# StarsX/FluidX12

Measured on AMD Instinct MI355X. Metric: voxel-updates/sec (advect+40 Jacobi) at 256^3; achieved HBM GB/s vs peak, higher is better.
Workload: dtype f32

## Files before the change

fluidx12_amd/build.py:

```python
import os
import shutil
import subprocess
import sys

HERE = os.path.dirname(os.path.abspath(__file__))
CSRC = os.path.join(HERE, "csrc")
ROOT = os.path.dirname(HERE)
LIB = os.path.join(HERE, "libfluidx_hip.so")
OBJDIR = os.path.join(HERE, "build")

SOURCES = ["fx_api.cpp", "fx_knobs.cpp", "fx_context.cpp", "fx_schedule.cpp", "fx_jacobi_plan.cpp", "fx_emit_plan.cpp", "fx_heat_plan.cpp", "fx_comm.cpp", "fx_checkpoint.cpp", "fx_sim.hip", "fx_vorticity.hip", "fx_emit.hip", "fx_obstacle.hip", "fx_heat.hip", "fx_open.hip", "fx_advect_lds.hip", "fx_jacobi_strip.hip", "fx_jacobi_strip3.hip", "fx_jacobi_strip4.hip", "fx_jacobi_block.hip", "fx_jacobi_freeze.hip", "fx_jacobi_stripm.hip", "fx_jacobi2d.hip", "fx_render.hip", "fx_render_accel.hip", "fx_resolve.hip", "fx_bc6h.hip", "fx_sh.hip"]
HEADERS = ["fx_internal.h", "fx_context.h", "fx_host.h", "fx_hostmath.h", "fx_pk.h", "fx_march.h", "fx_store.h", "fx_knobs.h", os.path.join(ROOT, "include", "fluidx_hip.h")]

FLAGS = ["--offload-arch=gfx950", "-O3", "-std=c++17", "-fPIC", "-ffp-contract=off", "-fno-fast-math",
         "-Wall", "-Wno-unused-function", "-D__HIP_PLATFORM_AMD__"]
LAB = os.environ.get("FLUIDX_BUILD_LAB", "0") == "1"
if LAB:
    FLAGS = FLAGS + ["-DFX_LAB"]


EXTRA_FLAGS = {"fx_jacobi_strip3.hip": ["-mllvm", "-amdgpu-sched-strategy=max-ilp"] + (["-DFX_STRIP3C_ROWS=" + os.environ["FLUIDX_BUILD_STRIP3C_ROWS"]] if os.environ.get("FLUIDX_BUILD_STRIP3C_ROWS") else []),
               "fx_jacobi_strip.hip": ["-mllvm", "-amdgpu-sched-strategy=max-ilp"],
               "fx_jacobi_strip4.hip": (os.environ["FLUIDX_BUILD_STRIP4_SCHED"].split() if os.environ.get("FLUIDX_BUILD_STRIP4_SCHED") is not None else ["-mllvm", "-amdgpu-sched-strategy=max-ilp"]) + (["-DFX_STRIP4_OUTER_ROWS=" + os.environ["FLUIDX_BUILD_STRIP4_OUTER_ROWS"]] if os.environ.get("FLUIDX_BUILD_STRIP4_OUTER_ROWS") else []) + os.environ.get("FLUIDX_BUILD_STRIP4_DEFS", "").split(),
               "fx_render_accel.hip": [("-D%s=%s" % (d, os.environ[e])) for e, d in (("FLUIDX_BUILD_MASK_BITS", "FX_MASK_BUDGET_BITS"), ("FLUIDX_BUILD_VIEW_AHEAD", "FX_VIEW_AHEAD"), ("FLUIDX_BUILD_LIGHT_AHEAD", "FX_LIGHT_AHEAD"), ("FLUIDX_BUILD_LIGHT_RAY_WGS", "FX_LIGHT_RAY_WGS"), ("FLUIDX_BUILD_LIGHT_RAY_UNROLL", "FX_LIGHT_RAY_UNROLL"), ("FLUIDX_BUILD_VIEW_NT", "FX_VIEW_NT"), ("FLUIDX_BUILD_VIEW_WPE", "FX_VIEW_WPE")) if os.environ.get(e)],
               "fx_jacobi_freeze.hip": ["-mllvm", "-amdgpu-atomic-optimizer-strategy=None"] + (["-DFX_FREEZE_PROF"] if os.environ.get("FLUIDX_BUILD_FREEZE_PROF") else [])}


def kernel_source_hash(kernel):
    import hashlib
    import re
    pat = re.compile(r"\bvoid\s+" + re.escape(kernel) + r"\s*\(")
    for s in SOURCES:
        if not s.endswith(".hip"):
            continue
        text = open(os.path.join(CSRC, s), "rb").read()
        if pat.search(text.decode("utf-8", "replace")):
            h = hashlib.sha256()
            h.update(text)
            h.update(open(os.path.join(CSRC, "fx_pk.h"), "rb").read())
            if b'#include "fx_march.h"' in text:
                h.update(open(os.path.join(CSRC, "fx_march.h"), "rb").read())
            h.update(" ".join(FLAGS + EXTRA_FLAGS.get(s, [])).encode())
            return h.hexdigest()[:16]
    return None


def hipcc():
    exe = shutil.which("hipcc") or "/opt/rocm/bin/hipcc"
    if not os.path.exists(exe):
        raise RuntimeError("hipcc not found: the HIP library cannot be built")
    return exe


def _newer(path, deps):
    if not os.path.exists(path):
        return True
    t = os.path.getmtime(path)
    return any(os.path.getmtime(d) > t for d in deps)


def build_lib(force=False, verbose=False):
    os.makedirs(OBJDIR, exist_ok=True)
    hdrs = [h if os.path.isabs(h) else os.path.join(CSRC, h) for h in HEADERS]
    objs = []
    cc = hipcc()
# ... 63 lines not shown
```

fluidx12_amd/capi.py:

```python
import ctypes as C
import os

from . import build as _build

FX_OK = 0
FX_E_INVALID, FX_E_DEVICE, FX_E_NOMEM, FX_E_STATE, FX_E_COMM, FX_E_HALO = -1, -2, -3, -4, -5, -6

RAY_MARCH_DIRECT, RAY_MARCH_CUBEMAP, SEPARATE_LIGHT_PASS, OPTIMIZED = 0, 1, 2, 3
FRAME_COUNT = 3
STORAGE_FP32, STORAGE_FP16 = 0, 1
JACOBI_FIXED, JACOBI_FAITHFUL = 0, 1
ADDRESS_CLAMP, ADDRESS_MIRROR = 0, 1
FLAG_JACOBI_FUSE_MASK, FLAG_NO_OVERLAP, FLAG_RENDER_ONLY = 0xF, 0x10, 0x20
OPT_OVERLAP, OPT_JACOBI_ROUND, OPT_ADAPTIVE_HALO, OPT_COUNT_SAMPLES, OPT_RENDER_ACCEL = 1, 2, 3, 4, 5
ABI_VERSION = 7
(FIELD_VELOCITY, FIELD_VELOCITY1, FIELD_COLOR, FIELD_COLOR_PREV, FIELD_PRESSURE, FIELD_DIVERGENCE,
 FIELD_LIGHTMAP, FIELD_CUBEMAP, FIELD_TARGET, FIELD_TARGET_FLOAT, FIELD_CUBE_DEPTH) = range(11)
FIELD_TEMPERATURE = 11
DEPTH_DEVICE = 0x1
LIGHT_DIRECTIONAL, LIGHT_POINT = 0, 1
MAX_EMITTERS = 16
OBSTACLES_DEVICE = 0x1
MAX_HEAT_SOURCES = 16
WALL_X_LO, WALL_X_HI, WALL_Y_LO, WALL_Y_HI, WALL_Z_LO, WALL_Z_HI = 0x01, 0x02, 0x04, 0x08, 0x10, 0x20
# ... 16 lines not shown

class Light(C.Structure):
    _fields_ = [("struct_size", C.c_uint32), ("kind", C.c_uint32), ("position", C.c_float * 3), ("color", C.c_float * 4),
                ("ambient", C.c_float * 4)]


class Emitter(C.Structure):
    _fields_ = [("struct_size", C.c_uint32), ("flags", C.c_uint32), ("center", C.c_float * 3), ("radius", C.c_float),
                ("color_rate", C.c_float * 4), ("force", C.c_float * 3), ("swirl", C.c_float)]


class Buoyancy(C.Structure):
    _fields_ = [("struct_size", C.c_uint32), ("flags", C.c_uint32), ("ambient", C.c_float), ("density_weight", C.c_float),
                ("lift", C.c_float), ("cooling", C.c_float), ("up", C.c_float * 3)]


class HeatSource(C.Structure):
    _fields_ = [("struct_size", C.c_uint32), ("flags", C.c_uint32), ("center", C.c_float * 3), ("radius", C.c_float), ("rate", C.c_float)]


class Timing(C.Structure):
    _fields_ = [("advect_ms", C.c_double), ("divergence_ms", C.c_double), ("jacobi_ms", C.c_double),
                ("project_ms", C.c_double), ("light_ms", C.c_double), ("view_ms", C.c_double),
                ("exchange_ms", C.c_double), ("steps", C.c_uint64), ("jacobi_launches", C.c_uint64),
                ("jacobi_sweeps", C.c_uint64), ("renders", C.c_uint64), ("resolve_ms", C.c_double),
                ("jacobi_main_ms", C.c_double), ("jacobi_main_launches", C.c_uint64), ("jacobi_main_sweeps", C.c_uint64),
                ("exchange_bytes", C.c_uint64), ("advect_halo_planes", C.c_uint64), ("chain_ms", C.c_double),
                ("freeze_solves", C.c_uint64), ("freeze_sweeps", C.c_uint64), ("exchange_calls", C.c_uint64),
                ("view_samples", C.c_uint64), ("light_samples", C.c_uint64), ("lightmap_fetches", C.c_uint64),
                ("freeze_strip_launches", C.c_uint64)]


_vp, _fp = C.c_void_p, C.POINTER(C.c_float)
SYMBOLS = {
    "fx_abi_version": (C.c_int, []),
    "fx_error_string": (C.c_char_p, [C.c_int]),
    "fx_create": (C.c_int, [C.POINTER(_vp), C.POINTER(Desc)]),
    "fx_destroy": (C.c_int, [_vp]),
    "fx_set_max_samples": (C.c_int, [_vp, C.c_uint32, C.c_uint32]),
    "fx_set_sh": (C.c_int, [_vp, _fp]),
    "fx_update_frame": (C.c_int, [_vp, C.c_float, C.c_uint8, _fp, _fp, _fp]),
    "fx_simulate": (C.c_int, [_vp, _vp, C.c_uint8]),
    "fx_render": (C.c_int, [_vp, _vp, C.c_uint8, C.c_uint8]),
    "fx_get_frame_info": (C.c_int, [_vp, C.POINTER(FrameInfo)]),
    "fx_synchronize": (C.c_int, [_vp]),
    "fx_last_error": (C.c_char_p, [_vp]),
    "fx_upload": (C.c_int, [_vp, C.c_int, _vp, C.c_size_t]),
    "fx_download": (C.c_int, [_vp, C.c_int, _vp, C.c_size_t]),
    "fx_field_bytes": (C.c_size_t, [_vp, C.c_int]),
    "fx_field_digest": (C.c_int, [_vp, C.c_int, C.c_uint32, C.c_uint32, C.POINTER(C.c_uint64)]),
    "fx_checkpoint_save": (C.c_int, [_vp, C.c_char_p]),
    "fx_checkpoint_load": (C.c_int, [_vp, C.c_char_p]),
    "fx_advect": (C.c_int, [_vp, _vp]),
    "fx_divergence": (C.c_int, [_vp, _vp]),
    "fx_jacobi": (C.c_int, [_vp, _vp, C.c_uint32]),
    "fx_project": (C.c_int, [_vp, _vp]),
    "fx_set_vorticity_confinement": (C.c_int, [_vp, C.c_float]),
    "fx_confine_vorticity": (C.c_int, [_vp, _vp]),
    "fx_set_emitters": (C.c_int, [_vp, C.POINTER(Emitter), C.c_uint32]),
    "fx_get_emitters": (C.c_int, [_vp, C.POINTER(Emitter), C.c_uint32, C.POINTER(C.c_uint32)]),
    "fx_set_impulse": (C.c_int, [_vp, C.c_int]),
    "fx_emit": (C.c_int, [_vp, _vp]),
    "fx_set_obstacles": (C.c_int, [_vp, _vp, _vp, C.c_size_t, C.c_uint32]),
    "fx_get_obstacles": (C.c_int, [_vp, _vp, C.c_size_t, C.POINTER(C.c_uint64)]),
    "fx_enforce_obstacles": (C.c_int, [_vp, _vp]),
    "fx_set_buoyancy": (C.c_int, [_vp, C.POINTER(Buoyancy)]),
    "fx_get_buoyancy": (C.c_int, [_vp, C.POINTER(Buoyancy), C.POINTER(C.c_int)]),
    "fx_set_heat_sources": (C.c_int, [_vp, C.POINTER(HeatSource), C.c_uint32]),
    "fx_get_heat_sources": (C.c_int, [_vp, C.POINTER(HeatSource), C.c_uint32, C.POINTER(C.c_uint32)]),
    "fx_heat": (C.c_int, [_vp, _vp]),
    "fx_set_open_walls": (C.c_int, [_vp, C.c_uint32]),
    "fx_get_open_walls": (C.c_int, [_vp, C.POINTER(C.c_uint32)]),
    "fx_open_inflow": (C.c_int, [_vp, _vp]),
    "fx_sh_transform": (C.c_int, [_vp, _fp, C.c_uint32, _fp]),
    "fx_set_environment": (C.c_int, [_vp, _fp, C.c_uint32]),
    "fx_render_environment": (C.c_int, [_vp, _vp, C.c_uint8]),
    "fx_clear_render_target": (C.c_int, [_vp, _vp, _fp]),
    "fx_render_cube": (C.c_int, [_vp, _vp, C.c_uint8]),
    "fx_set_scene_depth": (C.c_int, [_vp, _vp, _vp, C.c_uint32, C.c_uint32, C.c_float, C.c_float, C.c_uint32]),
    "fx_set_light": (C.c_int, [_vp, C.POINTER(Light)]),
    "fx_get_light": (C.c_int, [_vp, C.POINTER(Light)]),
    "fx_dds_cube_info": (C.c_int, [_vp, C.c_size_t, C.POINTER(C.c_uint32), C.POINTER(C.c_uint32)]),
    "fx_dds_decode_cube": (C.c_int, [_vp, _vp, C.c_size_t, C.c_uint32, _fp, C.c_size_t]),
    "fx_timing_enable": (C.c_int, [_vp, C.c_int]),
    "fx_set_option": (C.c_int, [_vp, C.c_uint32, C.c_uint32]),
    "fx_set_knob": (C.c_int, [C.c_char_p, C.c_char_p]),
    "fx_knob_name": (C.c_char_p, [C.c_uint32]),
    "fx_comm_gather_color": (C.c_int, [_vp, _vp, _vp, C.c_int, C.POINTER(C.c_uint32), C.POINTER(C.c_uint32)]),
    "fx_timing_read": (C.c_int, [_vp, C.POINTER(Timing), C.c_int]),
    "fx_comm_id_bytes": (C.c_size_t, []),
    "fx_comm_get_unique_id": (C.c_int, [_vp, C.c_size_t]),
    "fx_comm_init_rank": (C.c_int, [_vp, _vp, C.c_size_t, C.c_int, C.c_int]),
    "fx_comm_init_local": (C.c_int, [C.POINTER(_vp), C.c_int]),
    "fx_comm_init_peer": (C.c_int, [C.POINTER(_vp), C.c_int]),
}

_lib = None
LAB_KNOBS = {"ADVECT_BLOCK", "ADVECT_FAST", "ADVECT_LDS_HALF", "ADVECT_TILE_ROWS", "ADVECT_ZCHUNK", "BLOCK_REMAP", "BLOCK_SHAPE", "DEBUG_NO_COPY",
             "FREEZE_DENSE_LEVELS", "FREEZE_DENSE_ONE", "FREEZE_FAST", "FREEZE_FUSE_DIV", "FREEZE_NT", "FREEZE_SHRINK", "FREEZE_T", "FREEZE_WGS",
             "JACOBI2D_TILE", "JACOBI_BLOCK", "JACOBI_BLOCKG", "LIGHT_FILL_DIRTY", "LIGHT_RAY_NT", "LIGHT_RAY_WGS", "OBSTACLE_V4", "PROJECT_V4", "ROW_VW",
             "STRIP3H_PAIRS", "STRIP3_COOP", "STRIP3_NO512", "STRIP3_OFF", "STRIP3_ZCHUNK", "STRIP4T", "STRIP4T_256", "STRIP4T_512", "STRIP4T_FROM", "STRIP4T_GRID", "STRIP4T_NARROW", "STRIP4T_NARROW_FROM", "STRIP4T_PIECES", "STRIP4X", "STRIP4X_MINP", "STRIP4X_NT", "STRIP4X_ORDER", "STRIP4X_WGS",
             "STRIP4_OCTET", "STRIP4_ZCHUNK", "STRIP4_ZFLOOR", "STRIP_GENERIC", "STRIP_R", "STRIP_REMAP", "STRIP_WGS", "STRIP_WIDE", "STRIP_ZCHUNK", "VIEW_ORDER", "VIEW_WGS", "VORT_ZCHUNK", "XCD_REMAP"}


def lib_path():
    return _build.LIB
# ... 62 lines not shown
```

fluidx12_amd/csrc/fx_advect_lds.hip:

```cpp
#include "fx_internal.h"
#include <algorithm>
#include <cstdlib>
#include <cstdio>

namespace fx {

namespace {

constexpr int TX = 64;
constexpr int HX = TX + 2;
constexpr int NSLOT = 4;
template <bool HALF, int TY> struct Lay {
	static constexpr int NCELL = HX * (TY + 2);
	static constexpr int VEL_BYTES = NCELL * 4;
	static constexpr int COL_BYTES = HALF ? 2 * NCELL * 4 : NCELL * 16;
	static constexpr int SLOT_BYTES = COL_BYTES + 3 * VEL_BYTES;
};
typedef _Float16 h16;
typedef _Float16 h16x4 __attribute__((ext_vector_type(4)));
__device__ __forceinline__ h16 to_h16(float v) { asm("" : "+v"(v)); return (h16)v; }
__device__ __forceinline__ float lo_half(uint32_t d) { return (float)__builtin_bit_cast(h16, (uint16_t)(d & 0xffffu)); }
__device__ __forceinline__ float hi_half(uint32_t d) { return (float)__builtin_bit_cast(h16, (uint16_t)(d >> 16)); }

__device__ __forceinline__ float lerpf(float a, float b, float f) { return fmaf(f, b - a, a); }
__device__ __forceinline__ float saturatef(float x) { return fminf(fmaxf(x, 0.0f), 1.0f); }

__device__ __forceinline__ int addr_tap(int i, int n, int mode)
{
	if (mode == FX_ADDRESS_MIRROR) {
		const int period = 2 * n;
		int m = i % period;
		if (m < 0) m += period;
		return m < n ? m : period - 1 - m;
	}
	return min(max(i, 0), n - 1);
}

typedef __attribute__((address_space(3))) void lds_void;
typedef const __attribute__((address_space(1))) void glb_void;

template <int VEL_BYTES>
__device__ __forceinline__ void stage64(const void* col, const void* v0, const void* v1, const void* v2, uint32_t off_col, uint32_t off_vel, uint32_t lds_col, uint32_t lds_vel)
{
	uint32_t keep;
	lds_col = __builtin_amdgcn_readfirstlane(lds_col);
	lds_vel = __builtin_amdgcn_readfirstlane(lds_vel);
	asm volatile(
		"s_mov_b32 %0, m0\n\t"
		"s_mov_b32 m0, %7\n\t"
		"s_nop 0\n\t"
		"global_load_lds_dwordx4 %5, %1\n\t"
		"s_mov_b32 m0, %8\n\t"
		"s_nop 0\n\t"
		"global_load_lds_dword %6, %2\n\t"
		"s_add_u32 m0, m0, %9\n\t"
		"s_nop 0\n\t"
		"global_load_lds_dword %6, %3\n\t"
		"s_add_u32 m0, m0, %9\n\t"
		"s_nop 0\n\t"
		"global_load_lds_dword %6, %4\n\t"
		"s_mov_b32 m0, %0"
		: "=&s"(keep)
		: "s"(col), "s"(v0), "s"(v1), "s"(v2), "v"(off_col), "v"(off_vel), "s"(lds_col), "s"(lds_vel), "n"(VEL_BYTES)
		: "scc");
}

template <int VEL_BYTES>
__device__ __forceinline__ void stage64h(const void* col, const void* v0, const void* v1, const void* v2, uint32_t off_col, uint32_t off_vel, uint32_t lds_col, uint32_t lds_vel)
{
	uint32_t keep;
	lds_col = __builtin_amdgcn_readfirstlane(lds_col);
	lds_vel = __builtin_amdgcn_readfirstlane(lds_vel);
	const uint32_t off_col_hi = off_col + 4u;
	asm volatile(
		"s_mov_b32 %0, m0\n\t"
		"s_mov_b32 m0, %8\n\t"
		"s_nop 0\n\t"
		"global_load_lds_dword %5, %1\n\t"
		"s_add_u32 m0, m0, %10\n\t"
		"s_nop 0\n\t"
		"global_load_lds_dword %6, %1\n\t"
		"s_mov_b32 m0, %9\n\t"
		"s_nop 0\n\t"
		"global_load_lds_ushort %7, %2\n\t"
		"s_add_u32 m0, m0, %10\n\t"
		"s_nop 0\n\t"
		"global_load_lds_ushort %7, %3\n\t"
		"s_add_u32 m0, m0, %10\n\t"
		"s_nop 0\n\t"
		"global_load_lds_ushort %7, %4\n\t"
		"s_mov_b32 m0, %0"
		: "=&s"(keep)
		: "s"(col), "s"(v0), "s"(v1), "s"(v2), "v"(off_col), "v"(off_col_hi), "v"(off_vel), "s"(lds_col), "s"(lds_vel), "n"(VEL_BYTES)
		: "scc");
}

template <typename T>
__device__ __forceinline__ T ldg32(const void* base, uint32_t byte_off)
{
	return *reinterpret_cast<const T*>(static_cast<const char*>(base) + byte_off);
}


template <bool P2> __device__ __forceinline__ uint32_t rows(uint32_t y, int lgX, const Geom& g) { return P2 ? y << lgX : y * (uint32_t)g.X; }
template <bool P2> __device__ __forceinline__ uint32_t planes(uint32_t z, int lgP, const Geom& g) { return P2 ? z << lgP : z * ((uint32_t)g.X * (uint32_t)g.Y); }

template <bool HALF, bool P2>
__device__ __forceinline__ void advect_gather(const Geom& g, const SimParams& sp, int ix, int iy, int z0, int z1, bool z_present, float fx, float fy, float fz,
	const char* v0, const char* v1, const char* v2, const void* __restrict__ col_in, int lgX, int lgP, unsigned* halo_overflow, float (&u)[3], float (&c)[4])
{
	const int xa0 = addr_tap(ix, g.X, sp.address), xa1 = addr_tap(ix + 1, g.X, sp.address);
	const int ya0 = addr_tap(iy, g.Y, sp.address), ya1 = addr_tap(iy + 1, g.Y, sp.address);
	if (!z_present) {
		atomicOr(halo_overflow, 1u);
		z0 = min(max(z0, g.zlo), g.zhi);
		z1 = min(max(z1, g.zlo), g.zhi);
	}
	const uint32_t p0 = planes<P2>((uint32_t)g.lz(z0), lgP, g), p1 = planes<P2>((uint32_t)g.lz(z1), lgP, g);
	const uint32_t ry0 = rows<P2>((uint32_t)ya0, lgX, g), ry1 = rows<P2>((uint32_t)ya1, lgX, g);
	const uint32_t c000 = p0 + ry0 + (uint32_t)xa0, c100 = p0 + ry0 + (uint32_t)xa1;
	const uint32_t c010 = p0 + ry1 + (uint32_t)xa0, c110 = p0 + ry1 + (uint32_t)xa1;
	const uint32_t c001 = p1 + ry0 + (uint32_t)xa0, c101 = p1 + ry0 + (uint32_t)xa1;
	const uint32_t c011 = p1 + ry1 + (uint32_t)xa0, c111 = p1 + ry1 + (uint32_t)xa1;
	const char* vb[3] = { v0, v1, v2 };
	auto gv = [](const char* b, uint32_t cell) -> float { return HALF ? (float)ldg32<h16>(b, cell * 2u) : ldg32<float>(b, cell * 4u); };
	auto gc = [&](uint32_t cell) -> float4 {
		if (HALF) { const h16x4 h = ldg32<h16x4>(col_in, cell * 8u); return make_float4((float)h.x, (float)h.y, (float)h.z, (float)h.w); }
		return ldg32<float4>(col_in, cell * 16u);
	};
#pragma unroll
	for (int a = 0; a < 3; ++a) {
		const float c00 = lerpf(gv(vb[a], c000), gv(vb[a], c100), fx);
		const float c10 = lerpf(gv(vb[a], c010), gv(vb[a], c110), fx);
		const float c01 = lerpf(gv(vb[a], c001), gv(vb[a], c101), fx);
		const float c11 = lerpf(gv(vb[a], c011), gv(vb[a], c111), fx);
		u[a] = lerpf(lerpf(c00, c10, fy), lerpf(c01, c11, fy), fz);
	}
	const float4 t000 = gc(c000), t100 = gc(c100), t010 = gc(c010), t110 = gc(c110);
	const float4 t001 = gc(c001), t101 = gc(c101), t011 = gc(c011), t111 = gc(c111);
#define FX_TRI(m) lerpf(lerpf(lerpf(t000.m, t100.m, fx), lerpf(t010.m, t110.m, fx), fy), \
	lerpf(lerpf(t001.m, t101.m, fx), lerpf(t011.m, t111.m, fx), fy), fz)
	c[0] = FX_TRI(x); c[1] = FX_TRI(y); c[2] = FX_TRI(z); c[3] = FX_TRI(w);
#undef FX_TRI
}

template <bool HALF, bool ALPHA>
__device__ __forceinline__ void advect_finish(const SimParams& sp, float (&u)[3], float (&c)[4], float ex, float dx, float dz, float dt, float atten,
	uint32_t id, uint32_t stride, void* __restrict__ vel_out, void* __restrict__ col_out, float* __restrict__ alpha_out)
{
	if (__builtin_amdgcn_ballot_w64(sp.impulse && ex > -6.5f) != 0) {
		const float basis = exp2f(ex);
		if (basis >= 0.0183156393f) {
			float Fx, Fy, Fz;
			if (sp.is3d) {
				Fx = fmaf(basis, 0.0f, dz * -200.0f);
				Fy = fmaf(basis, 192.0f, 0.0f);
				Fz = fmaf(basis, 0.0f, dx * 200.0f);
			} else {
				Fx = 0.0f; Fy = basis * 48.0f; Fz = 0.0f;
			}
			u[0] = fmaf(Fx, dt, u[0]); u[1] = fmaf(Fy, dt, u[1]); u[2] = fmaf(Fz, dt, u[2]);
			const float bdt = basis * dt;
			c[0] = saturatef(fmaf(bdt, 8.0f, c[0]));
			c[1] = saturatef(fmaf(bdt, 16.0f, c[1]));
			c[2] = saturatef(fmaf(bdt, 40.0f, c[2]));
			c[3] = saturatef(fmaf(bdt, 40.0f, c[3]));
		}
	}
	char* vo = static_cast<char*>(vel_out);
	char* co = static_cast<char*>(col_out);
	if (HALF) {
		*reinterpret_cast<h16*>(vo + id * 2u) = to_h16(u[0] * atten);
		*reinterpret_cast<h16*>(vo + (stride + id) * 2u) = to_h16(u[1] * atten);
		*reinterpret_cast<h16*>(vo + (2u * stride + id) * 2u) = to_h16(u[2] * atten);
		h16x4 hc;
		hc.x = to_h16(c[0] * atten); hc.y = to_h16(c[1] * atten); hc.z = to_h16(c[2] * atten); hc.w = to_h16(c[3] * atten);
		*reinterpret_cast<h16x4*>(co + id * 8u) = hc;
		if (ALPHA) *reinterpret_cast<float*>(reinterpret_cast<char*>(alpha_out) + id * 4u) = (float)hc.w;
	} else {
		*reinterpret_cast<float*>(vo + id * 4u) = u[0] * atten;
		*reinterpret_cast<float*>(vo + (stride + id) * 4u) = u[1] * atten;
		*reinterpret_cast<float*>(vo + (2u * stride + id) * 4u) = u[2] * atten;
		*reinterpret_cast<float4*>(co + id * 16u) = make_float4(c[0] * atten, c[1] * atten, c[2] * atten, c[3] * atten);
		if (ALPHA) *reinterpret_cast<float*>(reinterpret_cast<char*>(alpha_out) + id * 4u) = c[3] * atten;
	}
}

}

template <bool HALF, int TY, bool DEFER, bool P2, bool ALPHA>
__global__ __launch_bounds__(64 * TY) __attribute__((amdgpu_waves_per_eu(4, 4))) void k_advect_lds(const Geom g, const SimParams sp,
	const void* __restrict__ vel_in, const void* __restrict__ col_in, void* __restrict__ vel_out, void* __restrict__ col_out, float* __restrict__ alpha_out,
	int z_begin, int nzp, int zchunk, int nchunks, unsigned* halo_overflow, float rX, float rY, float rZ, float inv_rr,
	int lgX, int lgY, int lg_gx, int lg_gy, uint32_t* __restrict__ far_list, uint32_t* __restrict__ far_flat, uint32_t* __restrict__ far_total, uint32_t far_cap)
{
	__shared__ uint32_t far_n, far_base;
	extern __shared__ __attribute__((aligned(16))) char lds[];

	const int tid = (int)threadIdx.x, lane = tid & 63, wave = __builtin_amdgcn_readfirstlane(tid >> 6);
	const int ntx = P2 ? 1 << lg_gx : lg_gx, nty = P2 ? 1 << lg_gy : lg_gy;
	const int ntiles = ntx * nty * nchunks;
	int tl = (int)blockIdx.x;
	{
		const int q = ntiles >> 3, r = ntiles & 7, xcd = tl & 7, j = tl >> 3;
		tl = xcd * q + min(xcd, r) + j;
	}
	const int tx = P2 ? tl & (ntx - 1) : tl % ntx, ty = P2 ? (tl >> lg_gx) & (nty - 1) : (tl / ntx) % nty, chunk = P2 ? tl >> (lg_gx + lg_gy) : tl / (ntx * nty);
	const int x0t = tx << 6, y0t = ty * TY;
	const int zb = z_begin + chunk * zchunk, ze = min(zb + zchunk, z_begin + nzp);
	if (zb >= ze) return;

	const int lgP = lgX + lgY;
	constexpr int COL_BYTES = Lay<HALF, TY>::COL_BYTES, SLOT_BYTES = Lay<HALF, TY>::SLOT_BYTES;
	constexpr int NCELL = Lay<HALF, TY>::NCELL, VEL_BYTES = Lay<HALF, TY>::VEL_BYTES, NT = 64 * TY;
	constexpr uint32_t ES = HALF ? 2 : 4, CS = HALF ? 8 : 16;
	const uint32_t stride = planes<P2>((uint32_t)g.nzl(), lgP, g);
	const char* v0 = reinterpret_cast<const char*>(vel_in);
	const char* v1 = v0 + (size_t)stride * ES;
	const char* v2 = v1 + (size_t)stride * ES;

	uint32_t src_a, src_b = 0;
	{
		const int c = tid, r = c / HX, cc = c - r * HX;
		src_a = rows<P2>((uint32_t)addr_tap(y0t - 1 + r, g.Y, sp.address), lgX, g) + (uint32_t)addr_tap(x0t - 1 + cc, g.X, sp.address);
	}
	const bool has_b = NT + tid < NCELL;
	if (has_b) {
		const int c = NT + tid, r = c / HX, cc = c - r * HX;
		src_b = rows<P2>((uint32_t)addr_tap(y0t - 1 + r, g.Y, sp.address), lgX, g) + (uint32_t)addr_tap(x0t - 1 + cc, g.X, sp.address);
	}
	const bool wave_has_b = NT + wave * 64 < NCELL;

	const uint32_t lds0 = (uint32_t)(size_t)(__attribute__((address_space(3))) char*)lds;
	auto fill = [&](int zq) {
		const int za = min(max(addr_tap(zq, g.Zg, sp.address), g.zlo), g.zhi);
		const size_t pz = planes<P2>((uint32_t)g.lz(za), lgP, g);
		const uint32_t slot = __builtin_amdgcn_readfirstlane(lds0 + (uint32_t)(((zq + 4) & 3) * SLOT_BYTES));
		const char* bc = reinterpret_cast<const char*>(col_in) + pz * CS;
		const char *b0 = v0 + pz * ES, *b1 = v1 + pz * ES, *b2 = v2 + pz * ES;
		if (HALF) stage64h<VEL_BYTES>(bc, b0, b1, b2, src_a * CS, src_a * ES, slot + (uint32_t)wave * (64 * 4), slot + COL_BYTES + (uint32_t)wave * (64 * 4));
		else stage64<VEL_BYTES>(bc, b0, b1, b2, src_a * CS, src_a * ES, slot + (uint32_t)wave * (64 * 16), slot + COL_BYTES + (uint32_t)wave * (64 * 4));
		if (wave_has_b) {
			if (has_b) {
				if (HALF) stage64h<VEL_BYTES>(bc, b0, b1, b2, src_b * CS, src_b * ES, slot + (NT + (uint32_t)wave * 64) * 4, slot + COL_BYTES + (NT + (uint32_t)wave * 64) * 4);
				else stage64<VEL_BYTES>(bc, b0, b1, b2, src_b * CS, src_b * ES, slot + (NT + (uint32_t)wave * 64) * 16, slot + COL_BYTES + (NT + (uint32_t)wave * 64) * 4);
			}
		}
	};

	if (DEFER && tid == 0) far_n = 0u;
	fill(zb - 1);
	fill(zb);
	fill(zb + 1);
	asm volatile("s_waitcnt vmcnt(0)" ::: "memory");
	__syncthreads();

	const int x = x0t + lane, y = y0t + wave;
	const bool has_voxel = P2 || (x < g.X && y < g.Y);
	const float dt = sp.dt;
	const float px = P2 ? ((float)x + 0.5f) * rX : ((float)x + 0.5f) / (float)g.X;
	const float py = P2 ? ((float)y + 0.5f) * rY : ((float)y + 0.5f) / (float)g.Y;
	const float dx = px + -0.5f, dy = py + -0.100000001f;
	const float dxy2 = fmaf(dy, dy, dx * dx);
	const uint32_t own = (uint32_t)((wave + 1) * HX + lane + 1);
	const float atten = fmaxf(fmaf(-dt, 0.200000003f, 1.0f), 0.0f);

	auto compute = [&](int z) {
		if (!has_voxel) return;
		const float pz = P2 ? ((float)z + 0.5f) * rZ : ((float)z + 0.5f) / (float)g.Zg;
		const float dz = pz + -0.5f;
		const float d2 = fmaf(dz, dz, dxy2);
		const float ex = ((d2 * -4.0f) * inv_rr) * 1.44269502f;

		const char* sc = lds + ((z + 4) & 3) * SLOT_BYTES;
		const uint32_t* vs = reinterpret_cast<const uint32_t*>(sc + COL_BYTES);
		auto vval = [](uint32_t d) -> float { return HALF ? lo_half(d) : __uint_as_float(d); };
		const float u0x = vval(vs[own]), u0y = vval(vs[NCELL + own]), u0z = vval(vs[2 * NCELL + own]);
		const float ax = fmaf(-u0x, dt, px), ay = fmaf(-u0y, dt, py), az = fmaf(-u0z, dt, pz);
		const float tx_ = ax * (float)g.X - 0.5f, ty_ = ay * (float)g.Y - 0.5f, tz_ = az * (float)g.Zg - 0.5f;
		const float flx = floorf(tx_), fly = floorf(ty_), flz = floorf(tz_);
		const float fx = tx_ - flx, fy = ty_ - fly, fz = tz_ - flz;
		const int ix = (int)flx, iy = (int)fly, iz = (int)flz;
		const int jx = ix - x, jy = iy - y, jz = iz - z;
		int z0 = addr_tap(iz, g.Zg, sp.address), z1 = addr_tap(iz + 1, g.Zg, sp.address);
		const bool z_present = z0 >= g.zlo && z0 <= g.zhi && z1 >= g.zlo && z1 <= g.zhi;
		const bool inwin = (unsigned)(jx + 1) <= 1u && (unsigned)(jy + 1) <= 1u && (unsigned)(jz + 1) <= 1u && z_present;

		float u[3], c[4];
		if (DEFER && !inwin) {
			const uint32_t slot = atomicAdd(&far_n, 1u);
			far_list[(size_t)blockIdx.x * far_cap + slot] = P2 ? (uint32_t)x | (uint32_t)y << lgX | (uint32_t)z << lgP
				: ((uint32_t)z * (uint32_t)g.Y + (uint32_t)y) * (uint32_t)g.X + (uint32_t)x;
		}
		if (DEFER || inwin) {
			const int kx = DEFER && !inwin ? 0 : jx, ky = DEFER && !inwin ? 0 : jy, kz = DEFER && !inwin ? z : iz;
			const uint32_t c0 = (uint32_t)((int)own + ky * HX + kx);
			const char* s0 = lds + ((kz + 4) & 3) * SLOT_BYTES;
			const char* s1 = lds + ((kz + 5) & 3) * SLOT_BYTES;
#pragma unroll
			for (int a = 0; a < 3; ++a) {
				const uint32_t* p0 = reinterpret_cast<const uint32_t*>(s0 + COL_BYTES + a * VEL_BYTES) + c0;
				const uint32_t* p1 = reinterpret_cast<const uint32_t*>(s1 + COL_BYTES + a * VEL_BYTES) + c0;
				const float c00 = lerpf(vval(p0[0]), vval(p0[1]), fx);
				const float c10 = lerpf(vval(p0[HX]), vval(p0[HX + 1]), fx);
				const float c01 = lerpf(vval(p1[0]), vval(p1[1]), fx);
				const float c11 = lerpf(vval(p1[HX]), vval(p1[HX + 1]), fx);
				u[a] = lerpf(lerpf(c00, c10, fy), lerpf(c01, c11, fy), fz);
			}
			float4 t000, t100, t010, t110, t001, t101, t011, t111;
			if (HALF) {
				auto tex = [](const char* slot, uint32_t c) -> float4 {
					const uint32_t rg = reinterpret_cast<const uint32_t*>(slot)[c], ba = reinterpret_cast<const uint32_t*>(slot)[NCELL + c];
					return make_float4(lo_half(rg), hi_half(rg), lo_half(ba), hi_half(ba));
				};
				t000 = tex(s0, c0); t100 = tex(s0, c0 + 1); t010 = tex(s0, c0 + HX); t110 = tex(s0, c0 + HX + 1);
				t001 = tex(s1, c0); t101 = tex(s1, c0 + 1); t011 = tex(s1, c0 + HX); t111 = tex(s1, c0 + HX + 1);
			} else {
				const float4* q0 = reinterpret_cast<const float4*>(s0) + c0;
				const float4* q1 = reinterpret_cast<const float4*>(s1) + c0;
				t000 = q0[0]; t100 = q0[1]; t010 = q0[HX]; t110 = q0[HX + 1];
				t001 = q1[0]; t101 = q1[1]; t011 = q1[HX]; t111 = q1[HX + 1];
			}
#define FX_TRI(m) lerpf(lerpf(lerpf(t000.m, t100.m, fx), lerpf(t010.m, t110.m, fx), fy), \
	lerpf(lerpf(t001.m, t101.m, fx), lerpf(t011.m, t111.m, fx), fy), fz)
			c[0] = FX_TRI(x); c[1] = FX_TRI(y); c[2] = FX_TRI(z); c[3] = FX_TRI(w);
#undef FX_TRI
		} else {
			advect_gather<HALF, P2>(g, sp, ix, iy, z0, z1, z_present, fx, fy, fz, v0, v1, v2, col_in, lgX, lgP, halo_overflow, u, c);
		}

		const uint32_t id = planes<P2>((uint32_t)g.lz(z), lgP, g) + rows<P2>((uint32_t)y, lgX, g) + (uint32_t)x;
		advect_finish<HALF, ALPHA>(sp, u, c, ex, dx, dz, dt, atten, id, stride, vel_out, col_out, alpha_out);
	};

	for (int z = zb; z < ze; ++z) {
		if (z + 2 <= ze) fill(z + 2);
		compute(z);
		if (!(P2 || y < g.Y)) asm volatile("s_waitcnt vmcnt(0)" ::: "memory");
		else if (ALPHA) asm volatile("s_waitcnt vmcnt(5)" ::: "memory");
		else asm volatile("s_waitcnt vmcnt(4)" ::: "memory");
		__syncthreads();
	}
	if (DEFER) {
		const uint32_t n = far_n;
		if (n != 0u) {
			if (tid == 0) far_base = atomicAdd(far_total, n);
			__syncthreads();
			const uint32_t base = far_base;
			const uint32_t* seg = far_list + (size_t)blockIdx.x * far_cap;
			for (uint32_t i = (uint32_t)tid; i < n; i += (uint32_t)NT) far_flat[base + i] = seg[i];
		}
	}
}

template <bool HALF, bool P2, bool ALPHA>
__global__ __launch_bounds__(256) void k_advect_far(const Geom g, const SimParams sp,
	const void* __restrict__ vel_in, const void* __restrict__ col_in, void* __restrict__ vel_out, void* __restrict__ col_out, float* __restrict__ alpha_out,
	const uint32_t* __restrict__ far_flat, const uint32_t* __restrict__ far_total, uint32_t* __restrict__ far_total_next, unsigned* halo_overflow,
	float rX, float rY, float rZ, float inv_rr, int lgX, int lgY)
{
	const uint32_t n = *far_total;
	if (blockIdx.x == 0 && threadIdx.x == 0) *far_total_next = 0u;
	const int lgP = lgX + lgY;
	constexpr uint32_t ES = HALF ? 2 : 4;
	const uint32_t stride = planes<P2>((uint32_t)g.nzl(), lgP, g);
	const char* v0 = reinterpret_cast<const char*>(vel_in);
	const char* v1 = v0 + (size_t)stride * ES;
	const char* v2 = v1 + (size_t)stride * ES;
	const float dt = sp.dt;
	const float atten = fmaxf(fmaf(-dt, 0.200000003f, 1.0f), 0.0f);
	for (uint32_t i = blockIdx.x * 256u + threadIdx.x; i < n; i += gridDim.x * 256u) {
		const uint32_t code = far_flat[i];
		int x, y, z;
		if (P2) { x = (int)(code & (uint32_t)(g.X - 1)); y = (int)((code >> lgX) & (uint32_t)(g.Y - 1)); z = (int)(code >> lgP); }
		else { const uint32_t XY = (uint32_t)g.X * (uint32_t)g.Y, rem = code % XY; z = (int)(code / XY); y = (int)(rem / (uint32_t)g.X); x = (int)(rem % (uint32_t)g.X); }
		const float px = P2 ? ((float)x + 0.5f) * rX : ((float)x + 0.5f) / (float)g.X;
		const float py = P2 ? ((float)y + 0.5f) * rY : ((float)y + 0.5f) / (float)g.Y;
		const float pz = P2 ? ((float)z + 0.5f) * rZ : ((float)z + 0.5f) / (float)g.Zg;
		const float dx = px + -0.5f, dy = py + -0.100000001f, dz = pz + -0.5f;
		const float dxy2 = fmaf(dy, dy, dx * dx);
		const float d2 = fmaf(dz, dz, dxy2);
		const float ex = ((d2 * -4.0f) * inv_rr) * 1.44269502f;
		const uint32_t id = planes<P2>((uint32_t)g.lz(z), lgP, g) + rows<P2>((uint32_t)y, lgX, g) + (uint32_t)x;
		auto gv = [](const char* b, uint32_t cell) -> float { return HALF ? (float)ldg32<h16>(b, cell * 2u) : ldg32<float>(b, cell * 4u); };
		const float u0x = gv(v0, id), u0y = gv(v1, id), u0z = gv(v2, id);
		const float ax = fmaf(-u0x, dt, px), ay = fmaf(-u0y, dt, py), az = fmaf(-u0z, dt, pz);
		const float tx_ = ax * (float)g.X - 0.5f, ty_ = ay * (float)g.Y - 0.5f, tz_ = az * (float)g.Zg - 0.5f;
		const float flx = floorf(tx_), fly = floorf(ty_), flz = floorf(tz_);
		const float fx = tx_ - flx, fy = ty_ - fly, fz = tz_ - flz;
		const int ix = (int)flx, iy = (int)fly, iz = (int)flz;
		const int z0 = addr_tap(iz, g.Zg, sp.address), z1 = addr_tap(iz + 1, g.Zg, sp.address);
		const bool z_present = z0 >= g.zlo && z0 <= g.zhi && z1 >= g.zlo && z1 <= g.zhi;
		float u[3], c[4];
		advect_gather<HALF, P2>(g, sp, ix, iy, z0, z1, z_present, fx, fy, fz, v0, v1, v2, col_in, lgX, lgP, halo_overflow, u, c);
		advect_finish<HALF, ALPHA>(sp, u, c, ex, dx, dz, dt, atten, id, stride, vel_out, col_out, alpha_out);
	}
}


hipError_t launch_advect_lds(const Geom& g, const SimParams& sp, int half_store, const void* vel_in, const void* col_in,
	void* vel_out, void* col_out, int z_begin, int z_end, unsigned* halo_overflow, uint32_t* far_scratch, size_t far_words, int far_parity, bool* far_used, hipStream_t s, bool force,
	AdvectAlpha* alpha)
{
	if (far_used) *far_used = false;
	if (alpha) alpha->written = false;
	auto pow2 = [](int v) { return v > 0 && (v & (v - 1)) == 0; };
	const int nzp = z_end - z_begin;
	const bool p2 = pow2(g.X) && pow2(g.Y) && pow2(g.Zg);
	const int TY = p2 && FX_KNOB_INT("ADVECT_TILE_ROWS", 8) == 16 ? 16 : 8;
	const size_t min_voxels = (size_t)1 << 22;
	if (g.Zg <= 1 || g.X < TX || g.Y < TY || nzp < 12 || (!force && (size_t)g.X * g.Y * (size_t)nzp < min_voxels) ||
		g.cells_local() * 16 >= ((size_t)1 << 32))
		return hipErrorNotSupported;
	const int half_on = FX_KNOB_INT("ADVECT_LDS_HALF", 1);
	if (half_store && !half_on) return hipErrorNotSupported;
	auto lg = [](int v) { int k = 0; while ((1 << k) < v) ++k; return k; };
	const int ntx = (g.X + TX - 1) / TX, nty = (g.Y + TY - 1) / TY;
	const int lgX = lg(g.X), lgY = lg(g.Y), lg_gx = p2 ? lg(ntx) : ntx, lg_gy = p2 ? lg(nty) : nty;
	const int tiles_xy = ntx * nty;
	const bool want_defer = far_scratch && FX_KNOB_INT("ADVECT_DEFER", 1) != 0;
	int zchunk = FX_KNOB_INT("ADVECT_ZCHUNK", want_defer ? 32 : 16);
	if (!p2 && !FX_KNOB("ADVECT_ZCHUNK")) {
		const int chunks = std::max(1, 512 / tiles_xy);
		zchunk = std::max(8, (nzp + chunks - 1) / chunks);
	}
	if (zchunk < 4) zchunk = 4;
	if (zchunk > nzp) zchunk = nzp;
	const int nchunks = (nzp + zchunk - 1) / zchunk;
	const float rX = 1.0f / (float)g.X, rY = 1.0f / (float)g.Y, rZ = 1.0f / (float)g.Zg, inv_rr = sp.is3d ? 256.0f : 1024.0f;
	const uint32_t nwg = (uint32_t)(tiles_xy * nchunks), far_cap = (uint32_t)(TX * TY * zchunk);
	const size_t flat_words = (size_t)g.X * g.Y * (size_t)nzp;
	const bool defer = want_defer && far_words >= 2 + flat_words + (size_t)nwg * far_cap && ((uint64_t)g.Zg << (lgX + lgY)) <= ((uint64_t)1 << 32);
	if (far_used) *far_used = defer;
	uint32_t* far_total = far_scratch ? far_scratch + (far_parity & 1) : nullptr;
	uint32_t* far_total_next = far_scratch ? far_scratch + ((far_parity & 1) ^ 1) : nullptr;
	uint32_t* far_flat = far_scratch ? far_scratch + 2 : nullptr;
	uint32_t* far_list = far_scratch ? far_scratch + 2 + flat_words : nullptr;
#define FX_ADV(H_, TY_, D_, P_, A_) do { \
		static bool attr_set = false; \
		if (!attr_set) { (void)hipFuncSetAttribute(reinterpret_cast<const void*>(k_advect_lds<H_, TY_, D_, P_, A_>), hipFuncAttributeMaxDynamicSharedMemorySize, NSLOT * Lay<H_, TY_>::SLOT_BYTES); attr_set = true; } \
		hipLaunchKernelGGL((k_advect_lds<H_, TY_, D_, P_, A_>), dim3(tiles_xy * nchunks), dim3(64 * TY_), (NSLOT * Lay<H_, TY_>::SLOT_BYTES), s, g, sp, vel_in, col_in, vel_out, col_out, alpha_out, \
			z_begin, nzp, zchunk, nchunks, halo_overflow, rX, rY, rZ, inv_rr, lgX, lgY, lg_gx, lg_gy, far_list, far_flat, far_total, far_cap); } while (0)
#define FX_FAR(H_, P_, A_) hipLaunchKernelGGL((k_advect_far<H_, P_, A_>), dim3(far_wgs), dim3(256), 0, s, g, sp, vel_in, col_in, vel_out, col_out, alpha_out, far_flat, far_total, far_total_next, halo_overflow, rX, rY, rZ, inv_rr, lgX, lgY)
	const int far_wgs = 1024;
	float* alpha_out = alpha && alpha->out && defer && TY == 8 && g.nzl() == g.Zg && z_begin == 0 && z_end == g.Zg ? alpha->out : nullptr;
	if (alpha_out) {
		if (half_store) { if (p2) { FX_ADV(true, 8, true, true, true); FX_FAR(true, true, true); } else { FX_ADV(true, 8, true, false, true); FX_FAR(true, false, true); } }
		else { if (p2) { FX_ADV(false, 8, true, true, true); FX_FAR(false, true, true); } else { FX_ADV(false, 8, true, false, true); FX_FAR(false, false, true); } }
		alpha->written = true;
	} else if (!p2) {
		if (defer) {
			if (half_store) { FX_ADV(true, 8, true, false, false); FX_FAR(true, false, false); } else { FX_ADV(false, 8, true, false, false); FX_FAR(false, false, false); }
		} else { if (half_store) FX_ADV(true, 8, false, false, false); else FX_ADV(false, 8, false, false, false); }
	} else if (defer) {
		if (TY == 16) { if (half_store) FX_ADV(true, 16, true, true, false); else FX_ADV(false, 16, true, true, false); }
		else { if (half_store) FX_ADV(true, 8, true, true, false); else FX_ADV(false, 8, true, true, false); }
		if (half_store) FX_FAR(true, true, false); else FX_FAR(false, true, false);
	} else {
		if (TY == 16) { if (half_store) FX_ADV(true, 16, false, true, false); else FX_ADV(false, 16, false, true, false); }
		else { if (half_store) FX_ADV(true, 8, false, true, false); else FX_ADV(false, 8, false, true, false); }
	}
#undef FX_FAR
#undef FX_ADV
	return hipGetLastError();
}

size_t advect_far_words(const Geom& g, int nzp)
{
	if (g.Zg <= 1 || g.X < TX || g.Y < 16 || nzp < 12) return 0;
	const size_t tiled = (size_t)((g.X + TX - 1) / TX * TX) * (size_t)((g.Y + 7) / 8 * 8);
	return 2 + (size_t)g.X * g.Y * (size_t)nzp + tiled * (size_t)(nzp + 32);
}

}
```

fluidx12_amd/csrc/fx_api.cpp:

```cpp
#include "fx_host.h"
#include <cstring>
#include "fx_hostmath.h"

using namespace fx;
using namespace fxh;

extern "C" {

int fx_abi_version(void) { return FX_ABI_VERSION; }

int fx_set_max_samples(fx_ctx* ctx, uint32_t max_ray, uint32_t max_light)
{
	if (!ctx || !max_ray || !max_light) return FX_E_INVALID;
	ctx->max_ray_samples = max_ray;
	ctx->max_light_samples = max_light;
	return FX_OK;
}

int fx_set_sh(fx_ctx* ctx, const float* coeffs27)
{
	if (!ctx) return FX_E_INVALID;
	if (!ctx->sh_dev) return FX_E_STATE;
	if (!coeffs27) { ctx->has_sh = false; return FX_OK; }
	DeviceGuard dg(ctx->device);
// ... 295 lines not shown

int fx_set_environment(fx_ctx* ctx, const float* cube, uint32_t n)
{
	if (!ctx || (cube && (!n || n > 8192))) return FX_E_INVALID;
	DeviceGuard dg(ctx->device);
	FX_HIP(hipDeviceSynchronize());
	if (ctx->env) { FX_HIP(hipFree(ctx->env)); ctx->env = nullptr; ctx->env_n = 0; }
	if (!cube) return FX_OK;
	const size_t bytes = (size_t)6 * n * n * 3 * sizeof(float);
	FX_HIP(hipMalloc((void**)&ctx->env, bytes));
	FX_HIP(hipMemcpy(ctx->env, cube, bytes, hipMemcpyHostToDevice));
	ctx->env_n = n;
	return FX_OK;
}

int fx_render_environment(fx_ctx* ctx, void* stream, uint8_t frame_index)
{
	if (!ctx || frame_index >= FX_FRAME_COUNT) return FX_E_INVALID;
	if (!ctx->env || !ctx->view_valid) return FX_E_STATE;
	DeviceGuard dg(ctx->device);
	hipStream_t s = pick_stream(ctx, stream);
	int rc = ensure_target(ctx, s);
	if (rc) return rc;
	ScopedMark mk(ctx, s, MK_RESOLVE);
	FX_HIP(launch_environment(ctx->env, (int)ctx->env_n, ctx->fc, (int)ctx->desc.viewport_w, (int)ctx->desc.viewport_h,
		ctx->target, ctx->target_float, s));
	return FX_OK;
}

int fx_get_frame_info(fx_ctx* ctx, fx_frame_info* out)
{
	if (!ctx || !out) return FX_E_INVALID;
	out->cube_lod = ctx->cube_lod;
	out->cube_size = (uint32_t)ctx->g.X >> ctx->cube_lod;
	out->ray_samples = ctx->ray_samples;
	out->visibility_mask = ctx->visibility_mask;
	out->frame_parity = ctx->frame_parity;
	out->edge_pixels = ctx->edge_pixels;
	out->time_step = ctx->time_step;
	std::memcpy(out->world_view_proj_i, ctx->fc.wvp_i, sizeof out->world_view_proj_i);
	std::memcpy(out->screen_to_world, ctx->fc.s2w, sizeof out->screen_to_world);
	return FX_OK;
}

int fx_advect(fx_ctx* ctx, void* stream)
{
	if (!ctx) return FX_E_INVALID;
	if (ctx->desc.flags & FX_FLAG_RENDER_ONLY) return FX_E_STATE;
	if (!ctx->frame_valid) return FX_E_STATE;
	if (ctx->nranks > 1) return FX_E_INVALID;
	hipStream_t s = pick_stream(ctx, stream);
	ScopedMark mk(ctx, s, MK_ADVECT);
	return advect_range(ctx, s, owned(ctx), false);
}

static int sim_guard(const fx_ctx* ctx, bool whole = true)
{
	if (!ctx) return FX_E_INVALID;
	if (ctx->desc.flags & FX_FLAG_RENDER_ONLY) return FX_E_STATE;
	if (whole && (ctx->g.nz != ctx->g.Zg || ctx->nranks > 1)) return FX_E_INVALID;
	return FX_OK;
}

static int run_stage(fx_ctx* ctx, void* stream, int (*phase)(fx_ctx*, hipStream_t))
{
	const int rc = sim_guard(ctx);
	return rc ? rc : phase(ctx, pick_stream(ctx, stream));
}

int fx_set_vorticity_confinement(fx_ctx* ctx, float epsilon)
{
	if (!std::isfinite(epsilon) || epsilon < 0.0f) return FX_E_INVALID;
	if (const int rc = sim_guard(ctx)) return rc;
	ctx->vort_eps = epsilon;
	return FX_OK;
}

int fx_confine_vorticity(fx_ctx* ctx, void* stream) { return run_stage(ctx, stream, confine_phase); }

int fx_set_emitters(fx_ctx* ctx, const fx_emitter* list, uint32_t count)
{
	if (const int rc = sim_guard(ctx)) return rc;
	if (count > FX_MAX_EMITTERS || (count && !list)) return FX_E_INVALID;
	for (uint32_t k = 0; k < count; ++k) {
		const fx_emitter& e = list[k];
		if (e.struct_size != sizeof(fx_emitter) || e.flags != 0) return FX_E_INVALID;
		if (!std::isfinite(e.radius) || !(e.radius > 0.0f) || !std::isfinite(e.swirl)) return FX_E_INVALID;
		for (int a = 0; a < 3; ++a) if (!std::isfinite(e.center[a]) || !std::isfinite(e.force[a])) return FX_E_INVALID;
		for (int a = 0; a < 4; ++a) if (!std::isfinite(e.color_rate[a]) || e.color_rate[a] < 0.0f) return FX_E_INVALID;
	}
	ctx->emitters.assign(list, list + count);
	return FX_OK;
}

int fx_get_emitters(fx_ctx* ctx, fx_emitter* out, uint32_t capacity, uint32_t* count)
{
	if (const int rc = sim_guard(ctx, false)) return rc;
	if (!count || (capacity && !out)) return FX_E_INVALID;
	*count = (uint32_t)ctx->emitters.size();
	for (uint32_t k = 0; k < capacity && k < *count; ++k) out[k] = ctx->emitters[k];
	return FX_OK;
}

int fx_set_impulse(fx_ctx* ctx, int enabled)
{
	if (const int rc = sim_guard(ctx, !enabled)) return rc;
// ... 333 lines not shown
			hipMemcpyAsync(ctx->rec_host, ctx->gath_dev, 4 * sizeof(int) * (size_t)nranks, hipMemcpyDeviceToHost, ctx->stream) == hipSuccess &&
			hipStreamSynchronize(ctx->stream) == hipSuccess;
		bool tiles = ok;
		for (int r = 0; ok && r + 1 < nranks; ++r) tiles = tiles && ctx->rec_host[4 * r] + ctx->rec_host[4 * r + 1] == ctx->rec_host[4 * (r + 1)];
		if (ok) ok = hipMemset(ctx->step_rec, 0, 4 * sizeof(int)) == hipSuccess;
		if (!ok || !tiles) {
			ctx->last_error = ok ? "fx_comm_init_rank: the slabs of the ranks do not tile the grid in rank order" : "fx_comm_init_rank: exchanging the slab ranges failed";
			std::fprintf(stderr, "fluidx: %s\n", ctx->last_error.c_str());
			destroy_lanes(g); delete t; delete g;
			return ok ? FX_E_INVALID : FX_E_COMM;
		}
	}
	ctx->group = g; ctx->rank = rank; ctx->nranks = nranks;
	return FX_OK;
}

int fx_comm_gather_color(fx_ctx* ctx, void* stream, fx_ctx* full, int root, const uint32_t* slab_z0, const uint32_t* slab_nz)
{
	if (!ctx || !ctx->group || root < 0 || root >= ctx->nranks) return FX_E_INVALID;
	if (group_broken(ctx)) return FX_E_STATE;
	if (!is_driver(ctx)) return FX_OK;
	const bool local = ctx->group->transport->is_local();
	const bool am_root = local || ctx->rank == root;
	if (am_root) {
		if (!full || full->g.X != ctx->g.X || full->g.Y != ctx->g.Y || full->g.Zg != ctx->g.Zg || full->g.nz != full->g.Zg ||
			full->half != ctx->half) return FX_E_INVALID;
		if (!local && full->device != ctx->device) return FX_E_INVALID;
		if (local && full->device != ctx->group->members[(size_t)root]->device) return FX_E_INVALID;
	}
	if (!local && (!slab_z0 || !slab_nz)) return FX_E_INVALID;
	const size_t plane_bytes = ctx->g.plane() * 4 * elem_size(ctx);
	std::vector<GatherPart> parts((size_t)ctx->nranks);
	for (int r = 0; r < ctx->nranks; ++r) {
		const fx_ctx* m = local ? ctx->group->members[r] : (r == ctx->rank ? ctx : nullptr);
		const uint32_t z0 = local ? (uint32_t)m->g.z0 : slab_z0[r], nz = local ? (uint32_t)m->g.nz : slab_nz[r];
		if (z0 > (uint32_t)ctx->g.Zg || nz > (uint32_t)ctx->g.Zg - z0) return FX_E_INVALID;
		if (!local && r == ctx->rank && (z0 != (uint32_t)ctx->g.z0 || nz != (uint32_t)ctx->g.nz)) return FX_E_INVALID;
		parts[r].rank = r;
		parts[r].bytes = (size_t)nz * plane_bytes;
		parts[r].src = m ? (const char*)m->col[m->frame_parity] + (size_t)m->g.H * plane_bytes : nullptr;
		parts[r].dst = am_root ? (char*)full->col[full->frame_parity] + (size_t)z0 * plane_bytes : nullptr;
		if (am_root) full->accel_alpha_of = nullptr;
	}
	DeviceGuard dg(ctx->device);
	hipStream_t s = pick_stream(ctx, stream);
	if (ctx->halo_fault) return FX_E_HALO;
	std::vector<hipStream_t> streams;
	if (ctx->group->per_member) for (fx_ctx* m : ctx->group->members) streams.push_back(m->stream);
	else streams.push_back(s);
	hipStream_t done_on = ctx->group->per_member ? streams[(size_t)root] : s;
	ScopedMark mk(ctx, s, MK_EXCH);
	int rc = ctx->group->transport->gather(ctx->group, parts, root, streams);
	if (rc) return rc;
	if (am_root && full->stream != done_on) {
		fx_lane& L = ctx->group->per_member ? ctx->group->lanes[(size_t)root] : ctx->group->lanes[0];
		DeviceGuard dgr(L.device);
		FX_HIP(hipEventRecord(L.ev_done, done_on));
		DeviceGuard dgf(full->device);
		FX_HIP(hipStreamWaitEvent(full->stream, L.ev_done, 0));
	}
	return FX_OK;
}

static int check_local_members(fx_ctx** ctxs, int nranks, bool one_device)
{
	if (!ctxs || nranks < 1) return FX_E_INVALID;
	int zexp = 0;
	for (int r = 0; r < nranks; ++r) {
		if (!ctxs[r]) return FX_E_INVALID;
		int rc = check_slab_chain(ctxs[r], r, nranks);
		if (rc) return rc;
		if (ctxs[r]->g.z0 != zexp || (one_device && ctxs[r]->device != ctxs[0]->device)) return FX_E_INVALID;
		const fx_desc &a = ctxs[r]->desc, &b = ctxs[0]->desc;
		if (a.grid_x != b.grid_x || a.grid_y != b.grid_y || a.grid_z != b.grid_z || a.halo_advect != b.halo_advect ||
			a.halo_jacobi != b.halo_jacobi || a.jacobi_iters != b.jacobi_iters || a.jacobi_mode != b.jacobi_mode ||
			a.storage != b.storage || a.advect_address != b.advect_address)
			return FX_E_INVALID;
		for (int q = 0; q < r; ++q) if (ctxs[q] == ctxs[r]) return FX_E_INVALID;
		zexp += ctxs[r]->g.nz;
	}
	return FX_OK;
}

static int init_in_process_group(fx_ctx** ctxs, int nranks, bool peer)
{
	int rc = check_local_members(ctxs, nranks, !peer);
	if (rc) return rc;
	if (peer) {
		for (int r = 0; r + 1 < nranks; ++r) {
			const int a = ctxs[r]->device, b = ctxs[r + 1]->device;
			if (a == b) continue;
			int ab = 0, ba = 0;
			if (hipDeviceCanAccessPeer(&ab, a, b) != hipSuccess || hipDeviceCanAccessPeer(&ba, b, a) != hipSuccess || !ab || !ba) {
				ctxs[0]->last_error = "fx_comm_init_peer: two neighbouring slabs live on devices without peer access";
				return FX_E_DEVICE;
			}
			for (int k = 0; k < 2; ++k) {
				DeviceGuard dg(k ? b : a);
				const hipError_t e = hipDeviceEnablePeerAccess(k ? a : b, 0);
				if (e != hipSuccess && e != hipErrorPeerAccessAlreadyEnabled) { (void)hipGetLastError(); return FX_E_DEVICE; }
				(void)hipGetLastError();
			}
		}
	}
	for (int r = 0; r < nranks; ++r)
		if (!ctxs[r]->step_rec) { if ((rc = make_step_record(ctxs[r], 1, false))) return rc; }
// ... 28 lines not shown
```

fluidx12_amd/csrc/fx_context.cpp:

```cpp
#include "fx_host.h"
#include <time.h>

using namespace fx;
using namespace fxh;

namespace fx {
bool digest_range_ok(const Geom& g, uint32_t z_begin, uint32_t z_count)
{
	if (!z_count) return true;
	if (g.nz < 0 || z_count > (uint32_t)g.nz) return false;
	const int64_t first = (int64_t)z_begin, end = first + (int64_t)z_count;
	return first >= (int64_t)g.z0 && end <= (int64_t)g.z0 + (int64_t)g.nz;
}
}

namespace fxh {

size_t ev_record(fx_ctx* c, hipStream_t s)
{
	if (c->ev_used == c->ev.size()) {
		hipEvent_t e;
		if (hipEventCreate(&e) != hipSuccess) return (size_t)-1;
		c->ev.push_back(e);
	}
// ... 12 lines not shown
		case MK_DIV: c->acc.divergence_ms += ms; break;
		case MK_JACOBI: c->acc.jacobi_ms += ms; c->acc.jacobi_launches += m.launches; c->acc.jacobi_sweeps += m.sweeps;
			c->acc.jacobi_main_ms += ms; c->acc.jacobi_main_launches += m.launches; c->acc.jacobi_main_sweeps += m.sweeps; break;
		case MK_JACOBI_TAIL: c->acc.jacobi_ms += ms; c->acc.jacobi_launches += m.launches; c->acc.jacobi_sweeps += m.sweeps; break;
		case MK_PROJECT: c->acc.project_ms += ms; break;
		case MK_LIGHT: c->acc.light_ms += ms; break;
		case MK_VIEW: c->acc.view_ms += ms; break;
		case MK_EXCH: c->acc.exchange_ms += ms; break;
		case MK_RESOLVE: c->acc.resolve_ms += ms; break;
		case MK_CHAIN: c->acc.chain_ms += ms; break;
		}
	}
	c->marks.clear();
	c->ev_used = 0;
	return FX_OK;
}

int ensure_stage(fx_ctx* ctx, size_t bytes)
{
	if (ctx->stage_bytes >= bytes) return FX_OK;
	if (ctx->stage) { FX_HIP(hipFree(ctx->stage)); ctx->stage = nullptr; ctx->stage_bytes = 0; }
	FX_HIP(hipMalloc((void**)&ctx->stage, bytes));
	ctx->stage_bytes = bytes;
	return FX_OK;
}

void destroy_lanes(fx_comm_group* g)
{
	for (fx_lane& l : g->lanes) {
		DeviceGuard dg(l.device);
		if (l.comm) (void)hipStreamDestroy(l.comm);
		if (l.face) (void)hipStreamDestroy(l.face);
		for (hipEvent_t e : { l.ev_ready, l.ev_done, l.ev_col_ready, l.ev_col_done, l.ev_int, l.ev_face1, l.x_ready, l.x_done }) if (e) (void)hipEventDestroy(e);
	}
	g->lanes.clear();
}

void group_release(fx_comm_group* g)
{
	{
		DeviceGuard dg(g->lanes.empty() ? 0 : g->lanes[0].device);
		if (g->shared_stream) (void)hipStreamDestroy(g->shared_stream);
	}
	destroy_lanes(g);
	delete g->transport;
	delete g;
}

void free_all(fx_ctx* c)
{
	for (int i = 0; i < 2; ++i) {
		if (c->vel[i]) (void)hipFree(c->vel[i]);
		if (c->col[i]) (void)hipFree(c->col[i]);
		if (c->p[i]) (void)hipFree(c->p[i]);
	}
	void* others[] = { c->env, c->cube_depth, c->depth_own, c->accel.occ, c->accel.alpha, c->accel.bits, c->accel.list, c->accel.cells, c->accel.gi, c->accel.ctr, c->target, c->target_float, c->p_face[0], c->p_face[1], c->b, c->frozen, c->frozen_alt, c->lightmap, c->cube, c->sh_dev, c->halo_overflow, c->stage,
		c->sh_scratch[0], c->sh_scratch[1], c->sh_scratch[2], c->sh_scratch[3], c->p_aux, c->fz_mask[0], c->fz_mask[1], c->fz_mask[2], c->fz_tile_next, c->fz_stat, c->fz_list[0], c->fz_list[1], c->fz_counts, c->sample_counters, c->adv_far, c->obst_code, c->obst_spare, c->obst_stats, c->temp[0], c->temp[1] };
	for (void* q : others) if (q) (void)hipFree(q);
	for (hipEvent_t e : c->ev) (void)hipEventDestroy(e);
	if (c->step_rec) (void)hipFree(c->step_rec);
	if (c->gath_dev) (void)hipFree(c->gath_dev);
	if (c->rec_host) (void)hipHostFree(c->rec_host);
	if (c->fz_active_host) (void)hipHostFree(c->fz_active_host);
	if (c->fz_active_ev) (void)hipEventDestroy(c->fz_active_ev);
	if (c->rec_ev) (void)hipEventDestroy(c->rec_ev);
	if (c->owns_stream && c->stream) (void)hipStreamDestroy(c->stream);
}

}

extern "C" {

const char* fx_error_string(int status)
{
	switch (status) {
	case FX_OK: return "ok";
	case FX_E_INVALID: return "invalid argument";
	case FX_E_DEVICE: return "HIP device/runtime error";
	case FX_E_NOMEM: return "out of memory";
	case FX_E_STATE: return "invalid call order";
	case FX_E_COMM: return "RCCL communication error";
	case FX_E_HALO: return "advection back-trace left the exchanged halo";
	default: return "unknown status";
	}
}

int fx_create(fx_ctx** out, const fx_desc* d)
{
	if (!out || !d || d->struct_size != sizeof(fx_desc)) return FX_E_INVALID;
	*out = nullptr;
	if (!d->grid_x || !d->grid_y || !d->grid_z) return FX_E_INVALID;
	if (d->grid_x != d->grid_y) return FX_E_INVALID;
	if (d->grid_x > 65535 || d->grid_z > 65535) return FX_E_INVALID;
	if (d->storage > FX_STORAGE_FP16 || d->jacobi_mode > FX_JACOBI_FAITHFUL || d->advect_address > FX_ADDRESS_MIRROR) return FX_E_INVALID;
	if (!d->jacobi_iters) return FX_E_INVALID;
	uint32_t z0 = d->slab_z0, nz = d->slab_nz ? d->slab_nz : d->grid_z;
	if (z0 + nz > d->grid_z) return FX_E_INVALID;
	const bool slab = nz != d->grid_z;

	int ndev = 0;
	if (hipGetDeviceCount(&ndev) != hipSuccess || ndev <= 0) return FX_E_DEVICE;
	int dev = d->device;
	if (dev < 0 && hipGetDevice(&dev) != hipSuccess) return FX_E_DEVICE;
	if (dev >= ndev) return FX_E_INVALID;

	fx_ctx* ctx = new (std::nothrow) fx_ctx();
	if (!ctx) return FX_E_NOMEM;
	ctx->desc = *d;
	ctx->desc.slab_z0 = z0; ctx->desc.slab_nz = nz;
	default_light(ctx);
// ... 29 lines not shown
			FX_HIP(hipMalloc((void**)&ctx->p[i], cells * 4));
			FX_HIP(hipMemsetAsync(ctx->vel[i], 0, 3 * cells * es, ctx->stream));
			FX_HIP(hipMemsetAsync(ctx->col[i], 0, 4 * cells * es, ctx->stream));
			FX_HIP(hipMemsetAsync(ctx->p[i], 0, cells * 4, ctx->stream));
		}
		if (slab && !(d->flags & FX_FLAG_RENDER_ONLY))
			for (int i = 0; i < 2; ++i) {
				FX_HIP(hipMalloc((void**)&ctx->p_face[i], cells * 4));
				FX_HIP(hipMemsetAsync(ctx->p_face[i], 0, cells * 4, ctx->stream));
			}
		if (!(d->flags & FX_FLAG_RENDER_ONLY)) {
			FX_HIP(hipMalloc((void**)&ctx->b, cells * 4));
			FX_HIP(hipMemsetAsync(ctx->b, 0, cells * 4, ctx->stream));
		}
		if (d->jacobi_mode == FX_JACOBI_FAITHFUL && !(d->flags & FX_FLAG_RENDER_ONLY)) {
			FX_HIP(hipMalloc((void**)&ctx->frozen, cells));
			FX_HIP(hipMemsetAsync(ctx->frozen, 0, cells, ctx->stream));
			if (ctx->g.Zg == 1) {
				FX_HIP(hipMalloc((void**)&ctx->frozen_alt, cells));
				FX_HIP(hipMemsetAsync(ctx->frozen_alt, 0, cells, ctx->stream));
			}
			if (jacobi_freeze_supported(ctx->g)) {
				const size_t mb = jacobi_freeze_mask_bytes(ctx->g), nt = (size_t)jacobi_freeze_tiles(ctx->g);
				FX_HIP(hipMalloc((void**)&ctx->p_aux, cells * 4));
				FX_HIP(hipMemsetAsync(ctx->p_aux, 0, cells * 4, ctx->stream));
				for (int i = 0; i < 3; ++i) {
					FX_HIP(hipMalloc((void**)&ctx->fz_mask[i], mb));
					FX_HIP(hipMemsetAsync(ctx->fz_mask[i], 0, mb, ctx->stream));
				}
				FX_HIP(hipMalloc((void**)&ctx->fz_tile_next, nt * sizeof(uint32_t)));
				FX_HIP(hipMemsetAsync(ctx->fz_tile_next, 0, nt * sizeof(uint32_t), ctx->stream));
				for (int i = 0; i < 2; ++i) FX_HIP(hipMalloc(&ctx->fz_list[i], jacobi_freeze_list_bytes(ctx->g)));
				FX_HIP(hipMalloc((void**)&ctx->fz_counts, 2 * jacobi_freeze_count_words() * sizeof(uint32_t)));
				FX_HIP(hipMemsetAsync(ctx->fz_counts, 0, 2 * jacobi_freeze_count_words() * sizeof(uint32_t), ctx->stream));
				FX_HIP(hipMalloc((void**)&ctx->fz_stat, kFreezeStatRing * sizeof(uint32_t)));
				FX_HIP(hipMemsetAsync(ctx->fz_stat, 0, kFreezeStatRing * sizeof(uint32_t), ctx->stream));
				ctx->fz_iters.assign(kFreezeStatRing, 0);
				if (jacobi_freeze_strip_supported(ctx->g) && hipHostMalloc((void**)&ctx->fz_active_host, 64, hipHostMallocMapped) == hipSuccess) {
					ctx->fz_active_host[0] = 0u;
					if (hipHostGetDevicePointer((void**)&ctx->fz_active_dev, ctx->fz_active_host, 0) != hipSuccess) ctx->fz_active_dev = nullptr;
				} else (void)hipGetLastError();
			}
		}
		FX_HIP(hipMalloc((void**)&ctx->halo_overflow, sizeof(unsigned)));
		FX_HIP(hipMemsetAsync(ctx->halo_overflow, 0, sizeof(unsigned), ctx->stream));
		if (!(d->flags & FX_FLAG_RENDER_ONLY)) {
			ctx->adv_far_tried = true;
			const size_t words = advect_far_words(ctx->g, ctx->g.nz);
			if (words) {
				if (hipMalloc((void**)&ctx->adv_far, words * sizeof(uint32_t)) == hipSuccess) {
					FX_HIP(hipMemsetAsync(ctx->adv_far, 0, 2 * sizeof(uint32_t), ctx->stream));
					ctx->adv_far_words = words;
				} else { (void)hipGetLastError(); ctx->adv_far = nullptr; }
			}
		}
		if (d->grid_z > 1) {
			FX_HIP(hipMalloc((void**)&ctx->lightmap, ctx->g.cells_owned() * 4));
			FX_HIP(hipMemsetAsync(ctx->lightmap, 0, ctx->g.cells_owned() * 4, ctx->stream));
			size_t off = 0;
			for (uint32_t m = 0; m < kNumMips; ++m) {
				ctx->cube_mip_offset[m] = off;
				const size_t sz = std::max<uint32_t>(d->grid_x >> m, 1);
				off += 6 * sz * sz * 4;
			}
			FX_HIP(hipMalloc((void**)&ctx->cube, off));
			FX_HIP(hipMemsetAsync(ctx->cube, 0, off, ctx->stream));
			if (d->viewport_w && d->viewport_h) {
				FX_HIP(hipMalloc((void**)&ctx->cube_depth, off));
				FX_HIP(hipMemsetD32Async((hipDeviceptr_t)ctx->cube_depth, 0x3f800000, off / 4, ctx->stream));
			}
			if (!slab && ctx->g.cells_owned() <= ((size_t)1 << 28) && ctx->g.X >= 4) {
				RenderAccel& A = ctx->accel;
				render_accel_layout(ctx->g, &A);
				const size_t ncell = (size_t)A.CX * A.CY * A.CZ, vox = ctx->g.cells_owned(), bw = render_accel_bits_words(A);
				FX_HIP(hipMalloc((void**)&A.occ, 2 * ncell * sizeof(float)));
				FX_HIP(hipMalloc((void**)&A.alpha, vox * sizeof(float)));
				FX_HIP(hipMalloc((void**)&A.bits, bw * sizeof(uint32_t)));
				FX_HIP(hipMemsetAsync(A.bits, 0, bw * sizeof(uint32_t), ctx->stream));
				FX_HIP(hipMalloc((void**)&A.list, vox * sizeof(uint32_t)));
				FX_HIP(hipMalloc((void**)&A.cells, ncell * sizeof(uint32_t)));
				FX_HIP(hipMalloc((void**)&A.ctr, render_accel_ctr_words(ctx->g) * sizeof(uint32_t)));
				FX_HIP(hipMemsetAsync(A.ctr, 0, render_accel_ctr_words(ctx->g) * sizeof(uint32_t), ctx->stream));
				ctx->accel_ok = true;
			}
			FX_HIP(hipMalloc((void**)&ctx->sh_dev, 27 * sizeof(float)));
			FX_HIP(hipMemsetAsync(ctx->sh_dev, 0, 27 * sizeof(float), ctx->stream));
		}
		FX_HIP(hipStreamSynchronize(ctx->stream));
		return FX_OK;
	}();
	if (rc != FX_OK) { free_all(ctx); delete ctx; return rc; }
	*out = ctx;
	return FX_OK;
}

int fx_destroy(fx_ctx* ctx)
{
	if (!ctx) return FX_E_INVALID;
	DeviceGuard dg(ctx->device);
	(void)hipDeviceSynchronize();
	if (ctx->group) {
		fx_comm_group* g = ctx->group;
		for (auto& m : g->members) if (m == ctx) m = nullptr;
		g->broken = true;
		if (--g->refs == 0) group_release(g);
	}
// ... 127 lines not shown
	const unsigned long long gfirst = (unsigned long long)z_begin * plane, gcells = (unsigned long long)g.Zg * plane;
	switch (field) {
	case FX_FIELD_VELOCITY: case FX_FIELD_VELOCITY1: {
		const char* src = (const char*)ctx->vel[field == FX_FIELD_VELOCITY1];
		for (int a = 0; a < 3; ++a) FX_HIP(launch_digest(src + (a * cl + first) * es, n, (int)es, a * gcells + gfirst, acc, ctx->stream));
		break;
	}
	case FX_FIELD_COLOR: case FX_FIELD_COLOR_PREV: {
		const char* src = (const char*)ctx->col[field == FX_FIELD_COLOR ? ctx->frame_parity : 1 - ctx->frame_parity];
		FX_HIP(launch_digest(src + first * 4 * es, 4 * n, (int)es, 4 * gfirst, acc, ctx->stream));
		break;
	}
	case FX_FIELD_PRESSURE: FX_HIP(launch_digest(ctx->p[ctx->p_cur] + first, n, 4, gfirst, acc, ctx->stream)); break;
	default: FX_HIP(launch_digest(ctx->b + first, n, 4, gfirst, acc, ctx->stream)); break;
	}
	FX_HIP(hipStreamSynchronize(ctx->stream));
	FX_HIP(hipMemcpy(out, acc, 16, hipMemcpyDeviceToHost));
	return FX_OK;
}

int fx_upload(fx_ctx* ctx, int field, const void* host, size_t bytes)
{
	if (!ctx || !host) return FX_E_INVALID;
	size_t need = 0;
	int rc = field_info(ctx, field, &need);
	if (rc) return rc;
	if (bytes != need) return FX_E_INVALID;
	DeviceGuard dg(ctx->device);
	FX_HIP(hipDeviceSynchronize());
	if (field <= FX_FIELD_DIVERGENCE || field == FX_FIELD_TEMPERATURE) { ctx->fz_dense_n = 0; ctx->fz_active_pending = false; }
	const size_t n = ctx->g.cells_owned(), off = (size_t)ctx->g.H * ctx->g.plane(), cl = ctx->g.cells_local();
	const size_t es = elem_size(ctx);
	switch (field) {
	case FX_FIELD_VELOCITY: case FX_FIELD_VELOCITY1: {
		if (field == FX_FIELD_VELOCITY && ctx->group) {
			if (!ctx->group->transport->is_local() && ctx->opt_adaptive && ctx->rec_pending && !ctx->collective_upload) return FX_E_STATE;
			ctx->need_valid = false;
		}
		char* dst = (char*)ctx->vel[field == FX_FIELD_VELOCITY1];
		if ((rc = ensure_stage(ctx, need))) return rc;
		FX_HIP(hipMemcpy(ctx->stage, host, need, hipMemcpyHostToDevice));
		for (int a = 0; a < 3; ++a)
			FX_HIP(launch_to_storage(ctx->stage + a * n, dst + (a * cl + off) * es, n, ctx->half, ctx->stream));
		break;
	}
	case FX_FIELD_COLOR: case FX_FIELD_COLOR_PREV: {
		if (ctx->col_halo_buf >= 0 && ctx->group) {
			if (!ctx->group->transport->is_local() && !ctx->collective_upload) return FX_E_STATE;
			if (ctx->group->transport->is_local()) { for (fx_ctx* m : ctx->group->members) if (m) m->col_halo_buf = -1; }
			else ctx->col_halo_buf = -1;
		}
		char* dst = (char*)ctx->col[field == FX_FIELD_COLOR ? ctx->frame_parity : 1 - ctx->frame_parity];
		if (ctx->accel_alpha_of == dst) ctx->accel_alpha_of = nullptr;
		if ((rc = ensure_stage(ctx, need))) return rc;
		FX_HIP(hipMemcpy(ctx->stage, host, need, hipMemcpyHostToDevice));
		FX_HIP(launch_to_storage(ctx->stage, dst + off * 4 * es, 4 * n, ctx->half, ctx->stream));
		break;
	}
	case FX_FIELD_PRESSURE:
		FX_HIP(hipMemcpy(ctx->p[ctx->p_cur] + off, host, need, hipMemcpyHostToDevice));
		break;
	case FX_FIELD_DIVERGENCE:
		FX_HIP(hipMemcpy(ctx->b + off, host, need, hipMemcpyHostToDevice));
		break;
	case FX_FIELD_TEMPERATURE:
		FX_HIP(hipMemcpy(ctx->temp[ctx->temp_cur], host, need, hipMemcpyHostToDevice));
		break;
	case FX_FIELD_CUBEMAP:
		FX_HIP(hipMemcpy(ctx->cube + ctx->cube_mip_offset[ctx->cube_lod], host, need, hipMemcpyHostToDevice));
		ctx->cube_depth_on[ctx->cube_lod] = false;
		break;
	default:
		return FX_E_INVALID;
	}
	FX_HIP(hipStreamSynchronize(ctx->stream));
	return FX_OK;
}

int fx_download(fx_ctx* ctx, int field, void* host, size_t bytes)
{
	if (!ctx || !host) return FX_E_INVALID;
	size_t need = 0;
	int rc = field_info(ctx, field, &need);
	if (rc) return rc;
	if (bytes != need) return FX_E_INVALID;
	DeviceGuard dg(ctx->device);
	FX_HIP(hipDeviceSynchronize());
	if (field <= FX_FIELD_DIVERGENCE && (rc = halo_fault_status(ctx))) return rc;
	const size_t n = ctx->g.cells_owned(), off = (size_t)ctx->g.H * ctx->g.plane(), cl = ctx->g.cells_local();
	const size_t es = elem_size(ctx);
	switch (field) {
	case FX_FIELD_VELOCITY: case FX_FIELD_VELOCITY1: {
		const char* src = (const char*)ctx->vel[field == FX_FIELD_VELOCITY1];
		if ((rc = ensure_stage(ctx, need))) return rc;
		for (int a = 0; a < 3; ++a)
			FX_HIP(launch_from_storage(src + (a * cl + off) * es, ctx->stage + a * n, n, ctx->half, ctx->stream));
		FX_HIP(hipStreamSynchronize(ctx->stream));
		FX_HIP(hipMemcpy(host, ctx->stage, need, hipMemcpyDeviceToHost));
		break;
	}
	case FX_FIELD_COLOR: case FX_FIELD_COLOR_PREV: {
		const char* src = (const char*)ctx->col[field == FX_FIELD_COLOR ? ctx->frame_parity : 1 - ctx->frame_parity];
		if ((rc = ensure_stage(ctx, need))) return rc;
		FX_HIP(launch_from_storage(src + off * 4 * es, ctx->stage, 4 * n, ctx->half, ctx->stream));
		FX_HIP(hipStreamSynchronize(ctx->stream));
		FX_HIP(hipMemcpy(host, ctx->stage, need, hipMemcpyDeviceToHost));
// ... 128 lines not shown
```

fluidx12_amd/csrc/fx_context.h:

```cpp
#pragma once
#include "fx_internal.h"
#include <vector>
#include <string>

struct fx_comm_group;
struct fx_lane;

struct fx_ctx {
	fx_desc desc;
	fx::Geom g;
	int half;
	int device;
	hipStream_t stream;
	bool owns_stream;

	void* vel[2];
	void* col[2];
	float* p[2];
	int p_cur;
	float* p_face[2];
	float* b;
	uint8_t* frozen;
	uint8_t* frozen_alt = nullptr;
	float* p_aux = nullptr;
	uint32_t* fz_active_host = nullptr;
	uint32_t* fz_active_dev = nullptr;
	hipEvent_t fz_active_ev = nullptr;
	bool fz_active_pending = false;
	int fz_dense_n = 0;
	uint8_t* fz_mask[3] = { nullptr, nullptr, nullptr };
	uint32_t* fz_tile_next = nullptr;
	void* fz_list[2] = { nullptr, nullptr };
	uint32_t* fz_counts = nullptr;
	uint32_t* fz_stat = nullptr;
	float* fz_x_p = nullptr;
	uint8_t* fz_x_m = nullptr;
	bool fz_fuse_div = false;
	uint32_t* adv_far = nullptr;
	bool adv_far_tried = false;
	size_t adv_far_words = 0;
	uint32_t adv_far_turn = 0;
	uint32_t fz_gen = 0;
	uint32_t fz_gen_mark = 0;
	std::vector<uint32_t> fz_iters;
	uint32_t* lightmap;
	uint8_t* cube;
	size_t cube_mip_offset[5];
	float* cube_depth;
	bool cube_depth_on[5];
	const float* depth;
	float* depth_own;
	float depth_zn, depth_zf;
	float vort_eps = 0.0f;
	std::vector<fx_emitter> emitters;
	bool impulse_on = true;
	uint8_t* obst_code = nullptr;
	uint8_t* obst_spare = nullptr;
	unsigned* obst_stats = nullptr;
	uint64_t obst_cells = 0;
	int obst_lo[3] = { 0, 0, 0 }, obst_hi[3] = { 0, 0, 0 };
	uint32_t open_faces = 0;
	bool buoy_on = false;
	fx_buoyancy buoy = { (uint32_t)sizeof(fx_buoyancy), 0u, 0.0f, 0.0f, 0.0f, 0.0f, { 0.0f, 1.0f, 0.0f } };
	float* temp[2] = { nullptr, nullptr };
	int temp_cur = 0;
	std::vector<fx_heat_source> heat_sources;
	uint32_t light_kind = 0;
	float wvp[16];
	float* env;
	uint32_t env_n;
	fx::RenderAccel accel = {};
	bool accel_ok = false;
	const void* accel_alpha_of = nullptr;
	bool rendered_since_step = false;
	bool lightmap_filled = false;
	float lightmap_key[9] = {};
	hipStream_t last_step_stream = nullptr;
	hipStream_t rendered_on = nullptr;
	int opt_render_accel = 1;
	uint8_t* target;
	float* target_float;
	float* sh_dev;
	bool has_sh;
	unsigned* halo_overflow;
	float* stage;
	size_t stage_bytes;
	float* sh_scratch[4];
	size_t sh_scratch_n;

	uint32_t max_ray_samples, max_light_samples;
	uint32_t ray_samples, cube_lod, visibility_mask;
	uint8_t frame_parity;
	float time_step;
	float edge_pixels;
// ... 98 lines not shown
```

fluidx12_amd/csrc/fx_internal.h:

```cpp
#pragma once
#include <hip/hip_runtime.h>
#include <stdint.h>
#include <stddef.h>
#include "../../include/fluidx_hip.h"
#include "fx_knobs.h"

namespace fx {

struct Geom {
	int X, Y;
	int Zg;
	int z0;
	int nz;
	int H;
	int zlo, zhi;
	__host__ __device__ size_t plane() const { return (size_t)X * Y; }
	__host__ __device__ int nzl() const { return nz + 2 * H; }
	__host__ __device__ size_t cells_local() const { return plane() * (size_t)nzl(); }
	__host__ __device__ size_t cells_owned() const { return plane() * (size_t)nz; }
	__host__ __device__ int lz(int z) const { return z - z0 + H; }
};
inline bool whole_grid(const Geom& g) { return g.nz == g.Zg && g.H == 0; }
inline bool open_faces_ok(const Geom& g, unsigned faces) { return !(faces & ~0x3Fu) && !(g.Zg <= 1 && (faces & (FX_WALL_Z_LO | FX_WALL_Z_HI))); }
inline bool colour_wants_wide_offsets(const Geom& g) { return g.cells_local() * 16 >= ((size_t)1 << 32); }

struct FrameConsts {
	float world_i[12];
	float world[12];
	float eye_pt[3];
	float light_pt[3];
	float light_color[4];
	float ambient[4];
	float wvp_i[16];
	float s2w[16];
};

struct DepthArgs {
	const float* depth;
	int W, H;
	float wvp[16];
	float z_near, z_far;
	float* cube_depth;
};

struct SimParams {
	float dt;
	int address;
	int is3d;
	int impulse = 1;
};

struct AdvectAlpha { float* out; bool written; };
hipError_t launch_advect(const Geom& g, const SimParams& sp, int half_store, const void* vel_in, const void* col_in,
	void* vel_out, void* col_out, int z_begin, int z_end, unsigned* halo_overflow, hipStream_t s, uint32_t* far_scratch = nullptr, size_t far_words = 0, int far_parity = 0, bool* far_used = nullptr,
	AdvectAlpha* alpha = nullptr);
hipError_t launch_advect_lds(const Geom& g, const SimParams& sp, int half_store, const void* vel_in, const void* col_in,
	void* vel_out, void* col_out, int z_begin, int z_end, unsigned* halo_overflow, uint32_t* far_scratch, size_t far_words, int far_parity, bool* far_used, hipStream_t s, bool force,
	AdvectAlpha* alpha = nullptr);
size_t advect_far_words(const Geom& g, int nzp);
hipError_t launch_confine_vorticity(const Geom& g, int half_store, const void* vel_in, void* vel_out, float eps, float dt, hipStream_t s);
const int kEmitTileX = 64, kEmitTileY = 4;
struct EmitBall { float c[3], rr, rate[4], force[3], swirl; int lo[3], hi[3]; };
struct EmitArgs { int n, x0, y0, z0, tiles_x, tiles_y, tiles_z; EmitBall e[FX_MAX_EMITTERS]; };
int emit_plan(const Geom& g, const fx_emitter* list, int count, EmitArgs* out);
hipError_t launch_emit(const Geom& g, int half_store, void* vel, void* col, float* alpha, const fx_emitter* list, int count, float dt, hipStream_t s);
const int kHeatTileX = 64, kHeatTileY = 4;
struct HeatBall { float c[3], rr, rate; int lo[3], hi[3]; };
struct HeatArgs { float ambient, weight, lift, cooling, up[3]; int axes, n, tiles_x, tiles_y; HeatBall s[FX_MAX_HEAT_SOURCES]; };
int heat_plan(const Geom& g, const fx_buoyancy& b, const fx_heat_source* list, int count, HeatArgs* out);
hipError_t launch_heat(const Geom& g, int half_store, const fx_buoyancy& b, const fx_heat_source* list, int count, const void* vel0, void* vel1,
	const void* col, const float* t_in, float* t_out, const uint8_t* code, float dt, int address, hipStream_t s, unsigned faces = 0);
__host__ __device__ inline float open_wall_weight(float fl, float f, int n, unsigned lo_open, unsigned hi_open)
{
	float w = 1.0f;
	if (lo_open && fl < 0.0f) w = fl == -1.0f ? f : 0.0f;
	if (hi_open && fl >= (float)(n - 1)) w = fl == (float)(n - 1) ? 1.0f - f : 0.0f;
	return w;
}
__host__ __device__ inline float open_wall_trace(float u0, float dt, int i, int n, unsigned lo_open, unsigned hi_open)
{
	const float p = ((float)i + 0.5f) / (float)n;
	const float a = fmaf(-u0, dt, p);
	const float t = a * (float)n - 0.5f;
	const float fl = floorf(t);
	return open_wall_weight(fl, t - fl, n, lo_open, hi_open);
}
const int kOpenTileX = 64, kOpenTileY = 4;
hipError_t launch_open_inflow(const Geom& g, int half_store, const void* vel0, void* col, float* alpha, unsigned faces, float dt, hipStream_t s);
hipError_t launch_divergence(const Geom& g, int half_store, const void* vel, float* b, int z_begin, int z_end, hipStream_t s);
hipError_t launch_obstacle_codes(const Geom& g, const uint8_t* solid_dev, uint8_t* code, unsigned* stats_dev, hipStream_t s);
hipError_t launch_obstacle_mask(const uint8_t* code, uint8_t* solid_dev, size_t n, hipStream_t s);
long long obstacle_enforce_tiles(const int lo[3], const int hi[3], int* x0, int* y0, int* tiles_x, int* tiles_y);
hipError_t launch_obstacle_enforce(const Geom& g, int half_store, const uint8_t* code, const int lo[3], const int hi[3], void* vel, void* col,
	float* alpha, hipStream_t s);
hipError_t launch_divergence_obs(const Geom& g, int half_store, const void* vel, const uint8_t* code, float* b, int z_begin, int z_end, hipStream_t s);
hipError_t launch_jacobi_bnd(const Geom& g, const float* p_in, const float* b, const uint8_t* code, float* p_out, unsigned faces,
	int z_begin, int z_end, hipStream_t s);
hipError_t launch_project_bnd(const Geom& g, const SimParams& sp, int half_store, const void* vel_in, const float* p, const uint8_t* code,
	void* vel_out, unsigned faces, int z_begin, int z_end, hipStream_t s);
enum SimStage { SIM_DIVERGENCE = 0, SIM_PROJECT = 1 };
enum SimRowKernel { ROW_SCALAR = 0, ROW_V4 = 4, ROW_VW2 = 2, ROW_VW3 = 3 };
int sim_row_kernel(const Geom& g, int half_store, int stage, int is3d);
bool digest_range_ok(const Geom& g, uint32_t z_begin, uint32_t z_count);
hipError_t launch_jacobi_sweep(const Geom& g, const float* p_in, const float* b, float* p_out, uint8_t* frozen,
	int z_begin, int z_end, hipStream_t s);
hipError_t launch_jacobi_sweep2(const Geom& g, const float* p_in, const float* b, float* p_out, uint8_t* frozen,
	int z_begin, int z_end, int z_begin2, int z_end2, hipStream_t s);
bool jacobi_strip_supported(const Geom& g);
bool jacobi_strip_wide(const Geom& g);
hipError_t launch_jacobi_strip(const Geom& g, const float* p_in, const float* b, float* p_out, int sweeps, int z_begin, int z_end, hipStream_t s);
bool jacobi_strip3_supported(const Geom& g);
// ... 118 lines not shown
```

fluidx12_amd/csrc/fx_schedule.cpp:

```cpp
#include "fx_host.h"
#include <memory>

using namespace fx;

namespace fxh {

int for_members(fx_ctx* ctx, std::vector<fx_ctx*>& out)
{
	out.clear();
	if (ctx->group && ctx->group->transport->is_local() && !ctx->group->broken) out = ctx->group->members;
	else out.push_back(ctx);
	return FX_OK;
}


static inline bool peer_group(const fx_ctx* c) { return c->group && c->group->per_member; }
static inline hipStream_t CS(const fx_ctx* m, hipStream_t s) { return peer_group(m) ? m->group->lane_of(m).compute : s; }
struct LaneRef { fx_lane* lane; hipStream_t compute; };
static std::vector<LaneRef> lanes_of(fx_ctx* lead, const std::vector<fx_ctx*>& M, hipStream_t s)
{
	std::vector<LaneRef> out;
	if (!lead->group) return out;
	if (lead->group->per_member) for (fx_ctx* m : M) out.push_back(LaneRef{ &lead->group->lane_of(m), lead->group->lane_of(m).compute });
	else out.push_back(LaneRef{ &lead->group->lanes[0], s });
// ... 21 lines not shown
	for (size_t i = 0; i < M.size(); ++i) {
		for (int j = 0; j < nspec; ++j) {
			if (specs[j].k <= 0) continue;
			ExchItem it[4];
			const int n = exchange_items(M[i], specs[j].set, specs[j].k, specs[j].pidx, it);
			halo_segments(M[i], it, n, segs[i]);
		}
		total += segs[i].size();
		if (M[i]->timing_on) for (const Seg& sg : segs[i]) M[i]->acc.exchange_bytes += sg.bytes;
	}
	if (!total) return FX_OK;
	for (fx_ctx* m : M) if (m->timing_on) m->acc.exchange_calls += 1;
	return ctx->group->transport->exchange(ctx->group, segs, streams, channel);
}

#define FX_LANES(body) do { for (const LaneRef& L : lanes_of(ctx, M, s)) { DeviceGuard dgl_(L.lane->device); body } } while (0)
static int comm_fork(fx_ctx* ctx, const std::vector<fx_ctx*>& M, hipStream_t s)
{
	FX_LANES(FX_HIP(hipEventRecord(L.lane->ev_ready, L.compute)); FX_HIP(hipStreamWaitEvent(L.lane->comm, L.lane->ev_ready, 0)););
	return FX_OK;
}
static int comm_mark_done(fx_ctx* ctx, const std::vector<fx_ctx*>& M, hipStream_t s) { FX_LANES(FX_HIP(hipEventRecord(L.lane->ev_done, L.lane->comm));); return FX_OK; }
static int comm_join(fx_ctx* ctx, const std::vector<fx_ctx*>& M, hipStream_t s) { FX_LANES(FX_HIP(hipStreamWaitEvent(L.compute, L.lane->ev_done, 0));); return FX_OK; }


int advect_range(fx_ctx* ctx, hipStream_t s, Range r, bool own_only)
{
	if (r.hi <= r.lo) return FX_OK;
	DeviceGuard dg(ctx->device);
	const SimParams sp{ ctx->time_step, (int)ctx->desc.advect_address, ctx->g.Zg > 1 ? 1 : 0, ctx->impulse_on ? 1 : 0 };
	const int par = ctx->frame_parity;
	Geom g = ctx->g;
	g.zlo = std::max(g.zlo, g.z0 - ctx->adv_w_lo); g.zhi = std::min(g.zhi, g.z0 + g.nz - 1 + ctx->adv_w_hi);
	if (own_only) { g.zlo = std::max(g.zlo, g.z0); g.zhi = std::min(g.zhi, g.z0 + g.nz - 1); }
	if (!ctx->adv_far && !ctx->adv_far_tried) {
		ctx->adv_far_tried = true;
		const size_t words = advect_far_words(g, g.nz);
		if (words) {
			if (hipMalloc((void**)&ctx->adv_far, words * sizeof(uint32_t)) == hipSuccess) {
				FX_HIP(hipMemsetAsync(ctx->adv_far, 0, 2 * sizeof(uint32_t), s));
				ctx->adv_far_words = words;
			} else {
				(void)hipGetLastError();
				ctx->adv_far = nullptr;
			}
		}
	}
	const bool lend = ctx->adv_far != nullptr;
	bool far_used = false;
	const bool frame_was_rendered = ctx->rendered_since_step && ctx->rendered_on == s;
	ctx->rendered_since_step = false;
	AdvectAlpha aa{ frame_was_rendered && ctx->accel_ok && ctx->opt_render_accel && FX_KNOB_INT("ADVECT_ALPHA", 1) ? ctx->accel.alpha : nullptr, false };
	if (ctx->accel_alpha_of == ctx->col[par]) ctx->accel_alpha_of = nullptr;
	FX_HIP(launch_advect(g, sp, ctx->half, ctx->vel[0], ctx->col[1 - par], ctx->vel[1], ctx->col[par],
		r.lo, r.hi, ctx->halo_overflow, s, lend ? ctx->adv_far : nullptr, lend ? ctx->adv_far_words : 0, (int)(ctx->adv_far_turn & 1u), &far_used, &aa));
	if (aa.written) ctx->accel_alpha_of = ctx->col[par];
	if (far_used) ++ctx->adv_far_turn;
	return FX_OK;
}

int options_digest(const fx_ctx* c)
{
	uint32_t h = 2166136261u;
	uint32_t dt_bits;
	std::memcpy(&dt_bits, &c->time_step, 4);
	for (uint32_t v : { (uint32_t)c->opt_overlap, (uint32_t)c->opt_round, (uint32_t)c->opt_adaptive, dt_bits }) h = (h ^ v) * 16777619u;
	return (int)(h & 0x3FFFFFFFu);
}

static int record_step(fx_ctx* ctx, std::vector<fx_ctx*>& M, hipStream_t s)
{
	if (!multi_rank(ctx) || !ctx->step_rec) return FX_OK;
	for (fx_ctx* m : M) {
		if (m->rec_in_project) { m->rec_in_project = false; continue; }
		DeviceGuard dg(m->device);
		FX_HIP(launch_face_need(m->g, m->half, m->vel[0], m->time_step, (int)m->desc.advect_address, options_digest(m), m->halo_overflow, m->step_rec, CS(m, s)));
	}
	DeviceGuard dg(ctx->device);
	if (ctx->group->transport->is_local()) {
		for (fx_ctx* m : M) {
			DeviceGuard dgm(m->device);
			FX_HIP(hipMemcpyAsync(m->rec_host, m->step_rec, 4 * sizeof(int), hipMemcpyDeviceToHost, CS(m, s)));
			FX_HIP(hipEventRecord(m->rec_ev, CS(m, s)));
		}
	} else {
		hipStream_t cs = s;
		if (overlap_level(ctx) >= 1) { int rc = comm_fork(ctx, M, s); if (rc) return rc; cs = ctx->group->lanes[0].comm; }
		if (ctx->group->transport->allgather(ctx->step_rec, 4, ctx->gath_dev, cs) != FX_OK) { ctx->last_error = "rccl: all-gather of the step record failed"; return FX_E_COMM; }
		FX_HIP(hipMemcpyAsync(ctx->rec_host, ctx->gath_dev, 4 * sizeof(int) * (size_t)ctx->nranks, hipMemcpyDeviceToHost, cs));
		FX_HIP(hipEventRecord(ctx->rec_ev, cs));
	}
	for (fx_ctx* m : M) { m->rec_pending = true; m->need_valid = true; m->rec_dt = m->time_step; }
	return FX_OK;
}

static int consume_record(fx_ctx* ctx, std::vector<fx_ctx*>& M)
{
	const int Ha = (int)ctx->desc.halo_advect;
	for (fx_ctx* m : M) { m->adv_w_lo = has_lower(m) ? Ha : 0; m->adv_w_hi = has_upper(m) ? Ha : 0; }
	if (!multi_rank(ctx) || !ctx->rec_pending) return FX_OK;
	const bool local = ctx->group->transport->is_local();
	for (fx_ctx* m : M) {
		DeviceGuard dg(m->device);
		FX_HIP(hipEventSynchronize(m->rec_ev));
		if (!local) break;
	}
	const int n = ctx->nranks;
	auto rec = [&](int r) -> const int* { return local ? M[(size_t)r]->rec_host : ctx->rec_host + 4 * r; };
// ... 41 lines not shown
	if (ov && ctx->group->min_nz <= 2 * Ha) ov = false;
	if (!ov) {
		if ((rc = consume_record(ctx, M))) return rc;
		if (col_ready) FX_LANES(FX_HIP(hipStreamWaitEvent(L.compute, L.lane->ev_col_done, 0)););
		const ExchSpec spec{ col_ready ? EX_ADVECT_VEL : EX_ADVECT_IN, Ha, 0 };
		if ((rc = do_exchange(ctx, M, &spec, 1, ON_COMPUTE, s))) return rc;
		for (fx_ctx* m : M) {
			ScopedMark mk(m, CS(m, s), MK_ADVECT);
			if (m->timing_on) m->acc.advect_halo_planes += (uint64_t)(m->adv_w_lo + m->adv_w_hi);
			if ((rc = advect_range(m, CS(m, s), owned(m), false))) return rc;
		}
		return FX_OK;
	}
	if ((rc = comm_fork(ctx, M, s))) return rc;
	for (fx_ctx* m : M) {
		ScopedMark mk(m, CS(m, s), MK_ADVECT);
		const Range o = owned(m);
		if ((rc = advect_range(m, CS(m, s), Range{ o.lo + (has_lower(m) ? Ha : 0), o.hi - (has_upper(m) ? Ha : 0) }, true))) return rc;
	}
	if ((rc = consume_record(ctx, M))) return rc;
	if (col_ready) FX_LANES(FX_HIP(hipStreamWaitEvent(L.lane->comm, L.lane->ev_col_done, 0)););
	const ExchSpec spec{ col_ready ? EX_ADVECT_VEL : EX_ADVECT_IN, Ha, 0 };
	if ((rc = do_exchange(ctx, M, &spec, 1, ON_COMM, s))) return rc;
	if ((rc = comm_mark_done(ctx, M, s))) return rc;
	if ((rc = comm_join(ctx, M, s))) return rc;
	for (fx_ctx* m : M) {
		ScopedMark mk(m, CS(m, s), MK_ADVECT);
		if (m->timing_on) m->acc.advect_halo_planes += (uint64_t)(m->adv_w_lo + m->adv_w_hi);
		const Range o = owned(m);
		if (has_lower(m) && (rc = advect_range(m, CS(m, s), Range{ o.lo, o.lo + Ha }, false))) return rc;
		if (has_upper(m) && (rc = advect_range(m, CS(m, s), Range{ o.hi - Ha, o.hi }, false))) return rc;
	}
	return FX_OK;
}

static float* alpha_mirror(const fx_ctx* ctx) { return ctx->accel_alpha_of == ctx->col[ctx->frame_parity] ? ctx->accel.alpha : nullptr; }

int confine_phase(fx_ctx* ctx, hipStream_t s)
{
	if (!(ctx->vort_eps > 0.0f) || !(ctx->time_step > 0.0f)) return FX_OK;
	DeviceGuard dg(ctx->device);
	ScopedMark mk(ctx, s, MK_ADVECT);
	FX_HIP(launch_confine_vorticity(ctx->g, ctx->half, ctx->vel[1], ctx->vel[0], ctx->vort_eps, ctx->time_step, s));
	std::swap(ctx->vel[0], ctx->vel[1]);
	return FX_OK;
}

int open_inflow_phase(fx_ctx* ctx, hipStream_t s)
{
	if (!ctx->open_faces || !(ctx->time_step > 0.0f)) return FX_OK;
	DeviceGuard dg(ctx->device);
	ScopedMark mk(ctx, s, MK_ADVECT);
	FX_HIP(launch_open_inflow(ctx->g, ctx->half, ctx->vel[0], ctx->col[ctx->frame_parity], alpha_mirror(ctx), ctx->open_faces, ctx->time_step, s));
	return FX_OK;
}

int emit_phase(fx_ctx* ctx, hipStream_t s)
{
	if (ctx->emitters.empty() || !(ctx->time_step > 0.0f)) return FX_OK;
	DeviceGuard dg(ctx->device);
	ScopedMark mk(ctx, s, MK_ADVECT);
	FX_HIP(launch_emit(ctx->g, ctx->half, ctx->vel[1], ctx->col[ctx->frame_parity], alpha_mirror(ctx), ctx->emitters.data(), (int)ctx->emitters.size(), ctx->time_step, s));
	return FX_OK;
}

int heat_phase(fx_ctx* ctx, hipStream_t s)
{
	if (!ctx->buoy_on || !ctx->temp[0] || !(ctx->time_step > 0.0f)) return FX_OK;
	DeviceGuard dg(ctx->device);
	ScopedMark mk(ctx, s, MK_ADVECT);
	const int cur = ctx->temp_cur;
	FX_HIP(launch_heat(ctx->g, ctx->half, ctx->buoy, ctx->heat_sources.data(), (int)ctx->heat_sources.size(), ctx->vel[0], ctx->vel[1],
		ctx->col[ctx->frame_parity], ctx->temp[cur], ctx->temp[1 - cur], ctx->obst_code, ctx->time_step, (int)ctx->desc.advect_address, s, ctx->open_faces));
	ctx->temp_cur = 1 - cur;
	return FX_OK;
}

int enforce_phase(fx_ctx* ctx, hipStream_t s)
{
	if (!ctx->obst_code || !ctx->obst_cells || !(ctx->time_step > 0.0f)) return FX_OK;
	DeviceGuard dg(ctx->device);
	ScopedMark mk(ctx, s, MK_ADVECT);
	FX_HIP(launch_obstacle_enforce(ctx->g, ctx->half, ctx->obst_code, ctx->obst_lo, ctx->obst_hi, ctx->vel[1], ctx->col[ctx->frame_parity], alpha_mirror(ctx), s));
	return FX_OK;
}

int divergence_phase(fx_ctx* ctx, hipStream_t s)
{
	DeviceGuard dg(ctx->device);
	ScopedMark mk(ctx, s, MK_DIV);
	const Range r = owned(ctx);
	if (ctx->obst_code) {
		FX_HIP(launch_divergence_obs(ctx->g, ctx->half, ctx->vel[1], ctx->obst_code, ctx->b, r.lo, r.hi, s));
		return FX_OK;
	}
	FX_HIP(launch_divergence(ctx->g, ctx->half, ctx->vel[1], ctx->b, r.lo, r.hi, s));
	return FX_OK;
}

static JacobiPolicy policy_of(const fx_ctx* c)
{
	return jacobi_policy(c->g, (int)(c->desc.flags & FX_FLAG_JACOBI_FUSE_MASK), c->frozen != nullptr, c->frozen_alt != nullptr);
}

static int jacobi_launch(fx_ctx* ctx, hipStream_t s, int src, JacobiLaunch l, Range r, ScopedMark* mk)
{
	r.lo = std::max(r.lo, 0); r.hi = std::min(r.hi, ctx->g.Zg);
	if (r.hi <= r.lo) return FX_OK;
	DeviceGuard dg(ctx->device);
	FX_HIP(launch_jacobi(ctx->g, l, ctx->p[src], ctx->b, ctx->p[src ^ 1], ctx->frozen, ctx->frozen ? ctx->frozen_alt : nullptr, r.lo, r.hi, s));
	if (l.family == JF_TILE2D && ctx->frozen) std::swap(ctx->frozen, ctx->frozen_alt);
	if (mk) { mk->launches += 1; mk->sweeps += l.sweeps; }
	return FX_OK;
}

static int jacobi_round(fx_ctx* ctx, hipStream_t s, int count, ScopedMark* mk)
{
	std::vector<JacobiLaunch> plan(count);
	plan.resize(jacobi_plan(policy_of(ctx), count, plan.data()));
	int left = count;
	for (const JacobiLaunch& l : plan) {
		const int t = l.sweeps;
		if (mk && mk->kind == MK_JACOBI && mk->launches && t * mk->launches < mk->sweeps) mk->split(MK_JACOBI_TAIL);
		left -= t;
		const int rc = jacobi_launch(ctx, s, ctx->p_cur, l, grown(ctx, multi_rank(ctx) ? left : 0), mk);
		if (rc) return rc;
		ctx->p_cur ^= 1;
	}
	return FX_OK;
}

static int clear_freeze_masks(std::vector<fx_ctx*>& M, hipStream_t s)
{
	for (fx_ctx* m : M)
		if (m->frozen) { DeviceGuard dg(m->device); if (hipMemsetAsync(m->frozen, 0, m->g.cells_local(), s) != hipSuccess) return FX_E_DEVICE; }
	return FX_OK;
// ... 290 lines not shown
```

fluidx12_amd/csrc/fx_sim.hip:

```cpp
#include "fx_internal.h"
#include <algorithm>
#include <cstdlib>
#include <cstdio>

namespace fx {

typedef _Float16 h16;
typedef _Float16 h16x4 __attribute__((ext_vector_type(4)));

struct __attribute__((packed, aligned(4))) F32Pair { float a, b; };
struct __attribute__((packed, aligned(2))) F16Pair { _Float16 a, b; };

template <bool HALF> struct Store;
template <> struct Store<false> {
	typedef float S;
	typedef float4 S4;
	static __device__ __forceinline__ void ld2(const S* p, size_t i, float& a, float& b)
	{
		const F32Pair v = *reinterpret_cast<const F32Pair*>(p + i);
		a = v.a; b = v.b;
	}
	static __device__ __forceinline__ float ld(const S* p, size_t i) { return p[i]; }
	static __device__ __forceinline__ float stored(float v) { return v; }
	static __device__ __forceinline__ void st(S* p, size_t i, float v) { p[i] = v; }
// ... 704 lines not shown
	if (__builtin_amdgcn_ballot_w64(lo > 0 || hi > 0) == 0) return;
#pragma unroll
	for (int o = 32; o > 0; o >>= 1) { lo = max(lo, __shfl_xor(lo, o)); hi = max(hi, __shfl_xor(hi, o)); }
	if ((threadIdx.x & 63) == 0) { if (lo > 0) atomicMax(rec, lo); if (hi > 0) atomicMax(rec + 1, hi); }
}

template <bool HALF>
__global__ __launch_bounds__(256) void k_copy_owned(const Geom g, const typename Store<HALF>::S* __restrict__ src,
	typename Store<HALF>::S* __restrict__ dst)
{
	const size_t n = g.cells_owned();
	const size_t off = (size_t)g.H * g.plane();
	for (size_t i = (size_t)blockIdx.x * blockDim.x + threadIdx.x; i < 3 * n; i += (size_t)gridDim.x * blockDim.x) {
		const size_t a = i / n, r = i - a * n;
		dst[a * g.cells_local() + off + r] = src[a * g.cells_local() + off + r];
	}
}

template <bool HALF>
__global__ __launch_bounds__(256) void k_to_storage(const float* __restrict__ src, typename Store<HALF>::S* __restrict__ dst, size_t n)
{
	for (size_t i = (size_t)blockIdx.x * blockDim.x + threadIdx.x; i < n; i += (size_t)gridDim.x * blockDim.x)
		Store<HALF>::st(dst, i, src[i]);
}
template <bool HALF>
__global__ __launch_bounds__(256) void k_from_storage(const typename Store<HALF>::S* __restrict__ src, float* __restrict__ dst, size_t n)
{
	for (size_t i = (size_t)blockIdx.x * blockDim.x + threadIdx.x; i < n; i += (size_t)gridDim.x * blockDim.x)
		dst[i] = Store<HALF>::ld(src, i);
}

static inline dim3 grid_xyz(const Geom& g, int nzp) { return dim3(((g.X + 63) / 64) * ((g.Y + 3) / 4) * nzp, 1, 1); }
static inline unsigned grid_1d(size_t n) { return (unsigned)((n + 255) / 256 < 4096 ? (n + 255) / 256 : 4096); }
enum { REMAP_JACOBI = 0, REMAP_ADVECT = 1, REMAP_DIV = 2, REMAP_PROJECT = 3 };
static int xcd_remap_on(int which)
{
	int mode[4] = { 1, 0, 0, 0 };
	const char* e = FX_KNOB("XCD_REMAP");
	int a, b_, c, d;
	if (e && sscanf(e, "%d,%d,%d,%d", &a, &b_, &c, &d) == 4) { mode[0] = a; mode[1] = b_; mode[2] = c; mode[3] = d; }
	return mode[which];
}

static int xcd_remap_for(int which, const Geom& g)
{
	const char* fe_ = FX_KNOB("XCD_REMAP");
	const bool forced = fe_ && *fe_;
	if (forced || which == REMAP_JACOBI) return xcd_remap_on(which);
	return g.Zg > 1 && g.plane() <= 32768 && g.cells_local() < (size_t)6 << 20 ? 1 : 0;
}

hipError_t launch_advect(const Geom& g, const SimParams& sp, int half_store, const void* vel_in, const void* col_in,
	void* vel_out, void* col_out, int z_begin, int z_end, unsigned* halo_overflow, hipStream_t s, uint32_t* far_scratch, size_t far_words, int far_parity, bool* far_used,
	AdvectAlpha* alpha)
{
	if (far_used) *far_used = false;
	if (alpha) alpha->written = false;
	if (z_end <= z_begin) return hipSuccess;
	int bx = 64, by = 4, bz = 1;
	if (const char* e = FX_KNOB("ADVECT_BLOCK")) {
		int a, b_, c;
		if (sscanf(e, "%d,%d,%d", &a, &b_, &c) == 3 && a > 0 && b_ > 0 && c > 0 && a * b_ * c <= 256) { bx = a; by = b_; bz = c; }
	}
	const int nzp = z_end - z_begin;
	{
		const char* le = FX_KNOB("ADVECT_LDS");
		if (!(le && le[0] == '0') && bx == 64 && by == 4 && bz == 1 && !xcd_remap_on(REMAP_ADVECT)) {
			const hipError_t e = launch_advect_lds(g, sp, half_store, vel_in, col_in, vel_out, col_out, z_begin, z_end, halo_overflow, far_scratch, far_words, far_parity, far_used, s, le && le[0] == '2', alpha);
			if (e != hipErrorNotSupported) return e;
		}
	}
	float* alpha_out = alpha && alpha->out && g.nzl() == g.Zg && z_begin == 0 && z_end == g.Zg ? alpha->out : nullptr;
	if (alpha_out) alpha->written = true;
	const char* fe = FX_KNOB("ADVECT_FAST");
	const bool fast_off = fe && fe[0] == '0';
	auto pow2 = [](int v) { return v > 0 && (v & (v - 1)) == 0; };
	if (!fast_off && pow2(g.X) && pow2(g.Y) && pow2(g.Zg) && g.X >= 2 && g.cells_local() * 16 < ((size_t)1 << 32) &&
		bx == 64 && by == 4 && bz == 1 && !xcd_remap_on(REMAP_ADVECT)) {
		const dim3 block(64, 4, 1), grid(((g.X + 63) / 64) * ((g.Y + 3) / 4) * nzp, 1, 1);
		const float rX = 1.0f / (float)g.X, rY = 1.0f / (float)g.Y, rZ = 1.0f / (float)g.Zg, inv_rr = sp.is3d ? 256.0f : 1024.0f;
		auto lg = [](int v) { int k = 0; while ((1 << k) < v) ++k; return k; };
		const int lgX = lg(g.X), lgY = lg(g.Y), lg_gx = lg((g.X + 63) / 64), lg_gy = lg((g.Y + 3) / 4);
		if (half_store)
			hipLaunchKernelGGL(k_advect_fast<true>, grid, block, 0, s, g, sp, (const h16*)vel_in, (const h16x4*)col_in,
				(h16*)vel_out, (h16x4*)col_out, z_begin, nzp, halo_overflow, rX, rY, rZ, inv_rr, lgX, lgY, lg_gx, lg_gy, alpha_out);
		else
			hipLaunchKernelGGL(k_advect_fast<false>, grid, block, 0, s, g, sp, (const float*)vel_in, (const float4*)col_in,
				(float*)vel_out, (float4*)col_out, z_begin, nzp, halo_overflow, rX, rY, rZ, inv_rr, lgX, lgY, lg_gx, lg_gy, alpha_out);
		return hipGetLastError();
	}
	const int cbz = g.Zg > 1 ? bz : 1;
	const dim3 block(bx, by, cbz), grid(((g.X + bx - 1) / bx) * ((g.Y + by - 1) / by) * ((nzp + cbz - 1) / cbz), 1, 1);
	if (half_store)
		hipLaunchKernelGGL(k_advect<true>, grid, block, 0, s, g, sp, (const h16*)vel_in, (const h16x4*)col_in,
			(h16*)vel_out, (h16x4*)col_out, z_begin, nzp, xcd_remap_for(REMAP_ADVECT, g), halo_overflow, alpha_out);
	else
		hipLaunchKernelGGL(k_advect<false>, grid, block, 0, s, g, sp, (const float*)vel_in, (const float4*)col_in,
			(float*)vel_out, (float4*)col_out, z_begin, nzp, xcd_remap_for(REMAP_ADVECT, g), halo_overflow, alpha_out);
	return hipGetLastError();
}

hipError_t launch_divergence(const Geom& g, int half_store, const void* vel, float* b, int z_begin, int z_end, hipStream_t s)
{
	if (z_end <= z_begin) return hipSuccess;
	const int w = sim_row_kernel(g, half_store, SIM_DIVERGENCE, g.Zg > 1);
	if (w == ROW_V4) {
		const int nzp = z_end - z_begin, X4 = g.X >> 2;
		const int bx = X4 < 64 ? X4 : 64;
		int by = 256 / bx; if (by > g.Y) by = g.Y;
		const dim3 block(bx, by, 1), grid(((X4 + bx - 1) / bx) * ((g.Y + by - 1) / by) * nzp, 1, 1);
		if (half_store) hipLaunchKernelGGL(k_divergence_v4<true>, grid, block, 0, s, g, (const h16*)vel, b, z_begin, nzp, xcd_remap_for(REMAP_DIV, g), by);
		else hipLaunchKernelGGL(k_divergence_v4<false>, grid, block, 0, s, g, (const float*)vel, b, z_begin, nzp, xcd_remap_for(REMAP_DIV, g), by);
		return hipGetLastError();
	}
	if (w != ROW_SCALAR) {
		const int nzp = z_end - z_begin, XW = g.X / w;
		const int bx = XW < 64 ? XW : 64;
		int by = 256 / bx; if (by > g.Y) by = g.Y;
		const dim3 block(bx, by, 1), grid(((XW + bx - 1) / bx) * ((g.Y + by - 1) / by) * nzp, 1, 1);
		if (half_store) hipLaunchKernelGGL((k_divergence_vw<2, true>), grid, block, 0, s, g, (const h16*)vel, b, z_begin, nzp, xcd_remap_for(REMAP_DIV, g), by);
		else if (w == 3) hipLaunchKernelGGL((k_divergence_vw<3, false>), grid, block, 0, s, g, (const float*)vel, b, z_begin, nzp, xcd_remap_for(REMAP_DIV, g), by);
// ... 165 lines not shown
```

fluidx12_amd/fluid.py:

```python
import ctypes as C
import os

import numpy as np

from . import capi


def look_at_lh(eye, focus, up):
    eye, focus, up = (np.asarray(v, np.float32) for v in (eye, focus, up))
    z = focus - eye
    z = z / np.float32(np.sqrt(np.dot(z, z)))
    x = np.cross(up, z).astype(np.float32)
    x = x / np.float32(np.sqrt(np.dot(x, x)))
    y = np.cross(z, x).astype(np.float32)
    m = np.zeros((4, 4), np.float32)
    m[:3, 0], m[:3, 1], m[:3, 2] = x, y, z
    m[3, :3] = [-np.dot(x, eye), -np.dot(y, eye), -np.dot(z, eye)]
    m[3, 3] = 1.0
    return m


def perspective_fov_lh(fovy, aspect, zn, zf):
    h = np.float32(np.cos(0.5 * fovy) / np.sin(0.5 * fovy))
    w = np.float32(h / np.float32(aspect))
# ... 144 lines not shown
                                                     capi.DEPTH_DEVICE), "SetSceneDepth")
            self._depth_ref = depth
            return
        a = np.ascontiguousarray(depth, np.float32)
        if a.shape != (h, w):
            raise ValueError("depth must be float32[%d][%d], got %s" % (h, w, a.shape))
        capi.check(self._lib.fx_set_scene_depth(self._ctx, stream, a.ctypes.data_as(C.c_void_p), w, h, float(z_near), float(z_far), 0),
                   "SetSceneDepth")
        self._depth_ref = None

    def SetLight(self, position, kind="directional", color=None, ambient=None):
        self._need()
        if position is None:
            capi.check(self._lib.fx_set_light(self._ctx, None), "SetLight")
            return
        l = capi.Light()
        capi.check(self._lib.fx_get_light(self._ctx, C.byref(l)), "SetLight")
        l.struct_size = C.sizeof(capi.Light)
        l.kind = {"directional": capi.LIGHT_DIRECTIONAL, "point": capi.LIGHT_POINT}[kind]
        l.position = (C.c_float * 3)(*[float(v) for v in position])
        if color is not None:
            l.color = (C.c_float * 4)(*[float(v) for v in color])
        if ambient is not None:
            l.ambient = (C.c_float * 4)(*[float(v) for v in ambient])
        capi.check(self._lib.fx_set_light(self._ctx, C.byref(l)), "SetLight")

    def GetLight(self):
        self._need()
        l = capi.Light()
        capi.check(self._lib.fx_get_light(self._ctx, C.byref(l)), "GetLight")
        return {"kind": "point" if l.kind == capi.LIGHT_POINT else "directional", "position": tuple(l.position), "color": tuple(l.color),
                "ambient": tuple(l.ambient)}

    def default_time_step(self):
        X, Y, Z = self.grid
        return (2.0 if Z > 1 else 1.0) / Y

    def Synchronize(self):
        self._need()
        rc = self._lib.fx_synchronize(self._ctx)
        if rc != capi.FX_OK:
            note = self.last_error
            capi.check(rc, "Synchronize" + (" [%s]" % note if note else ""))

    @property
    def last_error(self):
        self._need()
        e = self._lib.fx_last_error(self._ctx)
        return e.decode() if e else ""

    def Advect(self, stream=None):
        capi.check(self._lib.fx_advect(self._ctx, stream), "Advect")

    def SetVorticityConfinement(self, eps):
        self._need()
        capi.check(self._lib.fx_set_vorticity_confinement(self._ctx, float(eps)), "SetVorticityConfinement")

    def ConfineVorticity(self, stream=None):
        self._need()
        capi.check(self._lib.fx_confine_vorticity(self._ctx, stream), "ConfineVorticity")

    def SetEmitters(self, emitters):
        self._need()
        items = list(emitters or ())
        arr = (capi.Emitter * max(len(items), 1))()
        is3d = self.grid[2] > 1
        for k, e in enumerate(items):
            if isinstance(e, capi.Emitter):
                arr[k] = e
                continue
            arr[k].struct_size, arr[k].flags = C.sizeof(capi.Emitter), int(e.get("flags", 0))
            arr[k].center = (C.c_float * 3)(*[float(v) for v in e["center"]])
            arr[k].radius = float(e["radius"])
            arr[k].color_rate = (C.c_float * 4)(*[float(v) for v in e.get("color_rate", (8.0, 16.0, 40.0, 40.0))])
            arr[k].force = (C.c_float * 3)(*[float(v) for v in e.get("force", (0.0, 192.0 if is3d else 48.0, 0.0))])
            arr[k].swirl = float(e.get("swirl", 200.0))
        capi.check(self._lib.fx_set_emitters(self._ctx, arr if items else None, len(items)), "SetEmitters")

    def GetEmitters(self):
        self._need()
        n = C.c_uint32(0)
        arr = (capi.Emitter * capi.MAX_EMITTERS)()
        capi.check(self._lib.fx_get_emitters(self._ctx, arr, capi.MAX_EMITTERS, C.byref(n)), "GetEmitters")
        return [{"center": tuple(e.center), "radius": e.radius, "color_rate": tuple(e.color_rate), "force": tuple(e.force), "swirl": e.swirl,
                 "flags": e.flags} for e in arr[:n.value]]

    def SetImpulse(self, enabled):
        self._need()
        capi.check(self._lib.fx_set_impulse(self._ctx, 1 if enabled else 0), "SetImpulse")

    def Emit(self, stream=None):
        self._need()
        capi.check(self._lib.fx_emit(self._ctx, stream), "Emit")

    def SetObstacles(self, mask, stream=None):
        self._need()
        if mask is None:
            capi.check(self._lib.fx_set_obstacles(self._ctx, stream, None, 0, 0), "SetObstacles")
            return
        if hasattr(mask, "data_ptr") and getattr(mask, "is_cuda", False):
            import torch
            t = (mask != 0).to(dtype=torch.uint8).contiguous()
            torch.cuda.current_stream(t.device).synchronize()
            capi.check(self._lib.fx_set_obstacles(self._ctx, stream, t.data_ptr(), t.numel(), capi.OBSTACLES_DEVICE), "SetObstacles")
            return
        m = np.ascontiguousarray(np.asarray(mask) != 0, dtype=np.uint8)
# ... 232 lines not shown
```

include/fluidx_hip.h:

```cpp
#ifndef FLUIDX_HIP_H
#define FLUIDX_HIP_H

#include <stddef.h>
#include <stdint.h>

#ifdef __cplusplus
extern "C" {
#endif

#define FX_ABI_VERSION 7

enum fx_status {
	FX_OK = 0,
	FX_E_INVALID = -1,
	FX_E_DEVICE = -2,
	FX_E_NOMEM = -3,
	FX_E_STATE = -4,
	FX_E_COMM = -5,
	FX_E_HALO = -6
};

enum fx_render_flags {
	FX_RAY_MARCH_DIRECT = 0,
	FX_RAY_MARCH_CUBEMAP = 1,
// ... 60 lines not shown
	double   chain_ms;
	uint64_t freeze_solves, freeze_sweeps;
	uint64_t exchange_calls;
	uint64_t view_samples, light_samples, lightmap_fetches;
	uint64_t freeze_strip_launches;
} fx_timing;

int fx_abi_version(void);
const char* fx_error_string(int status);

int fx_create(fx_ctx** out, const fx_desc* desc);
int fx_destroy(fx_ctx* ctx);
int fx_set_max_samples(fx_ctx* ctx, uint32_t max_ray_samples, uint32_t max_light_samples);
int fx_set_sh(fx_ctx* ctx, const float* coeffs27);
int fx_update_frame(fx_ctx* ctx, float time_step, uint8_t frame_index,
	const float view[16], const float proj[16], const float eye[3]);
int fx_simulate(fx_ctx* ctx, void* stream, uint8_t frame_index);
int fx_render(fx_ctx* ctx, void* stream, uint8_t frame_index, uint8_t flags);
int fx_clear_render_target(fx_ctx* ctx, void* stream, const float rgba[4]);
int fx_render_cube(fx_ctx* ctx, void* stream, uint8_t frame_index);

#define FX_DEPTH_DEVICE 0x1u
int fx_set_scene_depth(fx_ctx* ctx, void* stream, const float* depth, uint32_t width, uint32_t height,
	float z_near, float z_far, uint32_t flags);

#define FX_LIGHT_DIRECTIONAL 0u
#define FX_LIGHT_POINT       1u
typedef struct fx_light {
	uint32_t struct_size, kind;
	float position[3];
	float color[4];
	float ambient[4];
} fx_light;
int fx_set_light(fx_ctx* ctx, const fx_light* light);
int fx_get_light(fx_ctx* ctx, fx_light* out);

int fx_set_environment(fx_ctx* ctx, const float* cube, uint32_t n);
int fx_render_environment(fx_ctx* ctx, void* stream, uint8_t frame_index);

int fx_get_frame_info(fx_ctx* ctx, fx_frame_info* out);

int fx_synchronize(fx_ctx* ctx);
const char* fx_last_error(fx_ctx* ctx);

int fx_upload(fx_ctx* ctx, int field, const void* host, size_t bytes);
int fx_download(fx_ctx* ctx, int field, void* host, size_t bytes);
size_t fx_field_bytes(fx_ctx* ctx, int field);
int fx_field_digest(fx_ctx* ctx, int field, uint32_t z_begin, uint32_t z_count, uint64_t out[2]);

int fx_checkpoint_save(fx_ctx* ctx, const char* path);
int fx_checkpoint_load(fx_ctx* ctx, const char* path);

int fx_advect(fx_ctx* ctx, void* stream);
int fx_divergence(fx_ctx* ctx, void* stream);
int fx_jacobi(fx_ctx* ctx, void* stream, uint32_t iters);
int fx_project(fx_ctx* ctx, void* stream);

int fx_set_vorticity_confinement(fx_ctx* ctx, float epsilon);
int fx_confine_vorticity(fx_ctx* ctx, void* stream);

#define FX_MAX_EMITTERS 16u
typedef struct fx_emitter {
	uint32_t struct_size, flags;
	float center[3];
	float radius;
	float color_rate[4];
	float force[3];
	float swirl;
} fx_emitter;
int fx_set_emitters(fx_ctx* ctx, const fx_emitter* list, uint32_t count);
int fx_get_emitters(fx_ctx* ctx, fx_emitter* out, uint32_t capacity, uint32_t* count);
int fx_set_impulse(fx_ctx* ctx, int enabled);
int fx_emit(fx_ctx* ctx, void* stream);

#define FX_OBSTACLES_DEVICE 0x1u
int fx_set_obstacles(fx_ctx* ctx, void* stream, const uint8_t* solid, size_t bytes, uint32_t flags);
int fx_get_obstacles(fx_ctx* ctx, uint8_t* solid_out, size_t bytes, uint64_t* solid_cells);
int fx_enforce_obstacles(fx_ctx* ctx, void* stream);

#define FX_WALL_X_LO 0x01u
#define FX_WALL_X_HI 0x02u
#define FX_WALL_Y_LO 0x04u
#define FX_WALL_Y_HI 0x08u
#define FX_WALL_Z_LO 0x10u
#define FX_WALL_Z_HI 0x20u
int fx_set_open_walls(fx_ctx* ctx, uint32_t faces);
int fx_get_open_walls(fx_ctx* ctx, uint32_t* faces);
int fx_open_inflow(fx_ctx* ctx, void* stream);

#define FX_MAX_HEAT_SOURCES 16u
typedef struct fx_buoyancy {
	uint32_t struct_size, flags;
	float ambient;
	float density_weight;
	float lift;
	float cooling;
	float up[3];
} fx_buoyancy;
typedef struct fx_heat_source {
	uint32_t struct_size, flags;
	float center[3];
	float radius;
	float rate;
} fx_heat_source;
int fx_set_buoyancy(fx_ctx* ctx, const fx_buoyancy* buoyancy);
int fx_get_buoyancy(fx_ctx* ctx, fx_buoyancy* out, int* enabled);
// ... 31 lines not shown
```

Before: 21.90 billion.

## Skip advection of provably empty colour boxes using per-box emptiness flags

Adds per-tile emptiness flags for the colour field, double-buffered across frames. The LDS advect kernel checks whether a tile's back-traced source region is entirely empty and, if so, takes a lean path (a new lean kernel) that skips staging and gathering colour. Flags are republished after each advect and cleared whenever emit, obstacle, inflow or upload modify colour. This aims to cut memory traffic for empty regions, at the cost of bookkeeping, extra atomics and the risk of stale flags producing wrong output.

```diff
diff --git a/fluidx12_amd/build.py b/fluidx12_amd/build.py
--- a/fluidx12_amd/build.py
+++ b/fluidx12_amd/build.py
@@ -9,8 +9,8 @@
 LIB = os.path.join(HERE, "libfluidx_hip.so")
 OBJDIR = os.path.join(HERE, "build")
 
-SOURCES = ["fx_api.cpp", "fx_knobs.cpp", "fx_context.cpp", "fx_schedule.cpp", "fx_jacobi_plan.cpp", "fx_emit_plan.cpp", "fx_heat_plan.cpp", "fx_comm.cpp", "fx_checkpoint.cpp", "fx_sim.hip", "fx_vorticity.hip", "fx_emit.hip", "fx_obstacle.hip", "fx_heat.hip", "fx_open.hip", "fx_advect_lds.hip", "fx_jacobi_strip.hip", "fx_jacobi_strip3.hip", "fx_jacobi_strip4.hip", "fx_jacobi_block.hip", "fx_jacobi_freeze.hip", "fx_jacobi_stripm.hip", "fx_jacobi2d.hip", "fx_render.hip", "fx_render_accel.hip", "fx_resolve.hip", "fx_bc6h.hip", "fx_sh.hip"]
-HEADERS = ["fx_internal.h", "fx_context.h", "fx_host.h", "fx_hostmath.h", "fx_pk.h", "fx_march.h", "fx_store.h", "fx_knobs.h", os.path.join(ROOT, "include", "fluidx_hip.h")]
+SOURCES = ["fx_api.cpp", "fx_knobs.cpp", "fx_context.cpp", "fx_schedule.cpp", "fx_jacobi_plan.cpp", "fx_emit_plan.cpp", "fx_heat_plan.cpp", "fx_comm.cpp", "fx_checkpoint.cpp", "fx_sim.hip", "fx_vorticity.hip", "fx_emit.hip", "fx_obstacle.hip", "fx_heat.hip", "fx_open.hip", "fx_advect_lds.hip", "fx_advect_lean.hip", "fx_jacobi_strip.hip", "fx_jacobi_strip3.hip", "fx_jacobi_strip4.hip", "fx_jacobi_block.hip", "fx_jacobi_freeze.hip", "fx_jacobi_stripm.hip", "fx_jacobi2d.hip", "fx_render.hip", "fx_render_accel.hip", "fx_resolve.hip", "fx_bc6h.hip", "fx_sh.hip"]
+HEADERS = ["fx_internal.h", "fx_advect_stage.h", "fx_context.h", "fx_host.h", "fx_hostmath.h", "fx_pk.h", "fx_march.h", "fx_store.h", "fx_knobs.h", os.path.join(ROOT, "include", "fluidx_hip.h")]
 
 FLAGS = ["--offload-arch=gfx950", "-O3", "-std=c++17", "-fPIC", "-ffp-contract=off", "-fno-fast-math",
          "-Wall", "-Wno-unused-function", "-D__HIP_PLATFORM_AMD__"]
diff --git a/fluidx12_amd/capi.py b/fluidx12_amd/capi.py
--- a/fluidx12_amd/capi.py
+++ b/fluidx12_amd/capi.py
@@ -92,6 +92,7 @@
     "fx_checkpoint_save": (C.c_int, [_vp, C.c_char_p]),
     "fx_checkpoint_load": (C.c_int, [_vp, C.c_char_p]),
     "fx_advect": (C.c_int, [_vp, _vp]),
+    "fx_get_lean_boxes": (C.c_int, [_vp, C.POINTER(C.c_uint32)]),
     "fx_divergence": (C.c_int, [_vp, _vp]),
     "fx_jacobi": (C.c_int, [_vp, _vp, C.c_uint32]),
     "fx_project": (C.c_int, [_vp, _vp]),
diff --git a/fluidx12_amd/csrc/fx_advect_lds.hip b/fluidx12_amd/csrc/fx_advect_lds.hip
--- a/fluidx12_amd/csrc/fx_advect_lds.hip
+++ b/fluidx12_amd/csrc/fx_advect_lds.hip
@@ -1,43 +1,13 @@
-#include "fx_internal.h"
+#include "fx_advect_stage.h"
 #include <algorithm>
 #include <cstdlib>
 #include <cstdio>
 
 namespace fx {
 
+using namespace advst;
+
 namespace {
-
-constexpr int TX = 64;
-constexpr int HX = TX + 2;
-constexpr int NSLOT = 4;
-template <bool HALF, int TY> struct Lay {
-	static constexpr int NCELL = HX * (TY + 2);
-	static constexpr int VEL_BYTES = NCELL * 4;
-	static constexpr int COL_BYTES = HALF ? 2 * NCELL * 4 : NCELL * 16;
-	static constexpr int SLOT_BYTES = COL_BYTES + 3 * VEL_BYTES;
-};
-typedef _Float16 h16;
-typedef _Float16 h16x4 __attribute__((ext_vector_type(4)));
-__device__ __forceinline__ h16 to_h16(float v) { asm("" : "+v"(v)); return (h16)v; }
-__device__ __forceinline__ float lo_half(uint32_t d) { return (float)__builtin_bit_cast(h16, (uint16_t)(d & 0xffffu)); }
-__device__ __forceinline__ float hi_half(uint32_t d) { return (float)__builtin_bit_cast(h16, (uint16_t)(d >> 16)); }
-
-__device__ __forceinline__ float lerpf(float a, float b, float f) { return fmaf(f, b - a, a); }
-__device__ __forceinline__ float saturatef(float x) { return fminf(fmaxf(x, 0.0f), 1.0f); }
-
-__device__ __forceinline__ int addr_tap(int i, int n, int mode)
-{
-	if (mode == FX_ADDRESS_MIRROR) {
-		const int period = 2 * n;
-		int m = i % period;
-		if (m < 0) m += period;
-		return m < n ? m : period - 1 - m;
-	}
-	return min(max(i, 0), n - 1);
-}
-
-typedef __attribute__((address_space(3))) void lds_void;
-typedef const __attribute__((address_space(1))) void glb_void;
 
 template <int VEL_BYTES>
 __device__ __forceinline__ void stage64(const void* col, const void* v0, const void* v1, const void* v2, uint32_t off_col, uint32_t off_vel, uint32_t lds_col, uint32_t lds_vel)
@@ -95,113 +65,25 @@
 		: "scc");
 }
 
-template <typename T>
-__device__ __forceinline__ T ldg32(const void* base, uint32_t byte_off)
-{
-	return *reinterpret_cast<const T*>(static_cast<const char*>(base) + byte_off);
-}
-
-
-template <bool P2> __device__ __forceinline__ uint32_t rows(uint32_t y, int lgX, const Geom& g) { return P2 ? y << lgX : y * (uint32_t)g.X; }
-template <bool P2> __device__ __forceinline__ uint32_t planes(uint32_t z, int lgP, const Geom& g) { return P2 ? z << lgP : z * ((uint32_t)g.X * (uint32_t)g.Y); }
-
-template <bool HALF, bool P2>
-__device__ __forceinline__ void advect_gather(const Geom& g, const SimParams& sp, int ix, int iy, int z0, int z1, bool z_present, float fx, float fy, float fz,
-	const char* v0, const char* v1, const char* v2, const void* __restrict__ col_in, int lgX, int lgP, unsigned* halo_overflow, float (&u)[3], float (&c)[4])
-{
-	const int xa0 = addr_tap(ix, g.X, sp.address), xa1 = addr_tap(ix + 1, g.X, sp.address);
-	const int ya0 = addr_tap(iy, g.Y, sp.address), ya1 = addr_tap(iy + 1, g.Y, sp.address);
-	if (!z_present) {
-		atomicOr(halo_overflow, 1u);
-		z0 = min(max(z0, g.zlo), g.zhi);
-		z1 = min(max(z1, g.zlo), g.zhi);
-	}
-	const uint32_t p0 = planes<P2>((uint32_t)g.lz(z0), lgP, g), p1 = planes<P2>((uint32_t)g.lz(z1), lgP, g);
-	const uint32_t ry0 = rows<P2>((uint32_t)ya0, lgX, g), ry1 = rows<P2>((uint32_t)ya1, lgX, g);
-	const uint32_t c000 = p0 + ry0 + (uint32_t)xa0, c100 = p0 + ry0 + (uint32_t)xa1;
-	const uint32_t c010 = p0 + ry1 + (uint32_t)xa0, c110 = p0 + ry1 + (uint32_t)xa1;
-	const uint32_t c001 = p1 + ry0 + (uint32_t)xa0, c101 = p1 + ry0 + (uint32_t)xa1;
-	const uint32_t c011 = p1 + ry1 + (uint32_t)xa0, c111 = p1 + ry1 + (uint32_t)xa1;
-	const char* vb[3] = { v0, v1, v2 };
-	auto gv = [](const char* b, uint32_t cell) -> float { return HALF ? (float)ldg32<h16>(b, cell * 2u) : ldg32<float>(b, cell * 4u); };
-	auto gc = [&](uint32_t cell) -> float4 {
-		if (HALF) { const h16x4 h = ldg32<h16x4>(col_in, cell * 8u); return make_float4((float)h.x, (float)h.y, (float)h.z, (float)h.w); }
-		return ldg32<float4>(col_in, cell * 16u);
-	};
-#pragma unroll
-	for (int a = 0; a < 3; ++a) {
-		const float c00 = lerpf(gv(vb[a], c000), gv(vb[a], c100), fx);
-		const float c10 = lerpf(gv(vb[a], c010), gv(vb[a], c110), fx);
-		const float c01 = lerpf(gv(vb[a], c001), gv(vb[a], c101), fx);
-		const float c11 = lerpf(gv(vb[a], c011), gv(vb[a], c111), fx);
-		u[a] = lerpf(lerpf(c00, c10, fy), lerpf(c01, c11, fy), fz);
-	}
-	const float4 t000 = gc(c000), t100 = gc(c100), t010 = gc(c010), t110 = gc(c110);
-	const float4 t001 = gc(c001), t101 = gc(c101), t011 = gc(c011), t111 = gc(c111);
-#define FX_TRI(m) lerpf(lerpf(lerpf(t000.m, t100.m, fx), lerpf(t010.m, t110.m, fx), fy), \
-	lerpf(lerpf(t001.m, t101.m, fx), lerpf(t011.m, t111.m, fx), fy), fz)
-	c[0] = FX_TRI(x); c[1] = FX_TRI(y); c[2] = FX_TRI(z); c[3] = FX_TRI(w);
-#undef FX_TRI
-}
-
-template <bool HALF, bool ALPHA>
-__device__ __forceinline__ void advect_finish(const SimParams& sp, float (&u)[3], float (&c)[4], float ex, float dx, float dz, float dt, float atten,
-	uint32_t id, uint32_t stride, void* __restrict__ vel_out, void* __restrict__ col_out, float* __restrict__ alpha_out)
-{
-	if (__builtin_amdgcn_ballot_w64(sp.impulse && ex > -6.5f) != 0) {
-		const float basis = exp2f(ex);
-		if (basis >= 0.0183156393f) {
-			float Fx, Fy, Fz;
-			if (sp.is3d) {
-				Fx = fmaf(basis, 0.0f, dz * -200.0f);
-				Fy = fmaf(basis, 192.0f, 0.0f);
-				Fz = fmaf(basis, 0.0f, dx * 200.0f);
-			} else {
-				Fx = 0.0f; Fy = basis * 48.0f; Fz = 0.0f;
-			}
-			u[0] = fmaf(Fx, dt, u[0]); u[1] = fmaf(Fy, dt, u[1]); u[2] = fmaf(Fz, dt, u[2]);
-			const float bdt = basis * dt;
-			c[0] = saturatef(fmaf(bdt, 8.0f, c[0]));
-			c[1] = saturatef(fmaf(bdt, 16.0f, c[1]));
-			c[2] = saturatef(fmaf(bdt, 40.0f, c[2]));
-			c[3] = saturatef(fmaf(bdt, 40.0f, c[3]));
-		}
-	}
-	char* vo = static_cast<char*>(vel_out);
-	char* co = static_cast<char*>(col_out);
-	if (HALF) {
-		*reinterpret_cast<h16*>(vo + id * 2u) = to_h16(u[0] * atten);
-		*reinterpret_cast<h16*>(vo + (stride + id) * 2u) = to_h16(u[1] * atten);
-		*reinterpret_cast<h16*>(vo + (2u * stride + id) * 2u) = to_h16(u[2] * atten);
-		h16x4 hc;
-		hc.x = to_h16(c[0] * atten); hc.y = to_h16(c[1] * atten); hc.z = to_h16(c[2] * atten); hc.w = to_h16(c[3] * atten);
-		*reinterpret_cast<h16x4*>(co + id * 8u) = hc;
-		if (ALPHA) *reinterpret_cast<float*>(reinterpret_cast<char*>(alpha_out) + id * 4u) = (float)hc.w;
-	} else {
-		*reinterpret_cast<float*>(vo + id * 4u) = u[0] * atten;
-		*reinterpret_cast<float*>(vo + (stride + id) * 4u) = u[1] * atten;
-		*reinterpret_cast<float*>(vo + (2u * stride + id) * 4u) = u[2] * atten;
-		*reinterpret_cast<float4*>(co + id * 16u) = make_float4(c[0] * atten, c[1] * atten, c[2] * atten, c[3] * atten);
-		if (ALPHA) *reinterpret_cast<float*>(reinterpret_cast<char*>(alpha_out) + id * 4u) = c[3] * atten;
-	}
-}
-
-}
-
-template <bool HALF, int TY, bool DEFER, bool P2, bool ALPHA>
+}
+
+template <bool HALF, int TY, bool DEFER, bool P2, bool ALPHA, bool FLAGS = false>
 __global__ __launch_bounds__(64 * TY) __attribute__((amdgpu_waves_per_eu(4, 4))) void k_advect_lds(const Geom g, const SimParams sp,
 	const void* __restrict__ vel_in, const void* __restrict__ col_in, void* __restrict__ vel_out, void* __restrict__ col_out, float* __restrict__ alpha_out,
 	int z_begin, int nzp, int zchunk, int nchunks, unsigned* halo_overflow, float rX, float rY, float rZ, float inv_rr,
-	int lgX, int lgY, int lg_gx, int lg_gy, uint32_t* __restrict__ far_list, uint32_t* __restrict__ far_flat, uint32_t* __restrict__ far_total, uint32_t far_cap)
-{
-	__shared__ uint32_t far_n, far_base;
+	int lgX, int lgY, int lg_gx, int lg_gy, uint32_t* __restrict__ far_list, uint32_t* __restrict__ far_flat, uint32_t* __restrict__ far_total, uint32_t far_cap,
+	const uint8_t* __restrict__ flags_src, uint8_t* __restrict__ flags_dst)
+{
+	static_assert(!FLAGS || (DEFER && P2 && TY == 8), "the emptiness flags belong to the default path");
+	__shared__ uint32_t far_n, far_base, nz_word;
 	extern __shared__ __attribute__((aligned(16))) char lds[];
 
 	const int tid = (int)threadIdx.x, lane = tid & 63, wave = __builtin_amdgcn_readfirstlane(tid >> 6);
 	const int ntx = P2 ? 1 << lg_gx : lg_gx, nty = P2 ? 1 << lg_gy : lg_gy;
 	const int ntiles = ntx * nty * nchunks;
 	int tl = (int)blockIdx.x;
-	{
+	if (FLAGS) tl = advect_flag_box(tl, ntiles, lg_gx, lg_gy);
+	else {
 		const int q = ntiles >> 3, r = ntiles & 7, xcd = tl & 7, j = tl >> 3;
 		tl = xcd * q + min(xcd, r) + j;
 	}
@@ -209,6 +91,8 @@
 	const int x0t = tx << 6, y0t = ty * TY;
 	const int zb = z_begin + chunk * zchunk, ze = min(zb + zchunk, z_begin + nzp);
 	if (zb >= ze) return;
+	if (FLAGS && advect_box_lean(flags_src, tx, ty, chunk, ntx, nty, nchunks, lane, sp, x0t, x0t + TX - 1, y0t, y0t + TY - 1, zb, ze - 1, rX, rY, rZ, inv_rr))
+		return;
 
 	const int lgP = lgX + lgY;
 	constexpr int COL_BYTES = Lay<HALF, TY>::COL_BYTES, SLOT_BYTES = Lay<HALF, TY>::SLOT_BYTES;
@@ -249,6 +133,7 @@
 	};
 
 	if (DEFER && tid == 0) far_n = 0u;
+	if (FLAGS && tid == 0) nz_word = 0u;
 	fill(zb - 1);
 	fill(zb);
 	fill(zb + 1);
@@ -265,8 +150,8 @@
 	const uint32_t own = (uint32_t)((wave + 1) * HX + lane + 1);
 	const float atten = fmaxf(fmaf(-dt, 0.200000003f, 1.0f), 0.0f);
 
-	auto compute = [&](int z) {
-		if (!has_voxel) return;
+	auto compute = [&](int z) -> uint32_t {
+		if (!has_voxel) return 0u;
 		const float pz = P2 ? ((float)z + 0.5f) * rZ : ((float)z + 0.5f) / (float)g.Zg;
 		const float dz = pz + -0.5f;
 		const float d2 = fmaf(dz, dz, dxy2);
@@ -330,12 +215,15 @@
 		}
 
 		const uint32_t id = planes<P2>((uint32_t)g.lz(z), lgP, g) + rows<P2>((uint32_t)y, lgX, g) + (uint32_t)x;
-		advect_finish<HALF, ALPHA>(sp, u, c, ex, dx, dz, dt, atten, id, stride, vel_out, col_out, alpha_out);
+		const uint32_t bits = advect_finish<HALF, ALPHA>(sp, u, c, ex, dx, dz, dt, atten, id, stride, vel_out, col_out, alpha_out);
+		return FLAGS && inwin ? bits : 0u;
 	};
 
+	uint32_t nz_all = 0u, nz_first = 0u, nz_last = 0u;
 	for (int z = zb; z < ze; ++z) {
 		if (z + 2 <= ze) fill(z + 2);
-		compute(z);
+		const uint32_t bits = compute(z);
+		if (FLAGS) { nz_all |= bits; if (z == zb) nz_first = bits; nz_last = bits; }
 		if (!(P2 || y < g.Y)) asm volatile("s_waitcnt vmcnt(0)" ::: "memory");
 		else if (ALPHA) asm volatile("s_waitcnt vmcnt(5)" ::: "memory");
 		else asm volatile("s_waitcnt vmcnt(4)" ::: "memory");
@@ -351,16 +239,18 @@
 			for (uint32_t i = (uint32_t)tid; i < n; i += (uint32_t)NT) far_flat[base + i] = seg[i];
 		}
 	}
-}
-
-template <bool HALF, bool P2, bool ALPHA>
+	if (FLAGS) advect_box_publish(flags_dst, tl, nz_all, nz_first, nz_last, tid, wave, TY, &nz_word);
+}
+
+template <bool HALF, bool P2, bool ALPHA, bool FLAGS = false>
 __global__ __launch_bounds__(256) void k_advect_far(const Geom g, const SimParams sp,
 	const void* __restrict__ vel_in, const void* __restrict__ col_in, void* __restrict__ vel_out, void* __restrict__ col_out, float* __restrict__ alpha_out,
 	const uint32_t* __restrict__ far_flat, const uint32_t* __restrict__ far_total, uint32_t* __restrict__ far_total_next, unsigned* halo_overflow,
-	float rX, float rY, float rZ, float inv_rr, int lgX, int lgY)
+	float rX, float rY, float rZ, float inv_rr, int lgX, int lgY, uint8_t* __restrict__ flags_dst, uint32_t* __restrict__ lean_count_next, int zchunk, int lg_gx, int lg_gy)
 {
 	const uint32_t n = *far_total;
 	if (blockIdx.x == 0 && threadIdx.x == 0) *far_total_next = 0u;
+	if (FLAGS && blockIdx.x == 0 && threadIdx.x == 0) *lean_count_next = 0u;
 	const int lgP = lgX + lgY;
 	constexpr uint32_t ES = HALF ? 2 : 4;
 	const uint32_t stride = planes<P2>((uint32_t)g.nzl(), lgP, g);
@@ -393,17 +283,22 @@
 		const bool z_present = z0 >= g.zlo && z0 <= g.zhi && z1 >= g.zlo && z1 <= g.zhi;
 		float u[3], c[4];
 		advect_gather<HALF, P2>(g, sp, ix, iy, z0, z1, z_present, fx, fy, fz, v0, v1, v2, col_in, lgX, lgP, halo_overflow, u, c);
-		advect_finish<HALF, ALPHA>(sp, u, c, ex, dx, dz, dt, atten, id, stride, vel_out, col_out, alpha_out);
+		const uint32_t bits = advect_finish<HALF, ALPHA>(sp, u, c, ex, dx, dz, dt, atten, id, stride, vel_out, col_out, alpha_out);
+		if (FLAGS && bits != 0u) {
+			const int ch = z / zchunk, zb = ch * zchunk;
+			advect_box_taint(flags_dst, (x >> 6) | (y >> 3) << lg_gx | ch << (lg_gx + lg_gy), x, y, z, zb, min(zb + zchunk, g.Zg));
+		}
 	}
 }
 
 
 hipError_t launch_advect_lds(const Geom& g, const SimParams& sp, int half_store, const void* vel_in, const void* col_in,
 	void* vel_out, void* col_out, int z_begin, int z_end, unsigned* halo_overflow, uint32_t* far_scratch, size_t far_words, int far_parity, bool* far_used, hipStream_t s, bool force,
-	AdvectAlpha* alpha)
+	AdvectAlpha* alpha, AdvectLean* lean)
 {
 	if (far_used) *far_used = false;
 	if (alpha) alpha->written = false;
+	if (lean) lean->used = false;
 	auto pow2 = [](int v) { return v > 0 && (v & (v - 1)) == 0; };
 	const int nzp = z_end - z_begin;
 	const bool p2 = pow2(g.X) && pow2(g.Y) && pow2(g.Zg);
@@ -436,15 +331,37 @@
 	uint32_t* far_total_next = far_scratch ? far_scratch + ((far_parity & 1) ^ 1) : nullptr;
 	uint32_t* far_flat = far_scratch ? far_scratch + 2 : nullptr;
 	uint32_t* far_list = far_scratch ? far_scratch + 2 + flat_words : nullptr;
-#define FX_ADV(H_, TY_, D_, P_, A_) do { \
+#define FX_ADVF(H_, TY_, D_, P_, A_, F_) do { \
 		static bool attr_set = false; \
-		if (!attr_set) { (void)hipFuncSetAttribute(reinterpret_cast<const void*>(k_advect_lds<H_, TY_, D_, P_, A_>), hipFuncAttributeMaxDynamicSharedMemorySize, NSLOT * Lay<H_, TY_>::SLOT_BYTES); attr_set = true; } \
-		hipLaunchKernelGGL((k_advect_lds<H_, TY_, D_, P_, A_>), dim3(tiles_xy * nchunks), dim3(64 * TY_), (NSLOT * Lay<H_, TY_>::SLOT_BYTES), s, g, sp, vel_in, col_in, vel_out, col_out, alpha_out, \
-			z_begin, nzp, zchunk, nchunks, halo_overflow, rX, rY, rZ, inv_rr, lgX, lgY, lg_gx, lg_gy, far_list, far_flat, far_total, far_cap); } while (0)
-#define FX_FAR(H_, P_, A_) hipLaunchKernelGGL((k_advect_far<H_, P_, A_>), dim3(far_wgs), dim3(256), 0, s, g, sp, vel_in, col_in, vel_out, col_out, alpha_out, far_flat, far_total, far_total_next, halo_overflow, rX, rY, rZ, inv_rr, lgX, lgY)
+		if (!attr_set) { (void)hipFuncSetAttribute(reinterpret_cast<const void*>(k_advect_lds<H_, TY_, D_, P_, A_, F_>), hipFuncAttributeMaxDynamicSharedMemorySize, NSLOT * Lay<H_, TY_>::SLOT_BYTES); attr_set = true; } \
+		hipLaunchKernelGGL((k_advect_lds<H_, TY_, D_, P_, A_, F_>), dim3(tiles_xy * nchunks), dim3(64 * TY_), (NSLOT * Lay<H_, TY_>::SLOT_BYTES), s, g, sp, vel_in, col_in, vel_out, col_out, alpha_out, \
+			z_begin, nzp, zchunk, nchunks, halo_overflow, rX, rY, rZ, inv_rr, lgX, lgY, lg_gx, lg_gy, far_list, far_flat, far_total, far_cap, flags_src, flags_dst); } while (0)
+#define FX_ADV(H_, TY_, D_, P_, A_) FX_ADVF(H_, TY_, D_, P_, A_, false)
+#define FX_FARF(H_, P_, A_, F_) hipLaunchKernelGGL((k_advect_far<H_, P_, A_, F_>), dim3(far_wgs), dim3(256), 0, s, g, sp, vel_in, col_in, vel_out, col_out, alpha_out, far_flat, far_total, far_total_next, halo_overflow, rX, rY, rZ, inv_rr, lgX, lgY, \
+		flags_dst, lean_count_next, zchunk, lg_gx, lg_gy)
+#define FX_FAR(H_, P_, A_) FX_FARF(H_, P_, A_, false)
 	const int far_wgs = 1024;
 	float* alpha_out = alpha && alpha->out && defer && TY == 8 && g.nzl() == g.Zg && z_begin == 0 && z_end == g.Zg ? alpha->out : nullptr;
-	if (alpha_out) {
+	const bool flags_on = lean && lean->src && lean->dst && lean->count && defer && p2 && TY == 8 && g.nzl() == g.Zg && z_begin == 0 && z_end == g.Zg &&
+		zchunk == std::min(32, nzp) && (size_t)nwg == lean->boxes && lean->boxes == advect_flag_boxes(g);
+	const uint8_t* flags_src = flags_on ? lean->src : nullptr;
+	uint8_t* flags_dst = flags_on ? lean->dst : nullptr;
+	uint32_t* lean_count_next = flags_on ? lean->count_next : nullptr;
+	if (flags_on) {
+		const LeanLaunch ll{ g, sp, vel_in, vel_out, col_out, alpha_out, nzp, zchunk, nchunks, rX, rY, rZ, inv_rr, lgX, lgY, lg_gx, lg_gy, far_list, far_flat, far_total, far_cap,
+			flags_src, flags_dst, lean->count };
+		hipError_t e = hipSuccess;
+		if (half_store) {
+			if (alpha_out) { FX_ADVF(true, 8, true, true, true, true); e = launch_advect_lean(ll, 1, s); FX_FARF(true, true, true, true); }
+			else { FX_ADVF(true, 8, true, true, false, true); e = launch_advect_lean(ll, 1, s); FX_FARF(true, true, false, true); }
+		} else {
+			if (alpha_out) { FX_ADVF(false, 8, true, true, true, true); e = launch_advect_lean(ll, 0, s); FX_FARF(false, true, true, true); }
+			else { FX_ADVF(false, 8, true, true, false, true); e = launch_advect_lean(ll, 0, s); FX_FARF(false, true, false, true); }
+		}
+		if (e != hipSuccess) return e;
+		if (alpha_out) alpha->written = true;
+		lean->used = true;
+	} else if (alpha_out) {
 		if (half_store) { if (p2) { FX_ADV(true, 8, true, true, true); FX_FAR(true, true, true); } else { FX_ADV(true, 8, true, false, true); FX_FAR(true, false, true); } }
 		else { if (p2) { FX_ADV(false, 8, true, true, true); FX_FAR(false, true, true); } else { FX_ADV(false, 8, true, false, true); FX_FAR(false, false, true); } }
 		alpha->written = true;
@@ -461,7 +378,9 @@
 		else { if (half_store) FX_ADV(true, 8, false, true, false); else FX_ADV(false, 8, false, true, false); }
 	}
 #undef FX_FAR
+#undef FX_FARF
 #undef FX_ADV
+#undef FX_ADVF
 	return hipGetLastError();
 }
 
@@ -472,4 +391,12 @@
 	return 2 + (size_t)g.X * g.Y * (size_t)nzp + tiled * (size_t)(nzp + 32);
 }
 
-}
+size_t advect_flag_boxes(const Geom& g)
+{
+	auto pow2 = [](int v) { return v > 0 && (v & (v - 1)) == 0; };
+	if (!whole_grid(g) || !pow2(g.X) || !pow2(g.Y) || !pow2(g.Zg) || advect_far_words(g, g.Zg) == 0) return 0;
+	const int zchunk = std::min(32, g.Zg);
+	return (size_t)(g.X / TX) * (size_t)(g.Y / 8) * (size_t)((g.Zg + zchunk - 1) / zchunk);
+}
+
+}
diff --git a/fluidx12_amd/csrc/fx_advect_lean.hip b/fluidx12_amd/csrc/fx_advect_lean.hip
--- /dev/null
+++ b/fluidx12_amd/csrc/fx_advect_lean.hip
@@ -0,0 +1,169 @@
+#include "fx_advect_stage.h"
+#include <type_traits>
+
+namespace fx {
+
+using namespace advst;
+
+namespace {
+constexpr int TY = 8;
+constexpr int NCELL = Lay<false, TY>::NCELL, VEL_BYTES = Lay<false, TY>::VEL_BYTES, NT = 64 * TY;
+constexpr int SLOT_BYTES = 3 * VEL_BYTES;
+}
+
+template <bool HALF, bool ALPHA>
+__global__ __launch_bounds__(64 * TY) void k_advect_lean(const LeanLaunch a)
+{
+	__shared__ uint32_t far_n, far_base, nz_word;
+	extern __shared__ __attribute__((aligned(16))) char lds[];
+
+	const Geom& g = a.g;
+	const SimParams& sp = a.sp;
+	const int tid = (int)threadIdx.x, lane = tid & 63, wave = __builtin_amdgcn_readfirstlane(tid >> 6);
+	const int ntx = 1 << a.lg_gx, nty = 1 << a.lg_gy;
+	const int ntiles = ntx * nty * a.nchunks;
+	const int tl = advect_flag_box((int)blockIdx.x, ntiles, a.lg_gx, a.lg_gy);
+	const int tx = tl & (ntx - 1), ty = (tl >> a.lg_gx) & (nty - 1), chunk = tl >> (a.lg_gx + a.lg_gy);
+	const int x0t = tx << 6, y0t = ty * TY;
+	const int zb = chunk * a.zchunk, ze = min(zb + a.zchunk, a.nzp);
+	if (zb >= ze) return;
+	if (!advect_box_lean(a.flags_src, tx, ty, chunk, ntx, nty, a.nchunks, lane, sp, x0t, x0t + TX - 1, y0t, y0t + TY - 1, zb, ze - 1, a.rX, a.rY, a.rZ, a.inv_rr))
+		return;
+	const bool store_colour = !(__builtin_amdgcn_readfirstlane((int)a.flags_dst[tl]) & 1);
+
+	const int lgX = a.lgX, lgP = a.lgX + a.lgY;
+	constexpr uint32_t ES = HALF ? 2 : 4;
+	const uint32_t stride = (uint32_t)g.nzl() << lgP;
+	const char* v0 = reinterpret_cast<const char*>(a.vel_in);
+	const char* v1 = v0 + (size_t)stride * ES;
+	const char* v2 = v1 + (size_t)stride * ES;
+
+	uint32_t src_a, src_b = 0;
+	{
+		const int c = tid, r = c / HX, cc = c - r * HX;
+		src_a = ((uint32_t)addr_tap(y0t - 1 + r, g.Y, sp.address) << lgX) + (uint32_t)addr_tap(x0t - 1 + cc, g.X, sp.address);
+	}
+	const bool has_b = NT + tid < NCELL;
+	if (has_b) {
+		const int c = NT + tid, r = c / HX, cc = c - r * HX;
+		src_b = ((uint32_t)addr_tap(y0t - 1 + r, g.Y, sp.address) << lgX) + (uint32_t)addr_tap(x0t - 1 + cc, g.X, sp.address);
+	}
+	const bool wave_has_b = NT + wave * 64 < NCELL;
+
+	const uint32_t lds0 = (uint32_t)(size_t)(__attribute__((address_space(3))) char*)lds;
+	auto fill = [&](int zq) {
+		const int za = min(max(addr_tap(zq, g.Zg, sp.address), g.zlo), g.zhi);
+		const size_t pz = (size_t)g.lz(za) << lgP;
+		const uint32_t slot = __builtin_amdgcn_readfirstlane(lds0 + (uint32_t)(((zq + 4) & 3) * SLOT_BYTES));
+		const char *b0 = v0 + pz * ES, *b1 = v1 + pz * ES, *b2 = v2 + pz * ES;
+		stage64v<HALF, VEL_BYTES>(b0, b1, b2, src_a * ES, slot + (uint32_t)wave * (64 * 4));
+		if (wave_has_b) {
+			if (has_b) stage64v<HALF, VEL_BYTES>(b0, b1, b2, src_b * ES, slot + (NT + (uint32_t)wave * 64) * 4);
+		}
+	};
+
+	if (tid == 0) { far_n = 0u; nz_word = 0u; atomicAdd(a.count, 1u); }
+	fill(zb - 1);
+	fill(zb);
+	fill(zb + 1);
+	asm volatile("s_waitcnt vmcnt(0)" ::: "memory");
+	__syncthreads();
+
+	const int x = x0t + lane, y = y0t + wave;
+	const float dt = sp.dt;
+	const float px = ((float)x + 0.5f) * a.rX;
+	const float py = ((float)y + 0.5f) * a.rY;
+	const float dx = px + -0.5f, dy = py + -0.100000001f;
+	const float dxy2 = fmaf(dy, dy, dx * dx);
+	const uint32_t own = (uint32_t)((wave + 1) * HX + lane + 1);
+	const float atten = fmaxf(fmaf(-dt, 0.200000003f, 1.0f), 0.0f);
+
+	auto compute = [&](int z, auto store_tag) -> uint32_t {
+		constexpr bool STORE = decltype(store_tag)::value;
+		const float pz = ((float)z + 0.5f) * a.rZ;
+		const float dz = pz + -0.5f;
+		const float d2 = fmaf(dz, dz, dxy2);
+		const float ex = ((d2 * -4.0f) * a.inv_rr) * 1.44269502f;
+
+		const uint32_t* vs = reinterpret_cast<const uint32_t*>(lds + ((z + 4) & 3) * SLOT_BYTES);
+		auto vval = [](uint32_t d) -> float { return HALF ? lo_half(d) : __uint_as_float(d); };
+		const float u0x = vval(vs[own]), u0y = vval(vs[NCELL + own]), u0z = vval(vs[2 * NCELL + own]);
+		const float ax = fmaf(-u0x, dt, px), ay = fmaf(-u0y, dt, py), az = fmaf(-u0z, dt, pz);
+		const float tx_ = ax * (float)g.X - 0.5f, ty_ = ay * (float)g.Y - 0.5f, tz_ = az * (float)g.Zg - 0.5f;
+		const float flx = floorf(tx_), fly = floorf(ty_), flz = floorf(tz_);
+		const float fx = tx_ - flx, fy = ty_ - fly, fz = tz_ - flz;
+		const int ix = (int)flx, iy = (int)fly, iz = (int)flz;
+		const int jx = ix - x, jy = iy - y, jz = iz - z;
+		const int z0 = addr_tap(iz, g.Zg, sp.address), z1 = addr_tap(iz + 1, g.Zg, sp.address);
+		const bool z_present = z0 >= g.zlo && z0 <= g.zhi && z1 >= g.zlo && z1 <= g.zhi;
+		const bool inwin = (unsigned)(jx + 1) <= 1u && (unsigned)(jy + 1) <= 1u && (unsigned)(jz + 1) <= 1u && z_present;
+		const float lx = lerpf(0.0f, 0.0f, fx), ly = lerpf(lx, lx, fy), lz = lerpf(ly, ly, fz);
+		const bool aside = !inwin || __float_as_uint(lz) != 0u;
+
+		if (aside) {
+			const uint32_t slot = atomicAdd(&far_n, 1u);
+			a.far_list[(size_t)blockIdx.x * a.far_cap + slot] = (uint32_t)x | (uint32_t)y << lgX | (uint32_t)z << lgP;
+		}
+		float u[3], c[4];
+		const int kx = !inwin ? 0 : jx, ky = !inwin ? 0 : jy, kz = !inwin ? z : iz;
+		const uint32_t c0 = (uint32_t)((int)own + ky * HX + kx);
+		const char* s0 = lds + ((kz + 4) & 3) * SLOT_BYTES;
+		const char* s1 = lds + ((kz + 5) & 3) * SLOT_BYTES;
+#pragma unroll
+		for (int k = 0; k < 3; ++k) {
+			const uint32_t* p0 = reinterpret_cast<const uint32_t*>(s0 + k * VEL_BYTES) + c0;
+			const uint32_t* p1 = reinterpret_cast<const uint32_t*>(s1 + k * VEL_BYTES) + c0;
+			const float c00 = lerpf(vval(p0[0]), vval(p0[1]), fx);
+			const float c10 = lerpf(vval(p0[HX]), vval(p0[HX + 1]), fx);
+			const float c01 = lerpf(vval(p1[0]), vval(p1[1]), fx);
+			const float c11 = lerpf(vval(p1[HX]), vval(p1[HX + 1]), fx);
+			u[k] = lerpf(lerpf(c00, c10, fy), lerpf(c01, c11, fy), fz);
+		}
+		c[0] = lz; c[1] = lz; c[2] = lz; c[3] = lz;
+
+		const uint32_t id = ((uint32_t)g.lz(z) << lgP) + ((uint32_t)y << lgX) + (uint32_t)x;
+		const uint32_t bits = advect_finish<HALF, ALPHA, STORE>(sp, u, c, ex, dx, dz, dt, atten, id, stride, a.vel_out, a.col_out, a.alpha_out);
+		return aside ? 0u : bits;
+	};
+
+	uint32_t nz_all = 0u, nz_first = 0u, nz_last = 0u;
+	auto run = [&](auto store_tag) {
+		constexpr bool STORE = decltype(store_tag)::value;
+		for (int z = zb; z < ze; ++z) {
+			if (z + 2 <= ze) fill(z + 2);
+			const uint32_t bits = compute(z, store_tag);
+			nz_all |= bits; if (z == zb) nz_first = bits; nz_last = bits;
+			if (STORE && ALPHA) asm volatile("s_waitcnt vmcnt(5)" ::: "memory");
+			else if (STORE || ALPHA) asm volatile("s_waitcnt vmcnt(4)" ::: "memory");
+			else asm volatile("s_waitcnt vmcnt(3)" ::: "memory");
+			__syncthreads();
+		}
+	};
+	if (store_colour) run(std::true_type{}); else run(std::false_type{});
+	{
+		const uint32_t n = far_n;
+		if (n != 0u) {
+			if (tid == 0) far_base = atomicAdd(a.far_total, n);
+			__syncthreads();
+			const uint32_t base = far_base;
+			const uint32_t* seg = a.far_list + (size_t)blockIdx.x * a.far_cap;
+			for (uint32_t i = (uint32_t)tid; i < n; i += (uint32_t)NT) a.far_flat[base + i] = seg[i];
+		}
+	}
+	advect_box_publish(a.flags_dst, tl, nz_all, nz_first, nz_last, tid, wave, TY, &nz_word);
+}
+
+hipError_t launch_advect_lean(const LeanLaunch& l, int half_store, hipStream_t s)
+{
+	const dim3 grid((1u << (l.lg_gx + l.lg_gy)) * (unsigned)l.nchunks), block(64 * TY);
+	if (half_store) {
+		if (l.alpha_out) hipLaunchKernelGGL((k_advect_lean<true, true>), grid, block, NSLOT * SLOT_BYTES, s, l);
+		else hipLaunchKernelGGL((k_advect_lean<true, false>), grid, block, NSLOT * SLOT_BYTES, s, l);
+	} else {
+		if (l.alpha_out) hipLaunchKernelGGL((k_advect_lean<false, true>), grid, block, NSLOT * SLOT_BYTES, s, l);
+		else hipLaunchKernelGGL((k_advect_lean<false, false>), grid, block, NSLOT * SLOT_BYTES, s, l);
+	}
+	return hipGetLastError();
+}
+
+}
diff --git a/fluidx12_amd/csrc/fx_advect_stage.h b/fluidx12_amd/csrc/fx_advect_stage.h
--- /dev/null
+++ b/fluidx12_amd/csrc/fx_advect_stage.h
@@ -0,0 +1,242 @@
+#pragma once
+#include "fx_internal.h"
+
+namespace fx {
+namespace advst {
+
+constexpr int TX = 64;
+constexpr int HX = TX + 2;
+constexpr int NSLOT = 4;
+template <bool HALF, int TY> struct Lay {
+	static constexpr int NCELL = HX * (TY + 2);
+	static constexpr int VEL_BYTES = NCELL * 4;
+	static constexpr int COL_BYTES = HALF ? 2 * NCELL * 4 : NCELL * 16;
+	static constexpr int SLOT_BYTES = COL_BYTES + 3 * VEL_BYTES;
+};
+typedef _Float16 h16;
+typedef _Float16 h16x4 __attribute__((ext_vector_type(4)));
+__device__ __forceinline__ h16 to_h16(float v) { asm("" : "+v"(v)); return (h16)v; }
+__device__ __forceinline__ float lo_half(uint32_t d) { return (float)__builtin_bit_cast(h16, (uint16_t)(d & 0xffffu)); }
+__device__ __forceinline__ float hi_half(uint32_t d) { return (float)__builtin_bit_cast(h16, (uint16_t)(d >> 16)); }
+
+__device__ __forceinline__ float lerpf(float a, float b, float f) { return fmaf(f, b - a, a); }
+__device__ __forceinline__ float saturatef(float x) { return fminf(fmaxf(x, 0.0f), 1.0f); }
+
+__device__ __forceinline__ int addr_tap(int i, int n, int mode)
+{
+	if (mode == FX_ADDRESS_MIRROR) {
+		const int period = 2 * n;
+		int m = i % period;
+		if (m < 0) m += period;
+		return m < n ? m : period - 1 - m;
+	}
+	return min(max(i, 0), n - 1);
+}
+
+template <bool HALF, int VEL_BYTES>
+__device__ __forceinline__ void stage64v(const void* v0, const void* v1, const void* v2, uint32_t off_vel, uint32_t lds_vel)
+{
+	uint32_t keep;
+	lds_vel = __builtin_amdgcn_readfirstlane(lds_vel);
+	if (HALF)
+		asm volatile(
+			"s_mov_b32 %0, m0\n\t"
+			"s_mov_b32 m0, %5\n\t"
+			"s_nop 0\n\t"
+			"global_load_lds_ushort %4, %1\n\t"
+			"s_add_u32 m0, m0, %6\n\t"
+			"s_nop 0\n\t"
+			"global_load_lds_ushort %4, %2\n\t"
+			"s_add_u32 m0, m0, %6\n\t"
+			"s_nop 0\n\t"
+			"global_load_lds_ushort %4, %3\n\t"
+			"s_mov_b32 m0, %0"
+			: "=&s"(keep)
+			: "s"(v0), "s"(v1), "s"(v2), "v"(off_vel), "s"(lds_vel), "n"(VEL_BYTES)
+			: "scc");
+	else
+		asm volatile(
+			"s_mov_b32 %0, m0\n\t"
+			"s_mov_b32 m0, %5\n\t"
+			"s_nop 0\n\t"
+			"global_load_lds_dword %4, %1\n\t"
+			"s_add_u32 m0, m0, %6\n\t"
+			"s_nop 0\n\t"
+			"global_load_lds_dword %4, %2\n\t"
+			"s_add_u32 m0, m0, %6\n\t"
+			"s_nop 0\n\t"
+			"global_load_lds_dword %4, %3\n\t"
+			"s_mov_b32 m0, %0"
+			: "=&s"(keep)
+			: "s"(v0), "s"(v1), "s"(v2), "v"(off_vel), "s"(lds_vel), "n"(VEL_BYTES)
+			: "scc");
+}
+
+template <typename T>
+__device__ __forceinline__ T ldg32(const void* base, uint32_t byte_off)
+{
+	return *reinterpret_cast<const T*>(static_cast<const char*>(base) + byte_off);
+}
+
+
+template <bool P2> __device__ __forceinline__ uint32_t rows(uint32_t y, int lgX, const Geom& g) { return P2 ? y << lgX : y * (uint32_t)g.X; }
+template <bool P2> __device__ __forceinline__ uint32_t planes(uint32_t z, int lgP, const Geom& g) { return P2 ? z << lgP : z * ((uint32_t)g.X * (uint32_t)g.Y); }
+
+template <bool HALF, bool P2>
+__device__ __forceinline__ void advect_gather(const Geom& g, const SimParams& sp, int ix, int iy, int z0, int z1, bool z_present, float fx, float fy, float fz,
+	const char* v0, const char* v1, const char* v2, const void* __restrict__ col_in, int lgX, int lgP, unsigned* halo_overflow, float (&u)[3], float (&c)[4])
+{
+	const int xa0 = addr_tap(ix, g.X, sp.address), xa1 = addr_tap(ix + 1, g.X, sp.address);
+	const int ya0 = addr_tap(iy, g.Y, sp.address), ya1 = addr_tap(iy + 1, g.Y, sp.address);
+	if (!z_present) {
+		atomicOr(halo_overflow, 1u);
+		z0 = min(max(z0, g.zlo), g.zhi);
+		z1 = min(max(z1, g.zlo), g.zhi);
+	}
+	const uint32_t p0 = planes<P2>((uint32_t)g.lz(z0), lgP, g), p1 = planes<P2>((uint32_t)g.lz(z1), lgP, g);
+	const uint32_t ry0 = rows<P2>((uint32_t)ya0, lgX, g), ry1 = rows<P2>((uint32_t)ya1, lgX, g);
+	const uint32_t c000 = p0 + ry0 + (uint32_t)xa0, c100 = p0 + ry0 + (uint32_t)xa1;
+	const uint32_t c010 = p0 + ry1 + (uint32_t)xa0, c110 = p0 + ry1 + (uint32_t)xa1;
+	const uint32_t c001 = p1 + ry0 + (uint32_t)xa0, c101 = p1 + ry0 + (uint32_t)xa1;
+	const uint32_t c011 = p1 + ry1 + (uint32_t)xa0, c111 = p1 + ry1 + (uint32_t)xa1;
+	const char* vb[3] = { v0, v1, v2 };
+	auto gv = [](const char* b, uint32_t cell) -> float { return HALF ? (float)ldg32<h16>(b, cell * 2u) : ldg32<float>(b, cell * 4u); };
+	auto gc = [&](uint32_t cell) -> float4 {
+		if (HALF) { const h16x4 h = ldg32<h16x4>(col_in, cell * 8u); return make_float4((float)h.x, (float)h.y, (float)h.z, (float)h.w); }
+		return ldg32<float4>(col_in, cell * 16u);
+	};
+#pragma unroll
+	for (int a = 0; a < 3; ++a) {
+		const float c00 = lerpf(gv(vb[a], c000), gv(vb[a], c100), fx);
+		const float c10 = lerpf(gv(vb[a], c010), gv(vb[a], c110), fx);
+		const float c01 = lerpf(gv(vb[a], c001), gv(vb[a], c101), fx);
+		const float c11 = lerpf(gv(vb[a], c011), gv(vb[a], c111), fx);
+		u[a] = lerpf(lerpf(c00, c10, fy), lerpf(c01, c11, fy), fz);
+	}
+	const float4 t000 = gc(c000), t100 = gc(c100), t010 = gc(c010), t110 = gc(c110);
+	const float4 t001 = gc(c001), t101 = gc(c101), t011 = gc(c011), t111 = gc(c111);
+#define FX_TRI(m) lerpf(lerpf(lerpf(t000.m, t100.m, fx), lerpf(t010.m, t110.m, fx), fy), \
+	lerpf(lerpf(t001.m, t101.m, fx), lerpf(t011.m, t111.m, fx), fy), fz)
+	c[0] = FX_TRI(x); c[1] = FX_TRI(y); c[2] = FX_TRI(z); c[3] = FX_TRI(w);
+#undef FX_TRI
+}
+
+template <bool HALF, bool ALPHA, bool COLOUR = true>
+__device__ __forceinline__ uint32_t advect_finish(const SimParams& sp, float (&u)[3], float (&c)[4], float ex, float dx, float dz, float dt, float atten,
+	uint32_t id, uint32_t stride, void* __restrict__ vel_out, void* __restrict__ col_out, float* __restrict__ alpha_out)
+{
+	if (__builtin_amdgcn_ballot_w64(sp.impulse && ex > -6.5f) != 0) {
+		const float basis = exp2f(ex);
+		if (basis >= 0.0183156393f) {
+			float Fx, Fy, Fz;
+			if (sp.is3d) {
+				Fx = fmaf(basis, 0.0f, dz * -200.0f);
+				Fy = fmaf(basis, 192.0f, 0.0f);
+				Fz = fmaf(basis, 0.0f, dx * 200.0f);
+			} else {
+				Fx = 0.0f; Fy = basis * 48.0f; Fz = 0.0f;
+			}
+			u[0] = fmaf(Fx, dt, u[0]); u[1] = fmaf(Fy, dt, u[1]); u[2] = fmaf(Fz, dt, u[2]);
+			const float bdt = basis * dt;
+			c[0] = saturatef(fmaf(bdt, 8.0f, c[0]));
+			c[1] = saturatef(fmaf(bdt, 16.0f, c[1]));
+			c[2] = saturatef(fmaf(bdt, 40.0f, c[2]));
+			c[3] = saturatef(fmaf(bdt, 40.0f, c[3]));
+		}
+	}
+	char* vo = static_cast<char*>(vel_out);
+	char* co = static_cast<char*>(col_out);
+	if (HALF) {
+		*reinterpret_cast<h16*>(vo + id * 2u) = to_h16(u[0] * atten);
+		*reinterpret_cast<h16*>(vo + (stride + id) * 2u) = to_h16(u[1] * atten);
+		*reinterpret_cast<h16*>(vo + (2u * stride + id) * 2u) = to_h16(u[2] * atten);
+		h16x4 hc;
+		hc.x = to_h16(c[0] * atten); hc.y = to_h16(c[1] * atten); hc.z = to_h16(c[2] * atten); hc.w = to_h16(c[3] * atten);
+		const uint2 hb = __builtin_bit_cast(uint2, hc);
+		if (COLOUR) *reinterpret_cast<h16x4*>(co + id * 8u) = hc;
+		if (ALPHA) *reinterpret_cast<float*>(reinterpret_cast<char*>(alpha_out) + id * 4u) = (float)hc.w;
+		return hb.x | hb.y;
+	} else {
+		*reinterpret_cast<float*>(vo + id * 4u) = u[0] * atten;
+		*reinterpret_cast<float*>(vo + (stride + id) * 4u) = u[1] * atten;
+		*reinterpret_cast<float*>(vo + (2u * stride + id) * 4u) = u[2] * atten;
+		const float4 t = make_float4(c[0] * atten, c[1] * atten, c[2] * atten, c[3] * atten);
+		const uint32_t bits = __float_as_uint(t.x) | __float_as_uint(t.y) | __float_as_uint(t.z) | __float_as_uint(t.w);
+		if (COLOUR) *reinterpret_cast<float4*>(co + id * 16u) = t;
+		if (ALPHA) *reinterpret_cast<float*>(reinterpret_cast<char*>(alpha_out) + id * 4u) = t.w;
+		return bits;
+	}
+}
+
+__device__ __forceinline__ int advect_flag_box(int wg, int ntiles, int lg_gx, int lg_gy)
+{
+	const int xcd = wg & 7, j = wg >> 3;
+	if (lg_gy < 4) {
+		const int q = ntiles >> 3, r = ntiles & 7;
+		return xcd * q + min(xcd, r) + j;
+	}
+	const int lg_brick = lg_gx + 1, lg_groups = lg_gy - 4;
+	const int slot = j >> lg_brick, within = j & ((1 << lg_brick) - 1);
+	const int c = slot >> lg_groups, m = slot & ((1 << lg_groups) - 1);
+	const int band = ((xcd - 3 * c) & 7) + 8 * m;
+	return (((c << lg_gy) + 2 * band) << lg_gx) + within;
+}
+
+constexpr uint32_t kBoxEmpty = 0x7Fu;
+
+__device__ __forceinline__ bool advect_box_lean(const uint8_t* __restrict__ flags, int tx, int ty, int ch, int ntx, int nty, int nch, int lane,
+	const SimParams& sp, int x0, int x1, int y0, int y1, int z0, int z1, float rX, float rY, float rZ, float inv_rr)
+{
+	bool ok = true;
+	if (lane < 27) {
+		const int ox = lane % 3 - 1, oy = (lane / 3) % 3 - 1, oz = lane / 9 - 1;
+		const int nx = min(max(tx + ox, 0), ntx - 1), ny = min(max(ty + oy, 0), nty - 1), nz = min(max(ch + oz, 0), nch - 1);
+		const int ex = nx - tx, ey = ny - ty, ez = nz - ch;
+		uint32_t need = 0u;
+		if (ex > 0) need |= 1u << 1; if (ex < 0) need |= 1u << 2;
+		if (ey > 0) need |= 1u << 3; if (ey < 0) need |= 1u << 4;
+		if (ez > 0) need |= 1u << 5; if (ez < 0) need |= 1u << 6;
+		if (!need) need = 1u;
+		ok = ((uint32_t)flags[(nz * nty + ny) * ntx + nx] & need) != 0u;
+	}
+	if (__builtin_amdgcn_ballot_w64(!ok) != 0) return false;
+	if (!sp.impulse) return true;
+	const float pxa = ((float)x0 + 0.5f) * rX, pxb = ((float)x1 + 0.5f) * rX;
+	const float pya = ((float)y0 + 0.5f) * rY, pyb = ((float)y1 + 0.5f) * rY;
+	const float pza = ((float)z0 + 0.5f) * rZ, pzb = ((float)z1 + 0.5f) * rZ;
+	const float dx = fminf(fmaxf(0.5f, pxa), pxb) + -0.5f, dy = fminf(fmaxf(0.100000001f, pya), pyb) + -0.100000001f, dz = fminf(fmaxf(0.5f, pza), pzb) + -0.5f;
+	const float d2 = fmaf(dz, dz, fmaf(dy, dy, dx * dx));
+	return ((d2 * -4.0f) * inv_rr) * 1.44269502f <= -6.5f;
+}
+
+__device__ __forceinline__ void advect_box_publish(uint8_t* __restrict__ flags, int box, uint32_t all, uint32_t first, uint32_t last,
+	int tid, int wave, int nwaves, uint32_t* nz_word)
+{
+	uint32_t nz = 0u;
+	const unsigned long long any = __builtin_amdgcn_ballot_w64(all != 0u);
+	if (any) {
+		nz = 1u;
+		if (any & 1ull) nz |= 1u << 1;
+		if (any >> 63) nz |= 1u << 2;
+		if (wave == 0) nz |= 1u << 3;
+		if (wave == nwaves - 1) nz |= 1u << 4;
+		if (__builtin_amdgcn_ballot_w64(first != 0u)) nz |= 1u << 5;
+		if (__builtin_amdgcn_ballot_w64(last != 0u)) nz |= 1u << 6;
+		if ((tid & 63) == 0) atomicOr(nz_word, nz);
+	}
+	__syncthreads();
+	if (tid == 0) flags[box] = (uint8_t)(~*nz_word & kBoxEmpty);
+}
+
+__device__ __forceinline__ void advect_box_taint(uint8_t* __restrict__ flags, int box, int x, int y, int z, int zb, int ze)
+{
+	uint32_t clr = 1u;
+	if ((x & 63) == 0) clr |= 1u << 1; if ((x & 63) == 63) clr |= 1u << 2;
+	if ((y & 7) == 0) clr |= 1u << 3; if ((y & 7) == 7) clr |= 1u << 4;
+	if (z == zb) clr |= 1u << 5; if (z == ze - 1) clr |= 1u << 6;
+	if (((uint32_t)flags[box] & clr) == 0u) return;
+	atomicAnd(reinterpret_cast<uint32_t*>(flags + (box & ~3)), ~(clr << (8 * (box & 3))));
+}
+
+}
+}
diff --git a/fluidx12_amd/csrc/fx_api.cpp b/fluidx12_amd/csrc/fx_api.cpp
--- a/fluidx12_amd/csrc/fx_api.cpp
+++ b/fluidx12_amd/csrc/fx_api.cpp
@@ -371,6 +371,18 @@
 	hipStream_t s = pick_stream(ctx, stream);
 	ScopedMark mk(ctx, s, MK_ADVECT);
 	return advect_range(ctx, s, owned(ctx), false);
+}
+
+int fx_get_lean_boxes(fx_ctx* ctx, uint32_t* boxes)
+{
+	if (!ctx || !boxes) return FX_E_INVALID;
+	if (ctx->desc.flags & FX_FLAG_RENDER_ONLY) return FX_E_STATE;
+	*boxes = 0u;
+	if (ctx->lean_count_last < 0 || !ctx->lean_count) return FX_OK;
+	DeviceGuard dg(ctx->device);
+	FX_HIP(hipDeviceSynchronize());
+	FX_HIP(hipMemcpy(boxes, ctx->lean_count + ctx->lean_count_last, sizeof(uint32_t), hipMemcpyDeviceToHost));
+	return FX_OK;
 }
 
 static int sim_guard(const fx_ctx* ctx, bool whole = true)
@@ -810,6 +822,10 @@
 	ScopedMark mk(ctx, s, MK_EXCH);
 	int rc = ctx->group->transport->gather(ctx->group, parts, root, streams);
 	if (rc) return rc;
+	if (am_root && full->col_flags[full->frame_parity]) {
+		DeviceGuard dgf(full->device);
+		FX_HIP(colour_flags_forget(full->col_flags[full->frame_parity], full->col_flag_boxes, &full->col_flags_live[full->frame_parity], full->stream));
+	}
 	if (am_root && full->stream != done_on) {
 		fx_lane& L = ctx->group->per_member ? ctx->group->lanes[(size_t)root] : ctx->group->lanes[0];
 		DeviceGuard dgr(L.device);
diff --git a/fluidx12_amd/csrc/fx_context.cpp b/fluidx12_amd/csrc/fx_context.cpp
--- a/fluidx12_amd/csrc/fx_context.cpp
+++ b/fluidx12_amd/csrc/fx_context.cpp
@@ -88,10 +88,11 @@
 	for (int i = 0; i < 2; ++i) {
 		if (c->vel[i]) (void)hipFree(c->vel[i]);
 		if (c->col[i]) (void)hipFree(c->col[i]);
+		if (c->col_flags[i]) (void)hipFree(c->col_flags[i]);
 		if (c->p[i]) (void)hipFree(c->p[i]);
 	}
 	void* others[] = { c->env, c->cube_depth, c->depth_own, c->accel.occ, c->accel.alpha, c->accel.bits, c->accel.list, c->accel.cells, c->accel.gi, c->accel.ctr, c->target, c->target_float, c->p_face[0], c->p_face[1], c->b, c->frozen, c->frozen_alt, c->lightmap, c->cube, c->sh_dev, c->halo_overflow, c->stage,
-		c->sh_scratch[0], c->sh_scratch[1], c->sh_scratch[2], c->sh_scratch[3], c->p_aux, c->fz_mask[0], c->fz_mask[1], c->fz_mask[2], c->fz_tile_next, c->fz_stat, c->fz_list[0], c->fz_list[1], c->fz_counts, c->sample_counters, c->adv_far, c->obst_code, c->obst_spare, c->obst_stats, c->temp[0], c->temp[1] };
+		c->sh_scratch[0], c->sh_scratch[1], c->sh_scratch[2], c->sh_scratch[3], c->p_aux, c->fz_mask[0], c->fz_mask[1], c->fz_mask[2], c->fz_tile_next, c->fz_stat, c->fz_list[0], c->fz_list[1], c->fz_counts, c->sample_counters, c->adv_far, c->lean_count, c->obst_code, c->obst_spare, c->obst_stats, c->temp[0], c->temp[1] };
 	for (void* q : others) if (q) (void)hipFree(q);
 	for (hipEvent_t e : c->ev) (void)hipEventDestroy(e);
 	if (c->step_rec) (void)hipFree(c->step_rec);
@@ -227,6 +228,22 @@
 					FX_HIP(hipMemsetAsync(ctx->adv_far, 0, 2 * sizeof(uint32_t), ctx->stream));
 					ctx->adv_far_words = words;
 				} else { (void)hipGetLastError(); ctx->adv_far = nullptr; }
+			}
+			const size_t boxes = ctx->adv_far ? advect_flag_boxes(ctx->g) : 0;
+			if (boxes) {
+				const size_t padded = (boxes + 3) & ~(size_t)3;
+				if (hipMalloc((void**)&ctx->col_flags[0], padded) == hipSuccess && hipMalloc((void**)&ctx->col_flags[1], padded) == hipSuccess &&
+					hipMalloc((void**)&ctx->lean_count, 2 * sizeof(uint32_t)) == hipSuccess) {
+					for (int i = 0; i < 2; ++i) FX_HIP(hipMemsetAsync(ctx->col_flags[i], 0x7F, padded, ctx->stream));
+					FX_HIP(hipMemsetAsync(ctx->lean_count, 0, 2 * sizeof(uint32_t), ctx->stream));
+					ctx->col_flag_boxes = boxes;
+					ctx->col_flags_live[0] = ctx->col_flags_live[1] = true;
+				} else {
+					(void)hipGetLastError();
+					for (int i = 0; i < 2; ++i) { if (ctx->col_flags[i]) (void)hipFree(ctx->col_flags[i]); ctx->col_flags[i] = nullptr; }
+					if (ctx->lean_count) (void)hipFree(ctx->lean_count);
+					ctx->lean_count = nullptr;
+				}
 			}
 		}
 		if (d->grid_z > 1) {
@@ -460,6 +477,10 @@
 		}
 		char* dst = (char*)ctx->col[field == FX_FIELD_COLOR ? ctx->frame_parity : 1 - ctx->frame_parity];
 		if (ctx->accel_alpha_of == dst) ctx->accel_alpha_of = nullptr;
+		{
+			const int buf = field == FX_FIELD_COLOR ? ctx->frame_parity : 1 - ctx->frame_parity;
+			FX_HIP(colour_flags_forget(ctx->col_flags[buf], ctx->col_flag_boxes, &ctx->col_flags_live[buf], ctx->stream));
+		}
 		if ((rc = ensure_stage(ctx, need))) return rc;
 		FX_HIP(hipMemcpy(ctx->stage, host, need, hipMemcpyHostToDevice));
 		FX_HIP(launch_to_storage(ctx->stage, dst + off * 4 * es, 4 * n, ctx->half, ctx->stream));
diff --git a/fluidx12_amd/csrc/fx_context.h b/fluidx12_amd/csrc/fx_context.h
--- a/fluidx12_amd/csrc/fx_context.h
+++ b/fluidx12_amd/csrc/fx_context.h
@@ -40,6 +40,11 @@
 	bool adv_far_tried = false;
 	size_t adv_far_words = 0;
 	uint32_t adv_far_turn = 0;
+	uint8_t* col_flags[2] = { nullptr, nullptr };
+	size_t col_flag_boxes = 0;
+	bool col_flags_live[2] = { false, false };
+	uint32_t* lean_count = nullptr;
+	int lean_count_last = -1;
 	uint32_t fz_gen = 0;
 	uint32_t fz_gen_mark = 0;
 	std::vector<uint32_t> fz_iters;
diff --git a/fluidx12_amd/csrc/fx_internal.h b/fluidx12_amd/csrc/fx_internal.h
--- a/fluidx12_amd/csrc/fx_internal.h
+++ b/fluidx12_amd/csrc/fx_internal.h
@@ -51,12 +51,26 @@
 };
 
 struct AdvectAlpha { float* out; bool written; };
+struct AdvectLean { const uint8_t* src; uint8_t* dst; uint32_t* count; uint32_t* count_next; size_t boxes; bool used; };
+size_t advect_flag_boxes(const Geom& g);
+inline hipError_t colour_flags_forget(uint8_t* flags, size_t boxes, bool* live, hipStream_t s)
+{
+	if (!flags || !*live) return hipSuccess;
+	*live = false;
+	return hipMemsetAsync(flags, 0, (boxes + 3) & ~(size_t)3, s);
+}
 hipError_t launch_advect(const Geom& g, const SimParams& sp, int half_store, const void* vel_in, const void* col_in,
 	void* vel_out, void* col_out, int z_begin, int z_end, unsigned* halo_overflow, hipStream_t s, uint32_t* far_scratch = nullptr, size_t far_words = 0, int far_parity = 0, bool* far_used = nullptr,
-	AdvectAlpha* alpha = nullptr);
+	AdvectAlpha* alpha = nullptr, AdvectLean* lean = nullptr);
 hipError_t launch_advect_lds(const Geom& g, const SimParams& sp, int half_store, const void* vel_in, const void* col_in,
 	void* vel_out, void* col_out, int z_begin, int z_end, unsigned* halo_overflow, uint32_t* far_scratch, size_t far_words, int far_parity, bool* far_used, hipStream_t s, bool force,
-	AdvectAlpha* alpha = nullptr);
+	AdvectAlpha* alpha = nullptr, AdvectLean* lean = nullptr);
+struct LeanLaunch {
+	Geom g; SimParams sp; const void* vel_in; void* vel_out; void* col_out; float* alpha_out; int nzp, zchunk, nchunks; float rX, rY, rZ, inv_rr;
+	int lgX, lgY, lg_gx, lg_gy; uint32_t* far_list; uint32_t* far_flat; uint32_t* far_total; uint32_t far_cap;
+	const uint8_t* flags_src; uint8_t* flags_dst; uint32_t* count;
+};
+hipError_t launch_advect_lean(const LeanLaunch& l, int half_store, hipStream_t s);
 size_t advect_far_words(const Geom& g, int nzp);
 hipError_t launch_confine_vorticity(const Geom& g, int half_store, const void* vel_in, void* vel_out, float eps, float dt, hipStream_t s);
 const int kEmitTileX = 64, kEmitTileY = 4;
diff --git a/fluidx12_amd/csrc/fx_schedule.cpp b/fluidx12_amd/csrc/fx_schedule.cpp
--- a/fluidx12_amd/csrc/fx_schedule.cpp
+++ b/fluidx12_amd/csrc/fx_schedule.cpp
@@ -97,8 +97,14 @@
 	ctx->rendered_since_step = false;
 	AdvectAlpha aa{ frame_was_rendered && ctx->accel_ok && ctx->opt_render_accel && FX_KNOB_INT("ADVECT_ALPHA", 1) ? ctx->accel.alpha : nullptr, false };
 	if (ctx->accel_alpha_of == ctx->col[par]) ctx->accel_alpha_of = nullptr;
+	const int turn = (int)(ctx->adv_far_turn & 1u);
+	AdvectLean lean{ ctx->col_flags[1 - par], ctx->col_flags[par], ctx->lean_count ? ctx->lean_count + turn : nullptr,
+		ctx->lean_count ? ctx->lean_count + (turn ^ 1) : nullptr, ctx->col_flag_boxes, false };
 	FX_HIP(launch_advect(g, sp, ctx->half, ctx->vel[0], ctx->col[1 - par], ctx->vel[1], ctx->col[par],
-		r.lo, r.hi, ctx->halo_overflow, s, lend ? ctx->adv_far : nullptr, lend ? ctx->adv_far_words : 0, (int)(ctx->adv_far_turn & 1u), &far_used, &aa));
+		r.lo, r.hi, ctx->halo_overflow, s, lend ? ctx->adv_far : nullptr, lend ? ctx->adv_far_words : 0, turn, &far_used, &aa, lend && ctx->col_flags[par] ? &lean : nullptr));
+	if (lean.used) ctx->col_flags_live[par] = true;
+	else FX_HIP(colour_flags_forget(ctx->col_flags[par], ctx->col_flag_boxes, &ctx->col_flags_live[par], s));
+	ctx->lean_count_last = lean.used ? turn : -1;
 	if (aa.written) ctx->accel_alpha_of = ctx->col[par];
 	if (far_used) ++ctx->adv_far_turn;
 	return FX_OK;
@@ -246,6 +252,7 @@
 	DeviceGuard dg(ctx->device);
 	ScopedMark mk(ctx, s, MK_ADVECT);
 	FX_HIP(launch_open_inflow(ctx->g, ctx->half, ctx->vel[0], ctx->col[ctx->frame_parity], alpha_mirror(ctx), ctx->open_faces, ctx->time_step, s));
+	FX_HIP(colour_flags_forget(ctx->col_flags[ctx->frame_parity], ctx->col_flag_boxes, &ctx->col_flags_live[ctx->frame_parity], s));
 	return FX_OK;
 }
 
@@ -255,6 +262,7 @@
 	DeviceGuard dg(ctx->device);
 	ScopedMark mk(ctx, s, MK_ADVECT);
 	FX_HIP(launch_emit(ctx->g, ctx->half, ctx->vel[1], ctx->col[ctx->frame_parity], alpha_mirror(ctx), ctx->emitters.data(), (int)ctx->emitters.size(), ctx->time_step, s));
+	FX_HIP(colour_flags_forget(ctx->col_flags[ctx->frame_parity], ctx->col_flag_boxes, &ctx->col_flags_live[ctx->frame_parity], s));
 	return FX_OK;
 }
 
@@ -276,6 +284,7 @@
 	DeviceGuard dg(ctx->device);
 	ScopedMark mk(ctx, s, MK_ADVECT);
 	FX_HIP(launch_obstacle_enforce(ctx->g, ctx->half, ctx->obst_code, ctx->obst_lo, ctx->obst_hi, ctx->vel[1], ctx->col[ctx->frame_parity], alpha_mirror(ctx), s));
+	FX_HIP(colour_flags_forget(ctx->col_flags[ctx->frame_parity], ctx->col_flag_boxes, &ctx->col_flags_live[ctx->frame_parity], s));
 	return FX_OK;
 }
 
diff --git a/fluidx12_amd/csrc/fx_sim.hip b/fluidx12_amd/csrc/fx_sim.hip
--- a/fluidx12_amd/csrc/fx_sim.hip
+++ b/fluidx12_amd/csrc/fx_sim.hip
@@ -780,10 +780,11 @@
 
 hipError_t launch_advect(const Geom& g, const SimParams& sp, int half_store, const void* vel_in, const void* col_in,
 	void* vel_out, void* col_out, int z_begin, int z_end, unsigned* halo_overflow, hipStream_t s, uint32_t* far_scratch, size_t far_words, int far_parity, bool* far_used,
-	AdvectAlpha* alpha)
+	AdvectAlpha* alpha, AdvectLean* lean)
 {
 	if (far_used) *far_used = false;
 	if (alpha) alpha->written = false;
+	if (lean) lean->used = false;
 	if (z_end <= z_begin) return hipSuccess;
 	int bx = 64, by = 4, bz = 1;
 	if (const char* e = FX_KNOB("ADVECT_BLOCK")) {
@@ -794,7 +795,7 @@
 	{
 		const char* le = FX_KNOB("ADVECT_LDS");
 		if (!(le && le[0] == '0') && bx == 64 && by == 4 && bz == 1 && !xcd_remap_on(REMAP_ADVECT)) {
-			const hipError_t e = launch_advect_lds(g, sp, half_store, vel_in, col_in, vel_out, col_out, z_begin, z_end, halo_overflow, far_scratch, far_words, far_parity, far_used, s, le && le[0] == '2', alpha);
+			const hipError_t e = launch_advect_lds(g, sp, half_store, vel_in, col_in, vel_out, col_out, z_begin, z_end, halo_overflow, far_scratch, far_words, far_parity, far_used, s, le && le[0] == '2', alpha, lean);
 			if (e != hipErrorNotSupported) return e;
 		}
 	}
diff --git a/fluidx12_amd/fluid.py b/fluidx12_amd/fluid.py
--- a/fluidx12_amd/fluid.py
+++ b/fluidx12_amd/fluid.py
@@ -220,6 +220,12 @@
     def Advect(self, stream=None):
         capi.check(self._lib.fx_advect(self._ctx, stream), "Advect")
 
+    def LeanBoxes(self):
+        self._need()
+        n = C.c_uint32(0)
+        capi.check(self._lib.fx_get_lean_boxes(self._ctx, C.byref(n)), "LeanBoxes")
+        return int(n.value)
+
     def SetVorticityConfinement(self, eps):
         self._need()
         capi.check(self._lib.fx_set_vorticity_confinement(self._ctx, float(eps)), "SetVorticityConfinement")
diff --git a/include/fluidx_hip.h b/include/fluidx_hip.h
--- a/include/fluidx_hip.h
+++ b/include/fluidx_hip.h
@@ -136,6 +136,7 @@
 int fx_checkpoint_load(fx_ctx* ctx, const char* path);
 
 int fx_advect(fx_ctx* ctx, void* stream);
+int fx_get_lean_boxes(fx_ctx* ctx, uint32_t* boxes);
 int fx_divergence(fx_ctx* ctx, void* stream);
 int fx_jacobi(fx_ctx* ctx, void* stream, uint32_t iters);
 int fx_project(fx_ctx* ctx, void* stream);
```

After: 21.47 billion. -2.0%, worse.
